# Lapis-Hong/wide_deep

Measured on NVIDIA H100. Metric: CTR examples/sec (train step), higher is better.
Workload: dtype bf16x3 (fp32 operands split into bf16 hi+lo, 3 tensor-core products, fp32 accumulate; 2^-16)

## Files before the change

wide_deep_b200/csrc/api.cu:

```cuda
#include <stdarg.h>
#include <stdlib.h>
#include <string.h>

#include <algorithm>
#include <cmath>
#include <random>

#include "common.cuh"
#include "farmhash.cuh"
#include "sparse_dev.cuh"

namespace wd {
static thread_local char g_err[1024] = "";
void set_error(const char* fmt, ...) {
    va_list ap;
    va_start(ap, fmt);
    vsnprintf(g_err, sizeof(g_err), fmt, ap);
    va_end(ap);
}
int init_sparse_tables(WdModel* m, uint64_t seed, int random_w);
int refresh_weight_copies(WdModel* m);
int wide_bias_grad(WdModel* m);
int metrics_setup();
int merge_sparse(WdModel* m, int which, const void* rows, const void* grads, int64_t n);
// ... 134 lines not shown
    if ((rc = upload(m, &p.col_field, d->col_field, C))) return rc;
    if ((rc = upload(m, &p.col_buckets, d->col_buckets, C))) return rc;
    if ((rc = upload(m, &p.col_aux_off, d->col_aux_off, C))) return rc;
    if ((rc = upload(m, &p.col_aux_n, d->col_aux_n, C))) return rc;
    if ((rc = upload(m, &p.col_norm_kind, d->col_norm_kind, C))) return rc;
    if ((rc = upload(m, &p.col_norm_a, d->col_norm_a, C))) return rc;
    if ((rc = upload(m, &p.col_norm_b, d->col_norm_b, C))) return rc;
    if ((rc = upload(m, &p.col_wide_base, d->col_wide_base, C))) return rc;
    if ((rc = upload(m, &p.col_emb_table, d->col_emb_table, C))) return rc;
    if ((rc = upload(m, &p.col_ind_off, d->col_ind_off, C))) return rc;
    if ((rc = upload(m, &p.vocab_fp, d->vocab_fp, d->n_vocab_fp))) return rc;
    if ((rc = upload(m, &p.boundaries, d->boundaries, d->n_boundaries))) return rc;
    if ((rc = upload(m, &p.cross_key_type, d->cross_key_type, d->n_cross_keys))) return rc;
    if ((rc = upload(m, &p.cross_key_idx, d->cross_key_idx, d->n_cross_keys))) return rc;
    if ((rc = upload(m, &m->d_num_field, d->num_field, d->n_numeric))) return rc;
    if ((rc = upload(m, &m->d_num_norm_kind, d->num_norm_kind, d->n_numeric))) return rc;
    if ((rc = upload(m, &m->d_num_x0_off, d->num_x0_off, d->n_numeric))) return rc;
    if ((rc = upload(m, &m->d_num_a, d->num_norm_a, d->n_numeric))) return rc;
    if ((rc = upload(m, &m->d_num_b, d->num_norm_b, d->n_numeric))) return rc;

    const int64_t Bm = m->max_batch;
    if ((rc = ensure_slot(m, 0))) return rc;
    if ((rc = dev_alloc(m, &m->d_col_offs, Bm * std::max(C, 1) + 2))) return rc;
    if ((rc = dev_alloc(m, &m->d_e_wide, m->max_nnz))) return rc;
    if ((rc = dev_alloc(m, &m->d_e_emb, m->max_nnz))) return rc;
    if ((rc = dev_alloc(m, &m->d_e_bc, m->max_nnz))) return rc;
    if ((rc = dev_alloc(m, &m->d_e_id, m->max_nnz))) return rc;
    if ((rc = dev_alloc(m, &m->d_nnz, 4))) return rc;
    if ((rc = dev_alloc(m, &m->d_flags, 4))) return rc;
    for (int k = 0; k < 4; ++k) if ((rc = dev_alloc(m, &m->d_sort_counter_s[k], 4))) return rc;
    {
        int64_t n = std::max<int64_t>(Bm * std::max(C, 1) + 2, m->max_nnz + 2);
        for (int k = 0; k < 4; ++k) {
            int32_t* t;
            if ((rc = dev_alloc(m, &t, n / 4096 + 8))) return rc;
            m->d_scan_tmp_s[k] = t;
        }
    }
    if ((rc = dev_alloc(m, &m->d_logits, Bm))) return rc;
    if (G == 1 && (rc = dev_alloc(m, &m->d_dlogit, Bm))) return rc;
    if ((rc = dev_alloc(m, &m->d_loss_part, 512))) return rc;
    if ((rc = dev_alloc(m, &m->d_loss, 4))) return rc;
    if ((rc = dev_alloc(m, &m->d_head_counter, 4))) return rc;
    if (getenv("WD_STEP_TRACE") && (rc = dev_alloc(m, &m->d_step_trace, 16))) return rc;
    if ((rc = dev_alloc(m, &m->d_step, 4))) return rc;
    if ((rc = dev_alloc(m, &m->d_bpow, 4))) return rc;
    {
        const float bp[4] = {m->lin_opt.beta1, m->lin_opt.beta2, m->dnn_opt.beta1, m->dnn_opt.beta2};
        WD_CUDA(cudaMemcpyAsync(m->d_bpow, bp, sizeof(bp), cudaMemcpyHostToDevice, m->stream));
        WD_CUDA(cudaStreamSynchronize(m->stream));
    }
    if (G == 1 && (rc = dev_alloc(m, &m->d_metrics, kMetricsDoubles))) return rc;
    WD_CUDA(cudaMallocHost(&m->h_loss_pinned, 64));

    auto add_dense = [&](int rows, int cols, int gparts, int g_rowtiles, int64_t gstride, bool transpose) {
        DenseTensor t{};
        t.off = m->dense_count; t.count = (int64_t)rows * cols; t.rows = rows; t.cols = cols;
        t.gpart_off = m->gpart_count; t.gparts = gparts; t.g_rowtiles = g_rowtiles; t.gstride = gstride;
        t.wt_off = transpose ? m->wt_count : -1;
        m->dense_count += (t.count + 3) / 4 * 4;
        m->gpart_count += (int64_t)gparts * gstride;
        if (transpose) m->wt_count += t.count;
        m->dense.push_back(t);
        return (int)m->dense.size() - 1;
    };
    if (m->use_wide) {
        add_dense(1, 1, m->row_tiles, 1, 4, false);
        if ((rc = dev_alloc(m, &m->d_wide, m->wide_rows))) return rc;
        if (m->lin_opt.kind == WD_OPT_ADAM && (rc = dev_alloc(m, &m->d_adam_touched[1], (m->wide_rows + 31) / 32))) return rc;
        if ((rc = dev_alloc(m, &m->d_wide_logit, Bm))) return rc;
    }

    m->x0_real.assign(std::max(d->d0_phys, 1), 0);
    if (m->use_deep) {
        int64_t row_base = 0;
        const int nslots = opt_nslots(m->dnn_opt);
        for (int t = 0; t < d->n_tables; ++t) {
            EmbTable tb{};
            tb.rows = d->table_rows[t]; tb.dim = d->table_dim[t]; tb.x0_off = d->table_x0_off[t];
            tb.dim_logical = d->table_dim_logical[t];
            if (tb.dim_logical < 1 || tb.dim_logical > tb.dim) { set_error("table %d: bad logical width", t); return WD_EINVAL; }
            tb.row_base = 0; tb.gs_off = -1; tb.stride = tb.dim * (1 + nslots); tb.col = -1;
            tb.sharded = G > 1 && d->table_sharded && d->table_sharded[t];
            tb.arows = tb.sharded ? (tb.rows - m->shard.rank + G - 1) / G : tb.rows;
            if (tb.dim % 4 || tb.x0_off % 4) { set_error("table %d: dim and deep-input offset must be multiples of 4", t); return WD_EINVAL; }
            for (int c = 0; c < C; ++c) if (d->col_emb_table[c] == t) tb.col = c;
            if (tb.col < 0) { set_error("table %d has no producing column", t); return WD_EINVAL; }
            tb.place = d->table_placement ? d->table_placement[t] : WD_PLACE_HBM;
            if (tb.place < WD_PLACE_HBM || tb.place > WD_PLACE_AUTO) { set_error("table %d: placement %d is not a WD_PLACE_*", t, tb.place); return WD_EINVAL; }
            tb.data = nullptr;
            for (int i = 0; i < tb.dim_logical; ++i) m->x0_real[tb.x0_off + i] = 1;
            m->emb_max_dim = std::max(m->emb_max_dim, tb.dim);
            m->tables.push_back(tb);
        }
        for (int pass = 0; pass < 2; ++pass) {
            if (pass == 1) m->small_base[0] = row_base;
            for (int t = 0; t < d->n_tables; ++t) {
                EmbTable& tb = m->tables[t];
                if (tb.sharded) continue;
                const bool small = m->dense_exchange_max_rows > 0 && tb.rows <= m->dense_exchange_max_rows;
                if (small != (pass == 1)) continue;
                if (small) {
                    m->n_small_tab++;
                    tb.gs_off = m->gs_emb_floats;
                    m->gs_emb_floats += tb.rows * tb.dim;
                }
                tb.row_base = row_base;
                row_base += tb.rows;
                m->rtab_order.push_back(t);
            }
        }
        m->emb_total_rows = row_base;
        if (m->dnn_opt.kind == WD_OPT_ADAM && (rc = dev_alloc(m, &m->d_adam_touched[0], (row_base + 31) / 32))) return rc;
        if (row_base >= (1ll << 31)) { set_error("more than 2^31 embedding rows on one device"); return WD_EUNSUPPORTED; }
        for (int i = 0; i < d->n_numeric; ++i) m->x0_real[d->num_x0_off[i]] = 1;
        for (int c = 0; c < C; ++c)
            if (d->col_ind_off[c] >= 0) for (int64_t i = 0; i < d->col_buckets[c]; ++i) m->x0_real[d->col_ind_off[c] + i] = 1;
        for (auto v : m->x0_real) m->d0_logical += v;
        const int nt = (int)m->tables.size();
        for (int t = 0; t < nt; ++t) {
            if (m->tables[t].sharded) continue;
            int di = -1;
            for (int i = 0; i < m->n_dims; ++i) if (m->dims[i] == m->tables[t].dim) di = i;
            if (di < 0) {
                if (m->n_dims == kMaxDims) { set_error("more than %d distinct embedding widths", kMaxDims); return WD_EUNSUPPORTED; }
                di = m->n_dims++; m->dims[di] = m->tables[t].dim; m->dim_ntables[di] = 0;
            }
            m->dim_ntables[di]++;
        }
        const int64_t actn = (int64_t)m->max_batch_pad * d->d0_phys;
        if ((rc = dev_alloc(m, &m->d_X0, actn))) return rc;
        if (fp32_ops && (rc = dev_alloc(m, &m->d_X0T, actn))) return rc;
        if (G == 1 && (rc = dev_alloc(m, &m->d_dX0, actn))) return rc;
        if (!fp32_ops)
            for (int part = 0; part < 2; ++part) {
                if ((rc = dev_alloc(m, &m->d_X0s[part], actn))) return rc;
            }

        if (d->n_towers > kMaxTowers) { set_error("more than %d towers", kMaxTowers); return WD_EUNSUPPORTED; }
        int hu_off = 0, did = 0;
        for (int t = 0; t < d->n_towers; ++t) {
            Tower tw{};
            tw.n_hidden = d->tower_nlayers[t]; tw.mode = d->tower_mode[t];
            std::vector<int> hu(d->hidden_units + hu_off, d->hidden_units + hu_off + tw.n_hidden);
            hu_off += tw.n_hidden;
            const std::vector<int> units = hu;
            if (m->crelu) for (int& h : hu) h *= 2;
            auto srcs = layer_sources(tw.mode, tw.n_hidden);
            for (int l = 0; l <= tw.n_hidden; ++l) {
                Layer L{};
                if ((int)srcs[l].size() > kMaxSegs) { set_error("layer with more than %d concatenated inputs", kMaxSegs); return WD_EUNSUPPORTED; }
                L.n_in_segs = (int)srcs[l].size();
                int koff = 0, klog = 0;
                for (int s = 0; s < L.n_in_segs; ++s) {
                    int src = srcs[l][s];
                    Seg sg{};
                    sg.src = src;
                    sg.width = src < 0 ? m->d0_logical : hu[src];
                    sg.width_phys = src < 0 ? d->d0_phys : pad_to(hu[src], 32);
                    sg.k_off = koff;
                    koff += sg.width_phys; klog += sg.width;
                    L.segs[s] = sg;
                }
                L.K = klog; L.K_phys = koff;
                const bool hidden = l < tw.n_hidden;
                L.N = hidden ? hu[l] : 1;
                L.N_phys = hidden ? pad_to(hu[l], 32) : 1;
                L.N_param = hidden ? units[l] : 1;
                L.t_gamma = L.t_beta = -1;
                bool logits_reads = false;
                for (int src : srcs[tw.n_hidden]) if (src == l) logits_reads = true;
                std::vector<int> idx(4, -1);
                if (hidden) {
                    {
                        const int tiles = ((L.K_phys + 127) / 128) * ((L.N_phys + 127) / 128);
                        int num_sms = kNumSms;
                        cudaDeviceGetAttribute(&num_sms, cudaDevAttrMultiProcessorCount, m->device);
                        int sp = m->wgrad_splits;
                        while (sp < 32 && tiles * sp * 2 <= num_sms && m->max_batch_pad / (sp * 2) >= 512) sp *= 2;
                        L.wgrad_splits = sp;
                    }
                    L.t_kernel = add_dense(L.K_phys, L.N_phys, L.wgrad_splits, 0, (int64_t)L.K_phys * L.N_phys, true);
                    L.t_bias = add_dense(1, L.N_phys, m->row_tiles, 1, L.N_phys, false);
                    if (m->crelu) m->dense[L.t_kernel].mirror_u = m->dense[L.t_bias].mirror_u = L.N_param;
                    if (m->batch_norm) {
                        L.t_gamma = add_dense(1, L.N_phys, m->row_tiles, 1, L.N_phys, false);
                        L.t_beta = add_dense(1, L.N_phys, m->row_tiles, 1, L.N_phys, false);
                    }
                    const int64_t n = (int64_t)m->max_batch_pad * L.N_phys;
                    if ((fp32_ops || logits_reads) && (rc = dev_alloc(m, &L.H, n))) return rc;
                    if (m->batch_norm || m->dropout_rate > 0.f || !L.H) { if ((rc = dev_alloc(m, &L.A, n))) return rc; } else L.A = L.H;
                    if (fp32_ops && (rc = dev_alloc(m, &L.HT, n))) return rc;
                    if ((rc = dev_alloc(m, &L.dH, n))) return rc;
                    if (fp32_ops) {
                        if ((rc = dev_alloc(m, &L.dZ, n))) return rc;
                        if ((rc = dev_alloc(m, &L.dZT, n))) return rc;
                    } else
                        for (int part = 0; part < 2; ++part) {
                            if ((rc = dev_alloc(m, &L.Hs[part], n))) return rc;
                            if ((rc = dev_alloc(m, &L.dZs[part], n))) return rc;
                        }
                } else {
                    L.t_kernel = add_dense(L.K_phys, 1, m->row_tiles, 1, L.K_phys, false);
                    L.t_bias = add_dense(1, 1, m->row_tiles, 1, 4, false);
                }
                idx[WD_D_KERNEL] = L.t_kernel; idx[WD_D_BIAS] = L.t_bias; idx[WD_D_GAMMA] = L.t_gamma; idx[WD_D_BETA] = L.t_beta;
                m->dense_index.push_back(idx);
                m->did_tower.push_back(t); m->did_layer.push_back(l);
                ++did;
                tw.layers.push_back(L);
            }
            if ((rc = dev_alloc(m, &tw.logit, Bm))) return rc;
            m->towers.push_back(tw);
        }
    }
    {
        const int64_t nw_small = m->use_wide ? m->wide_rows - m->small_base[1] : 0;
        const int64_t ne_small = (m->use_deep && m->n_small_tab > 0) ? m->emb_total_rows - m->small_base[0] : 0;
        const int64_t grads = m->gs_emb_floats + nw_small;
        m->gs_touch_off[0] = grads;
        m->gs_touch_off[1] = grads + ne_small;
        m->gs_count = grads > 0 ? grads + ne_small + nw_small : 0;
    }
    if (m->dense_count > 0) {
        if ((rc = dev_alloc(m, &m->d_P, m->dense_count))) return rc;
        if ((rc = dev_alloc(m, &m->d_S1, m->dense_count))) return rc;
        if ((rc = dev_alloc(m, &m->d_S2, m->dense_count))) return rc;
        if (G == 1 && (rc = dev_alloc(m, &m->d_G, m->dense_count + m->gs_count))) return rc;
        if ((rc = dev_alloc(m, &m->d_gpart, m->gpart_count))) return rc;
        if (fp32_ops) {
            if ((rc = dev_alloc(m, &m->d_Wt, m->wt_count))) return rc;
            float* split;
            if ((rc = dev_alloc(m, &split, 4 * m->wt_count))) return rc;
            m->d_W_hi = split; m->d_W_lo = split + m->wt_count; m->d_Wt_hi = split + 2 * m->wt_count; m->d_Wt_lo = split + 3 * m->wt_count;
        } else {
            if ((rc = dev_alloc(m, &m->d_Wq_hi, m->wt_count))) return rc;
            if ((rc = dev_alloc(m, &m->d_Wq_lo, m->wt_count))) return rc;
        }
        if ((rc = upload(m, &m->d_dense_desc, m->dense))) return rc;
    }

    m->sort_bits[0] = bits_for(std::max<int64_t>(m->emb_total_rows, 2));
    m->sort_bits[1] = bits_for(std::max<int64_t>(m->wide_rows, 2));
    if (m->sort_bits[0] > 30 || m->sort_bits[1] > 30) { set_error("more than 2^30 rows in one table space on one device"); return WD_EUNSUPPORTED; }
    const int which_lo = (m->use_deep && !m->tables.empty()) ? 0 : 1, which_hi = m->use_wide ? 1 : 0;
    for (int w = which_lo; w <= which_hi; ++w) {
        if ((rc = dev_alloc(m, &m->d_sk[w], m->max_nnz + 8))) return rc;
        if ((rc = dev_alloc(m, &m->d_sv[w], m->max_nnz + 8))) return rc;
        if ((rc = dev_alloc(m, &m->d_sk2[w], m->max_nnz + 8))) return rc;
        if ((rc = dev_alloc(m, &m->d_sv2[w], m->max_nnz + 8))) return rc;
        if ((rc = dev_alloc(m, &m->d_urow[w], m->max_nnz + 8))) return rc;
        if ((rc = dev_alloc(m, &m->d_ustart[w], m->max_nnz + 8))) return rc;
        if ((rc = dev_alloc(m, &m->d_ugrad[w], (m->max_nnz + 8) * (w == 0 ? std::max(m->emb_max_dim, 4) : 1)))) return rc;
        if ((rc = dev_alloc(m, &m->d_nuniq[w], 4))) return rc;
        if ((rc = dev_alloc(m, &m->d_nubig[w], 4))) return rc;
        if ((rc = dev_alloc(m, &m->d_nvalid[w], 4))) return rc;
        m->cpart_cap = 2 * (m->max_nnz / 16) + 64;
        if ((rc = dev_alloc(m, &m->d_choff[w], m->max_nnz + 8))) return rc;
        if ((rc = dev_alloc(m, &m->d_nchunks[w], 4))) return rc;
        if ((rc = dev_alloc(m, &m->d_cpart[w], m->cpart_cap * (w == 0 ? std::max(m->emb_max_dim, 4) : 1)))) return rc;
        m->sparse_cap[w] = m->max_nnz;
    }
    m->sort_hist_cap = 1024 * ((m->max_nnz + kSortTile - 1) / kSortTile + 1) + 4 * 1024 + 64;
    for (int k = 0; k < 4; ++k) if ((rc = dev_alloc(m, &m->d_sort_hist_s[k], m->sort_hist_cap))) return rc;
    if (m->use_deep) {
        if ((rc = place_tables(m, hbm_reserve_bytes(m) + (G > 1 ? shard_hbm_bytes(m, d) : 0)))) return rc;
    }
    if (G > 1 && (rc = shard_build(m, d))) return rc;
    if ((rc = build_record_sets(m))) return rc;
    if (G > 1) {
        DevPlan& dp = m->dplan;
        dp.sh_world = G;
        for (int sx = 0; sx < 2; ++sx) {
            ShardSpace& sp = m->shard.sp[sx];
            if (!sp.on) continue;
            if (sx == 0) { dp.sh_col_emb = sp.d_col_slot; dp.sh_base_emb = sp.set.rec.row_base; dp.sh_own_emb = sp.d_own; dp.sh_lrow_emb = sp.d_lrow; }
            else { dp.sh_col_wide = sp.d_col_slot; dp.sh_base_wide = sp.set.rec.row_base; dp.sh_own_wide = sp.d_own; dp.sh_lrow_wide = sp.d_lrow; }
        }
    }
    if ((rc = metrics_setup())) return rc;
    if ((rc = init_sparse_tables(m, 0, 0))) return rc;
    if ((rc = init_dense_slots(m))) return rc;
    for (auto& e : m->timer.ev) WD_CUDA(new_event(m, &e, cudaEventDefault));
    WD_CUDA(cudaStreamSynchronize(m->stream));
    return WD_OK;
}

extern "C" int wd_model_create(const WdPlanDesc* d, int device, WdModel** out) {
    if (!d || !out) { set_error("null argument"); return WD_EINVAL; }
    if (d->api_version != WD_API_VERSION) { set_error("plan api_version %d != library %d", d->api_version, WD_API_VERSION); return WD_EINVAL; }
    int ndev = 0;
    if (cudaGetDeviceCount(&ndev) != cudaSuccess || ndev == 0) {
        set_error("no CUDA device: libwd_b200 has no CPU fallback");
        return WD_ENODEVICE;
    }
    if (device < 0 || device >= ndev) { set_error("device %d out of range (%d devices)", device, ndev); return WD_EINVAL; }
    WD_CUDA(cudaSetDevice(device));
    WdModel* m = new WdModel();
    m->device = device;
    cudaError_t e = cudaSuccess;
    for (cudaStream_t* s : {&m->stream, &m->stream_up, &m->sstream[0], &m->sstream[1]})
        if (e == cudaSuccess) e = new_stream(m, s);
    for (cudaEvent_t* ev : {&m->ev_grouped[0], &m->ev_grouped[1], &m->ev_done[0], &m->ev_done[1], &m->ev_ids, &m->ev_wide_fwd,
                            &m->ev_wgrad_rest, &m->ev_head, &m->ev_dx0, &m->ev_bwd_done})
        if (e == cudaSuccess) e = new_event(m, ev, cudaEventDisableTiming);
    if (e != cudaSuccess) { set_error("cudaStreamCreate: %s", cudaGetErrorString(e)); wd_model_destroy(m); return WD_ECUDA; }
    m->graphs_enabled = getenv("WD_NO_GRAPH") == nullptr;
    int rc = build_model(d, m);
    if (rc) { wd_model_destroy(m); return rc; }
    *out = m;
    return WD_OK;
}

namespace wd {
int64_t hbm_reserve_bytes(const WdModel* m) {
    constexpr int kReserveSlots = 16;
    constexpr int64_t kGraphReserve = 256ll << 20;
    const int64_t Bm = m->max_batch;
    const int64_t slot_bytes = (Bm * std::max(m->n_cat_fields, 1) + 1) * 4 + m->keys_cap * 8 + Bm * std::max(m->n_dense_fields, 1) * 4 + 2 * Bm * 4;
    int max_stride = 0;
    for (auto& tb : m->tables) max_stride = std::max(max_stride, tb.stride);
    const int64_t stage_bytes = m->max_nnz * ((int64_t)max_stride + 1) * 4 + 64 * (int64_t)m->tables.size() + 4096;
    return kReserveSlots * slot_bytes + stage_bytes + kGraphReserve;
}
}

static int init_dense(WdModel* m, uint64_t seed) {
    if (m->dense_count == 0) return WD_OK;
    std::vector<float> P(m->dense_count, 0.f), S1(m->dense_count, 0.f), S2(m->dense_count, 0.f);
    std::mt19937_64 rng(seed * 7919 + 17);
    std::uniform_real_distribution<float> U(-1.f, 1.f);
    for (size_t ti = 0; ti < m->towers.size(); ++ti) {
        Tower& tw = m->towers[ti];
        for (int l = 0; l <= tw.n_hidden; ++l) {
            Layer& L = tw.layers[l];
            const DenseTensor& tk = m->dense[L.t_kernel];
            const float lim = std::sqrt(6.f / (float)(L.K + L.N_param));
            for (int s = 0; s < L.n_in_segs; ++s) {
                const Seg& sg = L.segs[s];
                for (int j = 0; j < sg.width_phys; ++j) {
                    bool real = sg.src < 0 ? (m->x0_real[j] != 0) : (j < sg.width);
                    if (!real) continue;
                    float* prow = &P[tk.off + (int64_t)(sg.k_off + j) * L.N_phys];
                    for (int n = 0; n < L.N_param; ++n) {
                        prow[n] = lim * U(rng);
                        if (tk.mirror_u) prow[n + tk.mirror_u] = -prow[n];
                    }
                }
            }
            if (L.t_gamma >= 0) for (int n = 0; n < L.N; ++n) P[m->dense[L.t_gamma].off + n] = 1.f;
        }
    }
    for (size_t i = 0; i < m->dense.size(); ++i) {
        const WdOptimizer& o = (m->use_wide && i == 0) ? m->lin_opt : m->dnn_opt;
        float s1 = slot1_init(o);
        for (int64_t j = 0; j < m->dense[i].count; ++j) S1[m->dense[i].off + j] = s1;
    }
    WD_CUDA(cudaMemcpyAsync(m->d_P, P.data(), P.size() * 4, cudaMemcpyHostToDevice, m->stream));
    WD_CUDA(cudaMemcpyAsync(m->d_S1, S1.data(), S1.size() * 4, cudaMemcpyHostToDevice, m->stream));
    WD_CUDA(cudaMemcpyAsync(m->d_S2, S2.data(), S2.size() * 4, cudaMemcpyHostToDevice, m->stream));
    WD_CUDA(cudaStreamSynchronize(m->stream));
    return refresh_weight_copies(m);
}

extern "C" int wd_model_init(WdModel* m, uint64_t seed) {
    if (!m) { set_error("null model"); return WD_EINVAL; }
    WD_CUDA(cudaSetDevice(m->device));
    int rc = init_sparse_tables(m, seed, 1);
    if (rc) return rc;
    rc = init_dense(m, seed);
    if (rc) return rc;
    WD_CUDA(cudaStreamSynchronize(m->stream));
    m->initialized = true;
    return WD_OK;
}

static int resolve_dense(WdModel* m, int did, int sub, int* out) {
    if (did < 0 || did >= (int)m->dense_index.size() || sub < 0 || sub > 3 || m->dense_index[did][sub] < 0) {
        set_error("no dense tensor (%d, %d)", did, sub);
        return WD_EINVAL;
    }
    *out = m->dense_index[did][sub];
    return WD_OK;
}

extern "C" int64_t wd_tensor_size(WdModel* m, int kind, int index, int sub) {
    if (!m) return WD_EINVAL;
    if (kind == WD_T_WIDE_COL) {
        if (index < 0 || index >= m->n_columns) return WD_EINVAL;
        const ShardSpace& sw = m->shard.sp[1];
        if (sw.on && sw.h_col_slot[index] >= 0) return (m->col_buckets[index] - m->shard.rank + m->shard.world - 1) / m->shard.world;
        return m->col_wide_base[index] >= 0 ? m->col_buckets[index] : WD_EINVAL;
    }
    if (kind == WD_T_WIDE_BIAS) return m->use_wide ? 1 : WD_EINVAL;
    if (kind == WD_T_EMB_TABLE) return (index >= 0 && index < (int)m->tables.size()) ? m->tables[index].arows * m->tables[index].dim_logical : WD_EINVAL;
    if (kind == WD_T_DENSE) {
        int di;
        if (resolve_dense(m, index, sub, &di)) return WD_EINVAL;
        Layer& L = m->towers[m->did_tower[index]].layers[m->did_layer[index]];
        return sub == WD_D_KERNEL ? (int64_t)L.K * L.N_param : (sub == WD_D_BIAS ? L.N_param : L.N);
    }
    return WD_EINVAL;
}

extern "C" int wd_memory_usage(WdModel* m, int64_t* device_bytes, int64_t* host_bytes) {
    if (!m) { set_error("null model"); return WD_EINVAL; }
    if (device_bytes) *device_bytes = m->bytes_allocated;
    if (host_bytes) *host_bytes = m->host_bytes;
    return WD_OK;
}

extern "C" int wd_tensor_io(WdModel* m, int kind, int index, int sub, int slot, void* host, int64_t count, int to_device) {
    if (!m || !host) { set_error("null argument"); return WD_EINVAL; }
    WD_CUDA(cudaSetDevice(m->device));
    WD_CUDA(cudaStreamSynchronize(m->stream));
    int64_t want = wd_tensor_size(m, kind, index, sub);
    if (want < 0 || want != count) { set_error("tensor (%d,%d,%d): size %lld, caller passed %lld", kind, index, sub, (long long)want, (long long)count); return WD_EINVAL; }
    if (slot < 0 || slot > 2) { set_error("slot out of range"); return WD_EINVAL; }
    const cudaMemcpyKind dir = to_device ? cudaMemcpyHostToDevice : cudaMemcpyDeviceToHost;
    if (kind == WD_T_WIDE_COL) {
        const ShardSpace& sw = m->shard.sp[1];
        float* dev = (sw.on && sw.h_col_slot[index] >= 0)
                         ? reinterpret_cast<float*>(sw.d_wide + sw.h_slot_base[sw.h_col_slot[index]]) + slot
                         : reinterpret_cast<float*>(m->d_wide + m->col_wide_base[index]) + slot;
        if (to_device) WD_CUDA(cudaMemcpy2DAsync(dev, 16, host, 4, 4, count, dir, m->stream));
        else WD_CUDA(cudaMemcpy2DAsync(host, 4, dev, 16, 4, count, dir, m->stream));
        WD_CUDA(cudaStreamSynchronize(m->stream));
        return WD_OK;
    }
    if (kind == WD_T_EMB_TABLE) {
        EmbTable& tb = m->tables[index];
        if (slot * tb.dim >= tb.stride) { set_error("table has no optimizer slot %d", slot); return WD_EINVAL; }
        float* dev = tb.data + slot * tb.dim;
        const size_t lw = (size_t)tb.dim_logical * 4;
        if (tb.host) {
            const int rc = host_cache_sync(m, true, to_device != 0);
            if (rc) return rc;
        }
        const cudaMemcpyKind dir = tb.host ? cudaMemcpyDefault : (to_device ? cudaMemcpyHostToDevice : cudaMemcpyDeviceToHost);
        if (to_device) WD_CUDA(cudaMemcpy2DAsync(dev, (size_t)tb.stride * 4, host, lw, lw, tb.arows, dir, m->stream));
        else WD_CUDA(cudaMemcpy2DAsync(host, lw, dev, (size_t)tb.stride * 4, lw, tb.arows, dir, m->stream));
        WD_CUDA(cudaStreamSynchronize(m->stream));
        return WD_OK;
    }
    float* arena = slot == 0 ? m->d_P : (slot == 1 ? m->d_S1 : m->d_S2);
    if (kind == WD_T_WIDE_BIAS) {
        WD_CUDA(cudaMemcpyAsync(to_device ? (void*)(arena + m->dense[0].off) : host, to_device ? host : (void*)(arena + m->dense[0].off), 4, dir, m->stream));
        WD_CUDA(cudaStreamSynchronize(m->stream));
        return WD_OK;
    }
    int di;
    int rc = resolve_dense(m, index, sub, &di);
    if (rc) return rc;
    const DenseTensor& t = m->dense[di];
    Layer& L = m->towers[m->did_tower[index]].layers[m->did_layer[index]];
    std::vector<float> phys(t.count, 0.f);
    float* h = (float*)host;
    if (!to_device || slot > 0) {
        WD_CUDA(cudaMemcpyAsync(phys.data(), arena + t.off, t.count * 4, cudaMemcpyDeviceToHost, m->stream));
        WD_CUDA(cudaStreamSynchronize(m->stream));
    }
    if (sub == WD_D_KERNEL) {
        int64_t lk = 0;
        for (int s = 0; s < L.n_in_segs; ++s) {
            const Seg& sg = L.segs[s];
            for (int j = 0; j < sg.width_phys; ++j) {
                bool real = sg.src < 0 ? (m->x0_real[j] != 0) : (j < sg.width);
                if (!real) continue;
                for (int n = 0; n < L.N_param; ++n) {
                    float& pv = phys[(int64_t)(sg.k_off + j) * L.N_phys + n];
                    if (to_device) {
                        pv = h[lk * L.N_param + n];
                        if (t.mirror_u) (&pv)[t.mirror_u] = slot == 0 ? -pv : pv;
                    } else h[lk * L.N_param + n] = pv;
                }
                ++lk;
            }
        }
        if (lk != L.K) { set_error("internal: logical K mismatch %lld vs %d", (long long)lk, L.K); return WD_ESTATE; }
    } else {
        const int nn = sub == WD_D_BIAS ? L.N_param : L.N;
        for (int n = 0; n < nn; ++n) {
            if (to_device) {
                phys[n] = h[n];
                if (t.mirror_u) phys[n + t.mirror_u] = slot == 0 ? -h[n] : h[n];
            } else h[n] = phys[n];
        }
    }
    if (to_device) {
        WD_CUDA(cudaMemcpyAsync(arena + t.off, phys.data(), t.count * 4, cudaMemcpyHostToDevice, m->stream));
        WD_CUDA(cudaStreamSynchronize(m->stream));
        if (slot == 0 && t.wt_off >= 0) return refresh_weight_copies(m);
    }
    return WD_OK;
}

static int check_ready(WdModel* m) {
    if (!m) { set_error("null model"); return WD_EINVAL; }
    WD_CUDA(cudaSetDevice(m->device));
    return WD_OK;
}
static void timer_begin(WdModel* m) {
    if (!m->timer.enabled) return;
    m->timer.n = 0;
    mark(m, "start");
}

static int ensure_slot(WdModel* m, int s) {
    if (s < 0 || s >= 64) { set_error("batch slot %d out of range [0, 64)", s); return WD_EINVAL; }
    while ((int)m->slots.size() <= s) {
        BatchSlot b;
        int rc;
        const int64_t Bm = m->max_batch;
        if ((rc = dev_alloc(m, &b.off, Bm * std::max(m->n_cat_fields, 1) + 1))) return rc;
        if ((rc = dev_alloc(m, &b.keys, m->keys_cap))) return rc;
        if ((rc = dev_alloc(m, &b.dense, Bm * std::max(m->n_dense_fields, 1)))) return rc;
        if ((rc = dev_alloc(m, &b.label, Bm))) return rc;
        if ((rc = dev_alloc(m, &b.weight, Bm))) return rc;
        m->slots.push_back(b);
    }
    return WD_OK;
}
static int select_slot(WdModel* m, int s) {
    int rc = ensure_slot(m, s);
    if (rc) return rc;
    BatchSlot& b = m->slots[s];
    m->cur_slot = s;
    if (b.filled) m->dbatch = b.view;
    if (b.up_pending) {
        WD_CUDA(cudaStreamWaitEvent(m->stream, b.ev_up, 0));
        b.up_pending = false;
    }
    return WD_OK;
}
static int use_slot(WdModel* m, int slot, const char* needs_labels) {
    int rc = select_slot(m, slot);
    if (rc) return rc;
    if (!m->slots[slot].filled) { set_error("batch slot %d was never uploaded", slot); return WD_ESTATE; }
    if (needs_labels && !m->dbatch.label) { set_error("%s needs labels", needs_labels); return WD_EINVAL; }
    return WD_OK;
}
static void fill_slot(WdModel* m, int s, const DevBatch& view, bool pending) {
    BatchSlot& sl = m->slots[s];
    sl.view = view;
    sl.filled = true;
    if (pending) sl.up_pending = true;
    if (s == m->cur_slot) m->dbatch = view;
}
static int mark_slot_used(WdModel* m) {
    BatchSlot& b = m->slots[m->cur_slot];
    if (!b.ev_used) WD_CUDA(new_event(m, &b.ev_used, cudaEventDisableTiming));
    WD_CUDA(cudaEventRecord(b.ev_used, m->stream));
    b.used_recorded = true;
    return WD_OK;
}

static int upload_into(WdModel* m, BatchSlot& sl, const WdBatch* b, cudaStream_t st, DevBatch* view) {
    if (!b || b->batch_size <= 0 || b->batch_size > m->max_batch) { set_error("batch_size %d outside (0, %d]", b ? b->batch_size : -1, m->max_batch); return WD_EINVAL; }
    const int B = b->batch_size, F = m->n_cat_fields, Nd = m->n_dense_fields;
    int64_t nnz = b->cat_offsets ? b->nnz : (int64_t)B * F;
    if (nnz > m->keys_cap) { set_error("batch has %lld keys, capacity %lld (raise max_keys)", (long long)nnz, (long long)m->keys_cap); return WD_EINVAL; }
    if (F > 0) {
        if (b->cat_offsets) WD_CUDA(cudaMemcpyAsync(sl.off, b->cat_offsets, ((int64_t)B * F + 1) * 4, cudaMemcpyHostToDevice, st));
        if (nnz > 0) WD_CUDA(cudaMemcpyAsync(sl.keys, b->cat_keys, nnz * 8, cudaMemcpyHostToDevice, st));
    }
    if (Nd > 0) WD_CUDA(cudaMemcpyAsync(sl.dense, b->dense, (int64_t)B * Nd * 4, cudaMemcpyHostToDevice, st));
    if (b->label) WD_CUDA(cudaMemcpyAsync(sl.label, b->label, (int64_t)B * 4, cudaMemcpyHostToDevice, st));
    if (b->weight) WD_CUDA(cudaMemcpyAsync(sl.weight, b->weight, (int64_t)B * 4, cudaMemcpyHostToDevice, st));
    view->B = B;
    view->cat_offsets = (F > 0 && b->cat_offsets) ? sl.off : nullptr;
    view->cat_keys = sl.keys;
    view->dense = sl.dense;
    view->label = b->label ? sl.label : nullptr;
    view->weight = b->weight ? sl.weight : nullptr;
    return WD_OK;
}

static int upload_current(WdModel* m, const WdBatch* b) {
    DevBatch view{};
    int rc = upload_into(m, m->slots[m->cur_slot], b, m->stream, &view);
    if (rc) return rc;
    fill_slot(m, m->cur_slot, view, false);
    mark(m, "h2d");
    return WD_OK;
}

extern "C" int wd_batch_prefetch_slot(WdModel* m, int slot, const WdBatch* b) {
    int rc = check_ready(m);
    if (rc) return rc;
    if ((rc = ensure_slot(m, slot))) return rc;
    BatchSlot& sl = m->slots[slot];
    if (!sl.ev_up) WD_CUDA(new_event(m, &sl.ev_up, cudaEventDisableTiming));
    if (sl.used_recorded) WD_CUDA(cudaStreamWaitEvent(m->stream_up, sl.ev_used, 0));
    DevBatch view{};
    if ((rc = upload_into(m, sl, b, m->stream_up, &view))) return rc;
    WD_CUDA(cudaEventRecord(sl.ev_up, m->stream_up));
    fill_slot(m, slot, view, true);
    return WD_OK;
}

extern "C" int wd_tsv_parse_slot(WdModel* m, int slot, const WdTsvSpec* sp, const char* text, int64_t text_len, const int64_t* starts,
                                 int32_t n_lines) {
    int rc = check_ready(m);
    if (rc) return rc;
    if (!sp || !text || !starts || n_lines < 0 || text_len < 0) { set_error("wd_tsv_parse_slot: bad arguments"); return WD_EINVAL; }
    if ((rc = ensure_slot(m, slot))) return rc;
    BatchSlot& sl = m->slots[slot];
    if (!sl.ev_up) WD_CUDA(new_event(m, &sl.ev_up, cudaEventDisableTiming));
    if (sl.used_recorded) WD_CUDA(cudaStreamWaitEvent(m->stream_up, sl.ev_used, 0));
    int status = 0;
    if ((rc = tsv_parse_device(m, sp, text, text_len, starts, n_lines, sl.off, sl.keys, sl.dense, sl.label, sl.weight, m->stream_up, &status))) return rc;
    DevBatch view{};
    if (status == 0) {
        view.B = n_lines;
        view.cat_offsets = m->n_cat_fields > 0 ? sl.off : nullptr;
        view.cat_keys = sl.keys;
        view.dense = sl.dense;
        view.label = sp->has_label ? sl.label : nullptr;
        view.weight = (sp->use_weight && sp->has_label) ? sl.weight : nullptr;
        m->tsv_device_batches++;
    } else {
        WdBatch hb{};
        if ((rc = tsv_parse_host(sp, text, starts, n_lines, &hb))) return rc;
        if ((rc = upload_into(m, sl, &hb, m->stream_up, &view))) return rc;
        m->tsv_host_batches++;
    }
    WD_CUDA(cudaEventRecord(sl.ev_up, m->stream_up));
    if (status != 0) WD_CUDA(cudaEventSynchronize(sl.ev_up));
    fill_slot(m, slot, view, true);
    return WD_OK;
}

extern "C" int wd_tsv_parse_stats(WdModel* m, int64_t* out, int32_t n, int32_t reset) {
    if (!m) { set_error("null model"); return WD_EINVAL; }
    const int64_t v[2] = {m->tsv_device_batches, m->tsv_host_batches};
    for (int i = 0; i < n && i < 2; ++i) out[i] = v[i];
    if (reset) m->tsv_device_batches = m->tsv_host_batches = 0;
    return WD_OK;
}

extern "C" int wd_batch_upload_slot(WdModel* m, int slot, const WdBatch* b) {
    int rc = check_ready(m);
    if (rc) return rc;
    if ((rc = select_slot(m, slot))) return rc;
    return upload_current(m, b);
}
extern "C" int wd_batch_upload(WdModel* m, const WdBatch* b) { return wd_batch_upload_slot(m, 0, b); }

static int finish_step(WdModel* m, float* loss_out, float* logits_out) {
    int32_t* flags_host = reinterpret_cast<int32_t*>(m->h_loss_pinned + 4);
    WD_CUDA(cudaMemcpyAsync(m->h_loss_pinned, m->d_loss, 4, cudaMemcpyDeviceToHost, m->stream));
    WD_CUDA(cudaMemcpyAsync(flags_host, m->d_flags, 4, cudaMemcpyDeviceToHost, m->stream));
    if (logits_out) WD_CUDA(cudaMemcpyAsync(logits_out, m->d_logits, (int64_t)m->dbatch.B * 4, cudaMemcpyDeviceToHost, m->stream));
    mark(m, "d2h");
    WD_CUDA(cudaStreamSynchronize(m->stream));
    if (flags_host[0] & 1) {
        cudaMemsetAsync(m->d_flags, 0, 16, m->stream);
        set_error("categorical-column id capacity exceeded (max_nnz=%lld): recreate the model with a larger max_nnz", (long long)m->max_nnz);
        return WD_EINVAL;
    }
    if (flags_host[0] & 2) {
        cudaMemsetAsync(m->d_flags, 0, 16, m->stream);
        set_error("row-sharded exchange capacity exceeded (a rank received more than %lld ids): raise shard_slack / shard_capacity", (long long)m->max_nnz);
        return WD_EINVAL;
    }
    if (flags_host[0] & 8) {
        cudaMemsetAsync(m->d_flags, 0, 16, m->stream);
        set_error("data-parallel list exchange: this rank touched more unique rows than the fixed list length it exchanges (wd_sparse_set_sorted list_len); raise fixed_rows");
        return WD_EINVAL;
    }
    if (flags_host[0] & 4) {
        cudaMemsetAsync(m->d_flags, 0, 16, m->stream);
        set_error("row-sharded exchange: a peer rank did not reach a barrier within 20 s (ranks out of step, or a rank failed)");
        return WD_ESTATE;
    }
    if (loss_out) *loss_out = m->dbatch.label ? m->h_loss_pinned[0] : 0.f;
    if (m->timer.enabled) {
        PhaseTimer& t = m->timer;
        for (int i = 1; i < t.n; ++i) cudaEventElapsedTime(&t.ms[i], t.ev[i - 1], t.ev[i]);
        t.ms[0] = 0.f;
        if (t.n > 1) cudaEventElapsedTime(&t.ms[0], t.ev[0], t.ev[t.n - 1]);
        t.n_last = t.n;
    }
    return WD_OK;
}

static bool list_present(const WdModel* m, int which) { return which == 0 ? (m->use_deep && !m->tables.empty()) : m->use_wide; }

__global__ void step_stamp_kernel(unsigned long long* t) { unsigned long long v; asm volatile("mov.u64 %0, %%globaltimer;" : "=l"(v)); *t = v; }
enum { ST_START = 0, ST_IDS, ST_GATHER, ST_HEAD, ST_BWD, ST_MAIN_END, ST_G0, ST_G1, ST_R0_BEG, ST_R0_END, ST_R1_BEG, ST_R1_END, ST_A0_END, ST_A1_END };
static void stamp(WdModel* m, int i) {
    if (!m->d_step_trace) return;
    step_stamp_kernel<<<1, 1, 0, m->stream>>>(m->d_step_trace + i);
    m->launches++;
}

namespace wd {
int group_async(WdModel* m) {
    if (m->timer.enabled) return WD_OK;
    WD_CUDA(cudaEventRecord(m->ev_ids, m->stream));
    for (int w = 0; w < 2; ++w) {
        if (!list_present(m, w)) continue;
        WD_CUDA(cudaStreamWaitEvent(m->sstream[w], m->ev_ids, 0));
        int rc = on_side(m, w, [&] { int r = sparse_group_which(m, w); stamp(m, ST_G0 + w); return r; });
        if (rc) return rc;
        WD_CUDA(cudaEventRecord(m->ev_grouped[w], m->sstream[w]));
        m->side_pending[w] = true;
    }
    return WD_OK;
}

static int forward_core(WdModel* m, bool train) {
    int rc;
    m->stepped = true;
    stamp(m, ST_START);
    if ((rc = ids_prepare(m))) return rc;
    mark(m, "ids");
    stamp(m, ST_IDS);
    const bool wide_aside = train && !m->timer.enabled && m->use_wide && m->use_deep && list_present(m, 1);
    if (wide_aside) {
        WD_CUDA(cudaEventRecord(m->ev_ids, m->stream));
        WD_CUDA(cudaStreamWaitEvent(m->sstream[1], m->ev_ids, 0));
        if ((rc = on_side(m, 1, [&] { return sparse_forward_wide(m); }))) return rc;
        WD_CUDA(cudaEventRecord(m->ev_wide_fwd, m->sstream[1]));
    }
    if (train && (rc = group_async(m))) return rc;
    if (!wide_aside && (rc = sparse_forward_wide(m))) return rc;
    if (m->n_host_tab > 0) {
        if (m->side_pending[0]) WD_CUDA(cudaStreamWaitEvent(m->stream, m->ev_grouped[0], 0));
        else if ((rc = sparse_group_which(m, 0))) return rc;
        if ((rc = host_tables_stage_in(m, train))) return rc;
    }
    if ((rc = sparse_forward_emb(m))) return rc;
    stamp(m, ST_GATHER);
    if ((rc = mlp_forward(m, train))) return rc;
    mark(m, "mlp_other");
    if (wide_aside) WD_CUDA(cudaStreamWaitEvent(m->stream, m->ev_wide_fwd, 0));
    if ((rc = loss_forward(m, train))) return rc;
    mark(m, "head");
    stamp(m, ST_HEAD);
    if (train && (m->side_pending[0] || m->side_pending[1])) WD_CUDA(cudaEventRecord(m->ev_head, m->stream));
    if (train && m->summary_armed && (rc = summary_launch(m))) return rc;
    return WD_OK;
}

int backward_core(WdModel* m) {
    int rc;
    m->side_active[0] = m->side_active[1] = false;
    if (m->gs_count > 0) WD_CUDA(cudaMemsetAsync(m->d_G + m->dense_count, 0, (size_t)m->gs_count * sizeof(float), m->stream));
    if (m->side_pending[1]) {
        if (m->gs_count > 0) { WD_CUDA(cudaEventRecord(m->ev_head, m->stream)); }
        WD_CUDA(cudaStreamWaitEvent(m->sstream[1], m->ev_head, 0));
        if ((rc = on_side(m, 1, [&] { stamp(m, ST_R1_BEG); int r = sparse_reduce_wide(m); if (!r) r = small_scatter(m, 1); stamp(m, ST_R1_END); return r; }))) return rc;
        m->side_active[1] = true;
    }
    m->record_dx0 = m->side_pending[0];
    m->dx0_recorded = false;
    m->dense_split_tensor = -1;
    m->record_wgrad_rest = m->fuse_dense && m->side_active[1] && m->operands == kBf16Operands && !m->timer.enabled && !m->crelu;
    if ((rc = mlp_backward(m))) return rc;
    m->record_dx0 = false;
    m->record_wgrad_rest = false;
    mark(m, "mlp_other");
    stamp(m, ST_BWD);
    if (m->side_pending[0] && m->dx0_recorded) {
        WD_CUDA(cudaStreamWaitEvent(m->sstream[0], m->ev_dx0, 0));
        if ((rc = on_side(m, 0, [&] { stamp(m, ST_R0_BEG); int r = sparse_reduce_emb(m); if (!r) r = small_scatter(m, 0); stamp(m, ST_R0_END); return r; }))) return rc;
        m->side_active[0] = true;
    }
    if ((rc = wide_bias_grad(m))) return rc;
    if ((rc = dense_reduce_grads(m))) return rc;
    mark(m, "dense_reduce");
    for (int w = 0; w < 2; ++w) {
        if (m->side_active[w] || !list_present(m, w)) { m->side_pending[w] = false; continue; }
        if (m->side_pending[w]) WD_CUDA(cudaStreamWaitEvent(m->stream, m->ev_grouped[w], 0));
        else if ((rc = sparse_group_which(m, w))) return rc;
        m->side_pending[w] = false;
        if ((rc = (w == 0 ? sparse_reduce_emb(m) : sparse_reduce_wide(m)))) return rc;
        if ((rc = small_scatter(m, w))) return rc;
    }
    if (m->gs_count > 0)
        for (int w = 0; w < 2; ++w)
            if (m->side_active[w]) {
                WD_CUDA(cudaEventRecord(m->ev_done[w], m->sstream[w]));
                WD_CUDA(cudaStreamWaitEvent(m->stream, m->ev_done[w], 0));
            }
    m->grads_pending = true;
    return WD_OK;
}

int apply_core(WdModel* m) {
    int rc;
    const bool split_dense = m->fuse_dense && m->dense_split_tensor >= 0 && m->side_active[1];
    for (int w = 0; w < 2; ++w) {
        if (m->side_active[w]) {
            if ((rc = on_side(m, w, [&]() -> int {
                    int r = sparse_apply_which(m, w);
                    stamp(m, ST_A0_END + w);
                    if (!r && w == 1 && split_dense) {
                        WD_CUDA(cudaStreamWaitEvent(m->stream, m->ev_wgrad_rest, 0));
                        m->dense_part = 2;
                        r = dense_apply(m);
                        m->dense_part = 0;
                    }
                    return r;
                }))) return rc;
            WD_CUDA(cudaEventRecord(m->ev_done[w], m->sstream[w]));
        } else if ((rc = sparse_apply_which(m, w))) return rc;
    }
    mark(m, "sparse_apply");
    m->dense_part = split_dense ? 1 : 0;
    rc = dense_apply(m);
    m->dense_part = 0;
    if (rc) return rc;
    if ((rc = small_apply(m))) return rc;
    mark(m, "dense_apply");
    stamp(m, ST_MAIN_END);
    if (m->dropout_rate > 0.f && (rc = step_tick(m))) return rc;
    if (m->lin_opt.kind == WD_OPT_ADAM || m->dnn_opt.kind == WD_OPT_ADAM) {
        for (int w = 0; w < 2; ++w)
            if (m->side_active[w]) WD_CUDA(cudaStreamWaitEvent(m->stream, m->ev_done[w], 0));
        if ((rc = adam_untouched_replicated(m))) return rc;
        mark(m, "adam_untouched");
        if ((rc = adam_tick(m))) return rc;
    }
    for (int w = 0; w < 2; ++w)
        if (m->side_active[w]) { WD_CUDA(cudaStreamWaitEvent(m->stream, m->ev_done[w], 0)); m->side_active[w] = false; }
    m->grads_pending = false;
    return WD_OK;
}
}

static int train_eager(WdModel* m) {
    int rc;
    m->fuse_dense = true;
    rc = forward_core(m, true);
    if (!rc) rc = backward_core(m);
    if (!rc) rc = apply_core(m);
    m->fuse_dense = false;
    return rc;
}

enum class GraphRun { eager, captured, replayed };

template <class Key, class F>
static int run_graphed(WdModel* m, StepGraph<Key>& g, const Key& key, cudaStream_t st, F issue, GraphRun* how) {
    *how = GraphRun::eager;
    if (!m->graphs_enabled || m->timer.enabled) return issue(false);
    if (g.exec && g.key == key) {
        *how = GraphRun::replayed;
        m->graph_replays++;
    } else if (g.eager < 2) {
        const int rc = issue(false);
        if (rc == WD_OK) g.eager++;
        return rc;
    } else {
        g.destroy();
        const int64_t l0 = m->launches;
        cudaGraph_t graph = nullptr;
        cudaError_t e = cudaStreamBeginCapture(st, cudaStreamCaptureModeThreadLocal);
        if (e == cudaSuccess) {
            const int rc = issue(true);
            const cudaError_t e2 = cudaStreamEndCapture(st, &graph);
            if (rc == WD_OK && e2 == cudaSuccess && graph) e = cudaGraphInstantiate(&g.exec, graph, 0);
            else e = e2 != cudaSuccess ? e2 : cudaErrorUnknown;
            if (graph) cudaGraphDestroy(graph);
        }
        if (e != cudaSuccess || !g.exec) {
            cudaGetLastError();
            g.exec = nullptr;
            m->graphs_enabled = false;
            return issue(false);
        }
        g.key = key;
        g.launches = m->launches - l0;
        m->launches = l0;
        *how = GraphRun::captured;
        m->graph_captures++;
    }
    WD_CUDA(cudaGraphLaunch(g.exec, st));
    m->launches += g.launches;
    return WD_OK;
}

template <class Key, class F>
static int run_train_graphed(WdModel* m, StepGraph<Key>& g, const Key& key, F issue, GraphRun* how) {
    if (m->summary_armed) {
        *how = GraphRun::eager;
        return issue(false);
    }
    return run_graphed(m, g, key, m->stream, issue, how);
}

static int after_graph(WdModel* m, GraphRun how, BatchSlot* bwd) {
    if (how == GraphRun::eager) return WD_OK;
    if (bwd && how == GraphRun::captured)
        for (int w = 0; w < 2; ++w) bwd->bwd_side_active[w] = m->side_active[w];
    if (bwd) WD_CUDA(cudaEventRecord(m->ev_bwd_done, m->stream));
    for (int w = 0; w < 2; ++w) {
        m->side_pending[w] = false;
        m->side_active[w] = bwd && bwd->bwd_side_active[w];
        if (m->side_active[w]) WD_CUDA(cudaStreamWaitEvent(m->sstream[w], m->ev_bwd_done, 0));
    }
    m->grads_pending = bwd != nullptr;
    return WD_OK;
}

static int train_current(WdModel* m, float* loss_out) {
    GraphRun how;
    int rc = run_train_graphed(m, m->slots[m->cur_slot].train, m->dbatch, [&](bool) { return train_eager(m); }, &how);
    if (rc) return rc;
    if ((rc = after_graph(m, how, nullptr))) return rc;
    if ((rc = mark_slot_used(m))) return rc;
    if (loss_out) return finish_step(m, loss_out, nullptr);
    return WD_OK;
}

extern "C" int wd_train_step_slot(WdModel* m, int slot, float* loss_out) {
    int rc = check_ready(m);
    if (rc) return rc;
    if ((rc = use_slot(m, slot, "training"))) return rc;
    timer_begin(m);
    return train_current(m, loss_out);
}
extern "C" int wd_train_step_resident(WdModel* m, float* loss_out) { return wd_train_step_slot(m, 0, loss_out); }

extern "C" int wd_train_step(WdModel* m, const WdBatch* b, float* loss_out) {
    int rc = check_ready(m);
    if (rc) return rc;
    if ((rc = select_slot(m, 0))) return rc;
    timer_begin(m);
    if ((rc = upload_current(m, b))) return rc;
    if ((rc = use_slot(m, 0, "training"))) return rc;
    float dummy;
    return train_current(m, loss_out ? loss_out : &dummy);
}

extern "C" int wd_forward_resident(WdModel* m, float* logits_out, float* loss_out) {
    int rc = check_ready(m);
    if (rc) return rc;
    if ((rc = select_slot(m, 0))) return rc;
    timer_begin(m);
    if ((rc = forward_core(m, false))) return rc;
    return finish_step(m, loss_out, logits_out);
}

extern "C" int wd_forward(WdModel* m, const WdBatch* b, float* logits_out, float* loss_out) {
    int rc = check_ready(m);
    if (rc) return rc;
    if ((rc = select_slot(m, 0))) return rc;
    timer_begin(m);
    if ((rc = upload_current(m, b))) return rc;
    if ((rc = forward_core(m, false))) return rc;
    return finish_step(m, loss_out, logits_out);
}


static int backward_eager(WdModel* m, bool join) {
    int rc;
    if ((rc = forward_core(m, true))) return rc;
    if ((rc = backward_core(m))) return rc;
    if (join)
        for (int w = 0; w < 2; ++w)
            if (m->side_active[w]) {
                WD_CUDA(cudaEventRecord(m->ev_done[w], m->sstream[w]));
                WD_CUDA(cudaStreamWaitEvent(m->stream, m->ev_done[w], 0));
            }
    return WD_OK;
}

static int refuse_split_step_with_cache(WdModel* m) {
    if (m->hcache.slots == 0) return WD_OK;
    set_error("the split step (wd_step_backward / wd_step_apply) is not supported on a model with a host-table cache");
    return WD_EUNSUPPORTED;
}

extern "C" int wd_step_backward_slot(WdModel* m, int slot, float* loss_out) {
    int rc = check_ready(m);
    if (rc) return rc;
    if ((rc = use_slot(m, slot, "training"))) return rc;
    if ((rc = refuse_split_step_with_cache(m))) return rc;
    timer_begin(m);
    BatchSlot& sl = m->slots[slot];
    GraphRun how;
    if ((rc = run_train_graphed(m, sl.bwd, m->dbatch, [&](bool capturing) { return backward_eager(m, capturing); }, &how))) return rc;
    if ((rc = after_graph(m, how, &sl))) return rc;
    if ((rc = mark_slot_used(m))) return rc;
    if (loss_out) return finish_step(m, loss_out, nullptr);
    return WD_OK;
}

extern "C" int wd_last_loss(WdModel* m, float* loss_out) {
    int rc = check_ready(m);
    if (rc) return rc;
    if (!loss_out) { set_error("wd_last_loss: null output"); return WD_EINVAL; }
    return finish_step(m, loss_out, nullptr);
}

extern "C" int wd_step_backward(WdModel* m, const WdBatch* b, float* loss_out) {
    int rc = check_ready(m);
    if (rc) return rc;
    if ((rc = refuse_split_step_with_cache(m))) return rc;
    if (b && (rc = wd_batch_upload(m, b))) return rc;
    timer_begin(m);
    if (!m->dbatch.label) { set_error("training needs labels"); return WD_EINVAL; }
    if ((rc = forward_core(m, true))) return rc;
    if ((rc = backward_core(m))) return rc;
    if (loss_out) return finish_step(m, loss_out, nullptr);
    return WD_OK;
}

extern "C" int wd_step_apply(WdModel* m) {
    int rc = check_ready(m);
    if (rc) return rc;
    if (!m->grads_pending) { set_error("wd_step_apply without wd_step_backward"); return WD_ESTATE; }
    return apply_core(m);
}

extern "C" int64_t wd_dense_grad_count(WdModel* m) { return m ? m->dense_count + m->gs_count : 0; }
extern "C" void* wd_dense_grad_ptr(WdModel* m) { return m ? m->d_G : nullptr; }

extern "C" int wd_sparse_grads(WdModel* m, int which, void** rows, void** grads, int64_t* n, int32_t* width, int64_t* capacity) {
    int rc = check_ready(m);
    if (rc) return rc;
    if (which < 0 || which > 1 || !m->d_urow[which]) { set_error("no sparse gradient list %d", which); return WD_EINVAL; }
    if (n) {
        int32_t nu = 0;
        WD_CUDA(cudaStreamSynchronize(m->stream));
        WD_CUDA(cudaStreamSynchronize(m->sstream[which]));
        WD_CUDA(cudaMemcpy(&nu, m->d_nuniq[which], 4, cudaMemcpyDeviceToHost));
        *n = nu;
    }
    if (rows) *rows = m->d_urow[which];
    if (grads) *grads = m->d_ugrad[which];
    if (width) *width = which == 0 ? m->emb_max_dim : 1;
    if (capacity) *capacity = m->sparse_cap[which];
    return WD_OK;
}

static int sparse_set_impl(WdModel* m, int which, const void* rows_dev, const void* grads_dev, int64_t n, int n_lists, int64_t list_len) {
    int rc = check_ready(m);
    if (rc) return rc;
    if (which < 0 || which > 1 || !m->d_urow[which]) { set_error("no sparse gradient list %d", which); return WD_EINVAL; }
    const bool side = m->side_active[which];
    auto merge = [&]() -> int {
        return n_lists > 0 ? merge_sparse_sorted(m, which, rows_dev, grads_dev, n_lists, list_len) : merge_sparse(m, which, rows_dev, grads_dev, n);
    };
    auto run = [&](bool) -> int { return side ? on_side(m, which, merge) : merge(); };
    if (n_lists == 0) return run(false);
    GraphRun how;
    return run_graphed(m, m->merge_graph[which], MergeKey{rows_dev, grads_dev, n_lists, list_len, side}, side ? m->sstream[which] : m->stream, run, &how);
}

extern "C" int wd_sparse_set(WdModel* m, int which, const void* rows_dev, const void* grads_dev, int64_t n) {
    return sparse_set_impl(m, which, rows_dev, grads_dev, n, 0, 0);
}
extern "C" int wd_sparse_set_sorted(WdModel* m, int which, const void* rows_dev, const void* grads_dev, int32_t n_lists, int64_t list_len) {
    if (n_lists < 1 || list_len < 1) { set_error("wd_sparse_set_sorted: bad list shape"); return WD_EINVAL; }
    return sparse_set_impl(m, which, rows_dev, grads_dev, 0, n_lists, list_len);
}

static int shard_ready(WdModel* m, int slot, const char* needs_labels) {
    int rc = check_ready(m);
    if (rc) return rc;
    if (m->shard.world <= 1) { set_error("model has no row-sharded tables (shard_world <= 1)"); return WD_ESTATE; }
    if (!m->shard.connected) { set_error("row-sharded model is not connected to its peers (wd_shard_connect_ipc / wd_shard_connect_local)"); return WD_ESTATE; }
    return use_slot(m, slot, needs_labels);
}

extern "C" int wd_shard_phase(WdModel* m, int slot, int phase, int train) {
    int rc = shard_ready(m, slot, train ? "training" : nullptr);
    if (rc) return rc;
    if (m->shard.ipc) { set_error("wd_shard_phase is for ranks of one process; multi-process ranks call wd_shard_train_step_slot"); return WD_ESTATE; }
    if (phase < 0 || phase > 4) { set_error("wd_shard_phase: phase %d outside [0, 4]", phase); return WD_EINVAL; }
    if (phase == 0) timer_begin(m);
    if ((rc = shard_step(m, train != 0, phase))) return rc;
    return train && phase == 4 ? mark_slot_used(m) : WD_OK;
}

extern "C" int wd_shard_finish(WdModel* m, float* loss_out, float* logits_out) {
    int rc = check_ready(m);
    if (rc) return rc;
    return finish_step(m, loss_out, logits_out);
}

extern "C" int wd_shard_train_step_slot(WdModel* m, int slot, float* loss_out) {
    int rc = shard_ready(m, slot, "training");
    if (rc) return rc;
    if (!m->shard.ipc) { set_error("wd_shard_train_step_slot needs wd_shard_connect_ipc (ranks of one process use wd_shard_phase)"); return WD_ESTATE; }
    timer_begin(m);
    GraphRun how;
    if ((rc = run_train_graphed(m, m->slots[slot].shard, m->dbatch, [&](bool) { return shard_step(m, true, kAllSegments); }, &how))) return rc;
    if ((rc = after_graph(m, how, nullptr))) return rc;
    if ((rc = mark_slot_used(m))) return rc;
    if (loss_out) return finish_step(m, loss_out, nullptr);
    return WD_OK;
}

extern "C" int wd_shard_forward_slot(WdModel* m, int slot, float* logits_out, float* loss_out) {
    int rc = shard_ready(m, slot, nullptr);
    if (rc) return rc;
    if (!m->shard.ipc) { set_error("wd_shard_forward_slot needs wd_shard_connect_ipc"); return WD_ESTATE; }
    if ((rc = shard_step(m, false, kAllSegments))) return rc;
    return finish_step(m, loss_out, logits_out);
}

namespace wd { int shard_metrics_reduce(WdModel* m); }

static int check_eval_rows(WdModel* m, int32_t n_valid) {
    if (n_valid < 0 || n_valid > m->dbatch.B) { set_error("n_valid %d outside [0, batch size %d]", n_valid, m->dbatch.B); return WD_EINVAL; }
    if (n_valid > 0 && !m->dbatch.label) { set_error("evaluation needs labels"); return WD_EINVAL; }
    return WD_OK;
}

extern "C" int wd_shard_eval_accumulate_slot(WdModel* m, int slot, int32_t n_valid) {
    int rc = shard_ready(m, slot, nullptr);
    if (rc) return rc;
// ... 191 lines not shown
```

wide_deep_b200/csrc/common.cuh:

```cuda
#pragma once
#include <cuda_bf16.h>
#include <cuda_runtime.h>
#include <stdint.h>
#include <stdio.h>
#include <string>
#include <vector>

#include "../../include/wd_b200.h"

namespace wd {

constexpr int kSortTile = 1024;

void set_error(const char* fmt, ...);

#define WD_CUDA(call)                                                                         \
    do {                                                                                      \
        cudaError_t e__ = (call);                                                             \
        if (e__ != cudaSuccess) {                                                             \
            wd::set_error("%s:%d %s -> %s", __FILE__, __LINE__, #call, cudaGetErrorString(e__)); \
            return WD_ECUDA;                                                                  \
        }                                                                                     \
    } while (0)

constexpr uint32_t kInvalidRow = 0xFFFFFFFFu;
constexpr int kMaxSegs = 8;
constexpr int kMaxTowers = 8;
constexpr int kNumSms = 132;
constexpr int kMaxDims = 8;
constexpr int kLists = 6;
constexpr int kMaxRanks = 16;
constexpr int kMetricsDoubles = 512;

struct DevPlan {
    int n_cat_fields, n_dense_fields, n_columns;
    const uint8_t* field_is_string;
    const int32_t* col_kind;
    const int32_t* col_field;
    const int64_t* col_buckets;
    const int32_t* col_aux_off;
    const int32_t* col_aux_n;
    const int32_t* col_norm_kind;
    const float* col_norm_a;
    const float* col_norm_b;
    const int64_t* col_wide_base;
    const int32_t* col_emb_table;
    const int32_t* col_ind_off;
    const uint64_t* vocab_fp;
    const float* boundaries;
    const int32_t* cross_key_type;
    const int32_t* cross_key_idx;
    const int64_t* table_row_base;
    int d0_phys;
    int sh_world;
    const int32_t *sh_col_emb, *sh_col_wide;
    const int64_t *sh_base_emb, *sh_base_wide;
    uint32_t *sh_own_emb, *sh_lrow_emb, *sh_own_wide, *sh_lrow_wide;
};

struct DevBatch {
    int B;
    const int32_t* cat_offsets;
    const uint64_t* cat_keys;
    const float* dense;
    const float* label;
    const float* weight;
};

struct EmbTable {
    int64_t rows;
    int dim;
    int dim_logical;
    int x0_off;
    int col;
    int64_t row_base;
    int64_t gs_off;
    float* data;
    int stride;
    bool sharded;
    int64_t arows;
    int place;
    bool host;
};

struct TabDesc {
    float* data;
    int64_t row_base;
    int stride, x0, col, dim;
};

struct RowRecords {
    int ntab;
    const int64_t* row_base;
    float* const* data;
    const int32_t* dim;
    const int32_t* stride;
    const int32_t* stage;
    float* stage_base;
    const int32_t* uslot;
};
struct RecordSet {
    RowRecords rec{};
    const int32_t* x0 = nullptr;
    const int64_t* rows = nullptr;
    const int64_t* gs_off = nullptr;
};

struct HostCache {
    int64_t slots = 0;
    int set_bits = 0;
    uint32_t* d_tag = nullptr;
    uint32_t* d_stamp = nullptr;
    uint8_t* d_dirty = nullptr;
    uint32_t* d_now = nullptr;
    unsigned long long* d_stats = nullptr;
    int32_t* d_uslot = nullptr;
    uint32_t* d_uvict = nullptr;
    uint8_t* d_uflag = nullptr;
    uint32_t *d_ck[2] = {}, *d_cv[2] = {};
};

struct DenseTensor {
    int64_t off;
    int64_t count;
    int rows, cols;
    int64_t gpart_off;
    int gparts;
    int g_rowtiles;
    int64_t gstride;
    int64_t wt_off;
    int mirror_u;
};

enum OperandFamily { kFp32Operands = 0, kBf16Operands = 1 };

struct Seg {
    int src;
    int width;
    int width_phys;
    int k_off;
};

struct Layer {
    int n_in_segs;
    Seg segs[kMaxSegs];
    int K, K_phys;
    int N, N_phys;
    int N_param;
    int t_kernel, t_bias, t_gamma, t_beta;
    int wgrad_splits;
    float* A;
    float* H;
    float* HT;
    float* dH;
    float* dZ;
    float* dZT;
    __nv_bfloat16 *Hs[2], *dZs[2];
    float* colpart;
};

struct Tower {
    int n_hidden;
    int mode;
    std::vector<Layer> layers;
    float* logit;
};

struct PhaseTimer {
    static constexpr int kMax = 160;
    cudaEvent_t ev[kMax];
    const char* name[kMax];
    float ms[kMax];
    int n = 0, n_last = 0;
    bool enabled = false;
};

template <class Key>
struct StepGraph {
    cudaGraphExec_t exec = nullptr;
    Key key{};
    int64_t launches = 0;
    int eager = 0;
    void destroy() {
        if (exec) cudaGraphExecDestroy(exec);
        exec = nullptr;
    }
};
inline bool operator==(const DevBatch& a, const DevBatch& b) {
    return a.B == b.B && a.cat_offsets == b.cat_offsets && a.cat_keys == b.cat_keys && a.dense == b.dense && a.label == b.label && a.weight == b.weight;
}
struct MergeKey {
    const void* rows;
    const void* grads;
    int n_lists;
    int64_t list_len;
    bool on_side;
    bool operator==(const MergeKey& o) const {
        return rows == o.rows && grads == o.grads && n_lists == o.n_lists && list_len == o.list_len && on_side == o.on_side;
    }
};

struct ShardEvalKey {
    DevBatch b;
    int n_valid;
    bool operator==(const ShardEvalKey& o) const { return b == o.b && n_valid == o.n_valid; }
};

struct BatchSlot {
    int32_t* off = nullptr;
    uint64_t* keys = nullptr;
    float *dense = nullptr, *label = nullptr, *weight = nullptr;
    DevBatch view{};
    bool filled = false;
    cudaEvent_t ev_up = nullptr;
    cudaEvent_t ev_used = nullptr;
    bool up_pending = false, used_recorded = false;
    StepGraph<DevBatch> train;
    StepGraph<DevBatch> bwd;
    StepGraph<DevBatch> shard;
    StepGraph<ShardEvalKey> shard_eval;
    bool bwd_side_active[2] = {false, false};
};


struct ShardPeer {
    uint2* inbox;
    int32_t* inbox_cnt;
    float* recv;
    const float* bagscale;
    const float* gradbase;
};
struct ShardSpace {
    bool on = false;
    int width = 0;
    int n_slots = 0;
    int bags_per_row = 0;
    int64_t nbags_cap = 0;
    int64_t local_rows = 0;
    int64_t pair_cap = 0;
    std::vector<int32_t> h_col_slot;
    std::vector<int64_t> h_slot_base;
    int32_t* d_col_slot = nullptr;
    RecordSet set;
    uint32_t* d_adam_touched = nullptr;
    int stage_stride = 0;
    float* d_stage = nullptr;
    HostCache cache;
    float4* d_wide = nullptr;
    uint32_t* d_own = nullptr;
    uint32_t* d_lrow = nullptr;
    int32_t* d_ostart = nullptr;
    int32_t* d_bagmask = nullptr;
    uint32_t* d_rtag = nullptr;
    uint32_t* d_rrow = nullptr;
    int32_t* d_nrecv = nullptr;
    ShardPeer* d_peers = nullptr;
    ShardPeer peers[kMaxRanks];
    int64_t off_inbox = 0, off_cnt = 0, off_recv = 0, off_bagscale = 0, off_grad = 0;
};
struct ShardState {
    int world = 1, rank = 0;
    bool connected = false, ipc = false;
    uint8_t* seg = nullptr;
    int64_t seg_bytes = 0;
    uint8_t* peer_seg[kMaxRanks] = {};
    ShardSpace sp[2];
    int64_t off_flags = 0, off_gred = 0, off_G = 0;
    int64_t off_metrics = 0;
    double* d_msum = nullptr;
    uint32_t** d_peer_flags = nullptr;
    uint32_t* d_epoch = nullptr;
    unsigned long long* d_trace = nullptr;
    float** d_peer_G = nullptr;
    float** d_peer_gred = nullptr;
    float* gred = nullptr;
    int64_t ar_count = 0;
    cudaEvent_t ev_a = nullptr;
    cudaStream_t aux = nullptr;
    cudaEvent_t ev_ids2 = nullptr, ev_routed1 = nullptr, ev_a2 = nullptr, ev_aux_done = nullptr;
};
constexpr int kBarriers = 8;
constexpr int kAllSegments = -1;

constexpr int kSummaryThreads = 256;
constexpr int kSummaryZeroBucket = (WD_SUMMARY_BUCKETS + 1) / 2;
struct SummarySeg {
    int kind;
    const float* ptr; int ld, cols;
    const uint8_t* mask;
    const float *gamma, *beta; int bn;
    float drop_rate; int layer_id;
    int blk0, nblk;
};
struct SummaryState {
    std::vector<SummarySeg> h;
    std::vector<int32_t> kind, tower, layer;
    int blocks = 0;
    SummarySeg* d_seg = nullptr;
    uint8_t* d_mask = nullptr;
    double* d_limits = nullptr;
    unsigned long long* d_counts = nullptr;
    double* d_part = nullptr;
    long long* d_ipart = nullptr;
};

struct TsvDev;

struct DevAlloc { void* p; int64_t bytes; };

}

struct WdModel {
    int device = 0;
    bool use_wide = false, use_deep = false;
    int n_cat_fields = 0, n_dense_fields = 0, n_columns = 0;
    std::vector<int32_t> col_kind, col_field, col_aux_off, col_aux_n, col_norm_kind, col_emb_table, col_ind_off;
    std::vector<int64_t> col_buckets, col_wide_base;
    std::vector<float> col_norm_a, col_norm_b;
    int n_numeric = 0;
    int d0_phys = 0;
    int64_t wide_rows = 0;
    int activation = 0, batch_norm = 0;
    WdOptimizer lin_opt{}, dnn_opt{};
    int max_batch = 0, max_batch_pad = 0;
    int64_t max_nnz = 0;
    int gemm_engine = 0;
    wd::OperandFamily operands = wd::kFp32Operands;

    cudaStream_t stream = nullptr;
    cudaStream_t sstream[2] = {nullptr, nullptr};
    cudaStream_t stream_up = nullptr;
    cudaEvent_t ev_ids = nullptr, ev_head = nullptr, ev_dx0 = nullptr, ev_bwd_done = nullptr, ev_wide_fwd = nullptr, ev_wgrad_rest = nullptr;
    bool sort_smem_opt_in = false;
    bool crelu = false;
    bool list_apply_fused[2] = {false, false};
    bool record_wgrad_rest = false;
    int dense_split_tensor = -1, dense_part = 0;
    cudaEvent_t ev_grouped[2] = {nullptr, nullptr}, ev_done[2] = {nullptr, nullptr};
    bool side_pending[2] = {false, false};
    bool side_active[2] = {false, false};
    bool record_dx0 = false, dx0_recorded = false;
    wd::StepGraph<wd::MergeKey> merge_graph[2];
    int64_t dense_exchange_max_rows = 0;
    int64_t small_base[2] = {0, 0};
    int64_t gs_count = 0, gs_emb_floats = 0;
    int64_t gs_touch_off[2] = {0, 0};
    int n_small_tab = 0;
    uint32_t* d_adam_touched[2] = {nullptr, nullptr};
    int32_t* d_nubig[2] = {nullptr, nullptr};
    wd::ShardState shard;
    wd::DevPlan dplan{};
    std::vector<cudaStream_t> streams;
    std::vector<cudaEvent_t> events;
    std::vector<wd::DevAlloc> allocs;
    int64_t bytes_allocated = 0;
    std::vector<void*> host_allocs;
    int64_t host_bytes = 0;
    int n_host_tab = 0;
    std::vector<int> rtab_order;
    float* d_stage = nullptr;
    int stage_stride = 0;
    uint32_t* d_g_emb = nullptr;
    wd::HostCache hcache;
    bool stepped = false;

    int32_t *d_num_field = nullptr, *d_num_norm_kind = nullptr, *d_num_x0_off = nullptr;
    float *d_num_a = nullptr, *d_num_b = nullptr;

    int64_t keys_cap = 0;
    wd::DevBatch dbatch{};

    int32_t* d_col_offs = nullptr;
    uint32_t* d_e_wide = nullptr;
    uint32_t* d_e_emb = nullptr;
    int32_t* d_e_bc = nullptr;
    int32_t* d_e_id = nullptr;
    int32_t* d_nnz = nullptr;
    int32_t* d_flags = nullptr;
    void* d_scan_tmp_s[4] = {nullptr, nullptr, nullptr, nullptr};
    int scratch_sel = 0;

    float4* d_wide = nullptr;
    float* d_wide_logit = nullptr;

    std::vector<wd::EmbTable> tables;
    int64_t emb_total_rows = 0;
    int emb_max_dim = 0;
    int n_dims = 0;
    int dims[wd::kMaxDims];
    int dim_ntables[wd::kMaxDims];
    wd::RecordSet tabs;
    wd::RecordSet rtabs;
    wd::TabDesc* d_dim_desc[wd::kMaxDims] = {};
    float *d_X0 = nullptr, *d_dX0 = nullptr;
    float* d_X0T = nullptr;
    __nv_bfloat16* d_X0s[2] = {nullptr, nullptr};
    int ldt = 0;
    std::vector<wd::Tower> towers;

    std::vector<wd::DenseTensor> dense;
    int64_t dense_count = 0, gpart_count = 0, wt_count = 0;
    float *d_P = nullptr, *d_S1 = nullptr, *d_S2 = nullptr, *d_G = nullptr, *d_gpart = nullptr;
    float* d_Wt = nullptr;
    float *d_W_hi = nullptr, *d_W_lo = nullptr;
    float *d_Wt_hi = nullptr, *d_Wt_lo = nullptr;
    __nv_bfloat16 *d_Wq_hi = nullptr, *d_Wq_lo = nullptr;
    wd::DenseTensor* d_dense_desc = nullptr;
    int row_tiles = 0;
    int wgrad_splits = 4;

    float* d_logits = nullptr;
    float* d_dlogit = nullptr;
    float* d_loss_part = nullptr;
    float* d_loss = nullptr;
    unsigned long long* d_step_trace = nullptr;
    int32_t* d_head_counter = nullptr;
    float* d_bpow = nullptr;
    float* h_loss_pinned = nullptr;

    uint32_t *d_sk[wd::kLists] = {}, *d_sv[wd::kLists] = {};
    uint32_t *d_sk2[wd::kLists] = {}, *d_sv2[wd::kLists] = {};
    int32_t* d_sort_hist_s[4] = {nullptr, nullptr, nullptr, nullptr};
    int64_t sort_hist_cap = 0;
    int32_t* d_sort_counter_s[4] = {nullptr, nullptr, nullptr, nullptr};
    uint32_t* d_urow[wd::kLists] = {};
    int32_t* d_ustart[wd::kLists] = {};
    float* d_ugrad[wd::kLists] = {};
    int32_t* d_nuniq[wd::kLists] = {};
    int32_t* d_nvalid[wd::kLists] = {};
    int32_t* d_choff[wd::kLists] = {};
    int32_t* d_nchunks[wd::kLists] = {};
    float* d_cpart[wd::kLists] = {};
    int64_t cpart_cap = 0;
    int64_t sparse_cap[2] = {0, 0};
    bool sparse_overridden[2] = {false, false};
    int64_t sparse_override_n[2] = {0, 0};
    int sort_bits[wd::kLists] = {};

    double* d_metrics = nullptr;
    int64_t eval_batches = 0;

    int64_t launches = 0;
    int64_t graph_captures = 0, graph_replays = 0;
    float dropout_rate = 0.f;
    unsigned long long dropout_seed = 0;
    unsigned int* d_step = nullptr;
    bool fuse_dense = false;
    int64_t gemm_fallbacks = 0;
    int cur_slot = 0;
    bool graphs_enabled = true;
    int cur_layer = 0;
    wd::PhaseTimer timer;
    std::vector<wd::BatchSlot> slots;
    wd::TsvDev* tsv = nullptr;
    int64_t tsv_device_batches = 0, tsv_host_batches = 0;
    bool initialized = false;
    bool grads_pending = false;
    wd::SummaryState* summ = nullptr;
    bool summary_armed = false, summary_ready = false;

    std::vector<uint8_t> x0_real;
    int d0_logical = 0;
    std::vector<std::vector<int>> dense_index;
    std::vector<int> did_tower, did_layer;
};

namespace wd {
int ids_prepare(WdModel* m);
int sparse_forward(WdModel* m);
int sparse_forward_wide(WdModel* m);
int sparse_forward_emb(WdModel* m);
int sparse_group(WdModel* m);
int sparse_reduce_emb(WdModel* m);
int sparse_reduce_wide(WdModel* m);
int sparse_apply(WdModel* m);
int sparse_apply_which(WdModel* m, int which);
int sparse_group_which(WdModel* m, int which);
int merge_sparse_sorted(WdModel* m, int which, const void* rows, const void* grads, int n_lists, int64_t list_len);
int small_scatter(WdModel* m, int which);
int small_apply(WdModel* m);
int adam_untouched_replicated(WdModel* m);
int mlp_forward(WdModel* m, bool want_transposes);
int mlp_backward(WdModel* m);
int dense_reduce_grads(WdModel* m);
int dense_apply(WdModel* m);
int loss_forward(WdModel* m, bool need_grad);
int model_init_params(WdModel* m, uint64_t seed);
int step_tick(WdModel* m);
int adam_tick(WdModel* m);
int place_tables(WdModel* m, int64_t hbm_reserve);
int build_record_sets(WdModel* m);
int host_tables_stage_in(WdModel* m, bool train);
int host_tables_write_back(WdModel* m);
int host_cache_sync(WdModel* m, bool flush, bool invalidate);
struct CacheMarks { const char *sort, *assign, *in, *out; };
int stage_in_rows(WdModel* m, HostCache& c, int L, const RowRecords& rr, int S, bool train, const CacheMarks& marks);
int write_back_rows(WdModel* m, const HostCache& c, int L, const RowRecords& rr, int S, const CacheMarks& marks);
int64_t shard_hbm_bytes(const WdModel* m, const WdPlanDesc* d);
int64_t hbm_reserve_bytes(const WdModel* m);
int tsv_parse_device(WdModel* m, const WdTsvSpec* sp, const char* text, int64_t text_len, const int64_t* starts, int n, int32_t* off,
                     uint64_t* keys, float* dense, float* label, float* weight, cudaStream_t st, int* status);
int tsv_parse_host(const WdTsvSpec* sp, const char* text, const int64_t* starts, int n, WdBatch* out);
void tsv_dev_destroy(WdModel* m);
int metrics_accumulate(WdModel* m, int rows);
int metrics_finish(WdModel* m, const double* acc, double* out10);
int summary_prepare(WdModel* m, const std::vector<uint8_t>& x0_real);
int summary_launch(WdModel* m);

int radix_sort_pairs(WdModel* m, uint32_t** keys, uint32_t** vals, uint32_t** keys2, uint32_t** vals2, int bits, const int32_t* d_n);
int exclusive_scan_i32(WdModel* m, int32_t* data, int64_t n, int32_t* total_out);
int seg_heads(WdModel* m, const int32_t* d_n, const uint32_t* keys, uint32_t invalid, int32_t* pos, int64_t cap, int32_t* ustart, uint32_t* urow,
              int32_t* d_nuniq);
int chunk_offsets(WdModel* m, const int32_t* d_nuniq, const int32_t* ustart, uint32_t* urow, int32_t* choff, int64_t cap, int chunk,
                  int32_t* d_nchunks);

template <typename T>
int dev_alloc(WdModel* m, T** p, int64_t count, bool zero = true) {
    if (count <= 0) count = 1;
    void* q = nullptr;
    cudaError_t e = cudaMalloc(&q, (size_t)count * sizeof(T));
    if (e != cudaSuccess) {
        set_error("cudaMalloc of %lld bytes failed: %s", (long long)(count * sizeof(T)), cudaGetErrorString(e));
        return WD_ENOMEM;
    }
    if (zero) {
        e = cudaMemsetAsync(q, 0, (size_t)count * sizeof(T), m->stream);
        if (e != cudaSuccess) { set_error("cudaMemset failed: %s", cudaGetErrorString(e)); return WD_ECUDA; }
    }
    m->allocs.push_back({q, count * (int64_t)sizeof(T)});
    m->bytes_allocated += count * (int64_t)sizeof(T);
    *p = (T*)q;
    return WD_OK;
}
inline int dev_free(WdModel* m, void* p) {
    for (size_t i = 0; i < m->allocs.size(); ++i) {
        if (m->allocs[i].p != p) continue;
        WD_CUDA(cudaFree(p));
        m->bytes_allocated -= m->allocs[i].bytes;
        m->allocs.erase(m->allocs.begin() + i);
        break;
    }
    return WD_OK;
}
inline cudaError_t new_stream(WdModel* m, cudaStream_t* s) {
    const cudaError_t e = cudaStreamCreateWithFlags(s, cudaStreamNonBlocking);
    if (e == cudaSuccess) m->streams.push_back(*s);
    return e;
}
inline cudaError_t new_event(WdModel* m, cudaEvent_t* ev, unsigned flags) {
    const cudaError_t e = cudaEventCreateWithFlags(ev, flags);
    if (e == cudaSuccess) m->events.push_back(*ev);
    return e;
}
template <typename T> struct same_type { using type = T; };
template <typename T>
int upload(WdModel* m, T** dst, const typename same_type<T>::type* src, int64_t n) {
    if (!*dst) {
        int rc = dev_alloc(m, dst, n, true);
        if (rc) return rc;
    }
    if (n > 0) WD_CUDA(cudaMemcpyAsync((void*)*dst, src, n * sizeof(T), cudaMemcpyHostToDevice, m->stream));
    return WD_OK;
}
template <typename T, typename A>
int upload(WdModel* m, T** dst, const std::vector<A>& h) { return upload(m, dst, h.data(), (int64_t)h.size()); }

inline void mark(WdModel* m, const char* name) {
    PhaseTimer& t = m->timer;
    if (!t.enabled || t.n >= PhaseTimer::kMax) return;
    t.name[t.n] = name;
    cudaEventRecord(t.ev[t.n], m->stream);
    t.n++;
}

template <typename F>
int on_stream(WdModel* m, cudaStream_t stream, int scratch_sel, F fn) {
    cudaStream_t main_stream = m->stream;
    m->stream = stream; m->scratch_sel = scratch_sel;
    int rc = fn();
    m->stream = main_stream; m->scratch_sel = 0;
    return rc;
}
template <typename F>
int on_side(WdModel* m, int which, F fn) { return on_stream(m, m->sstream[which], 1 + which, fn); }
template <typename F>
int on_aux(WdModel* m, F fn) { return on_stream(m, m->shard.aux, 3, fn); }

inline int grid_for(int64_t n, int block, int cap = kNumSms * 16) {
    int64_t g = (n + block - 1) / block;
    if (g < 1) g = 1;
    if (g > cap) g = cap;
    return (int)g;
}
}
```

wide_deep_b200/csrc/gemm.cuh:

```cuda
#pragma once
#include <cuda.h>
#include <cuda_bf16.h>

#include "common.cuh"

namespace wd {

__device__ __forceinline__ float act_fwd(int kind, float z) {
    switch (kind) {
        case WD_ACT_RELU: return fmaxf(z, 0.f);
        case WD_ACT_RELU6: return fminf(fmaxf(z, 0.f), 6.f);
        case WD_ACT_SIGMOID: return 1.f / (1.f + expf(-z));
        case WD_ACT_TANH: return tanhf(z);
        case WD_ACT_LEAKY_RELU: return z > 0.f ? z : 0.2f * z;
        case WD_ACT_ELU: return z > 0.f ? z : expm1f(z);
        case WD_ACT_SELU: return 1.0507009873554805f * (z > 0.f ? z : 1.6732632423543772f * expm1f(z));
        case WD_ACT_SOFTPLUS: return fmaxf(z, 0.f) + log1pf(expf(-fabsf(z)));
        case WD_ACT_SOFTSIGN: return z / (1.f + fabsf(z));
    }
    return z;
}
__device__ __forceinline__ float act_bwd(int kind, float a) {
    switch (kind) {
        case WD_ACT_RELU: return a > 0.f ? 1.f : 0.f;
        case WD_ACT_RELU6: return (a > 0.f && a < 6.f) ? 1.f : 0.f;
        case WD_ACT_SIGMOID: return a * (1.f - a);
        case WD_ACT_TANH: return 1.f - a * a;
        case WD_ACT_LEAKY_RELU: return a > 0.f ? 1.f : 0.2f;
        case WD_ACT_ELU: return a > 0.f ? 1.f : a + 1.f;
        case WD_ACT_SELU: return a > 0.f ? 1.0507009873554805f : a + 1.0507009873554805f * 1.6732632423543772f;
        case WD_ACT_SOFTPLUS: return 1.f - expf(-a);
        case WD_ACT_SOFTSIGN: { float t = 1.f - fabsf(a); return t * t; }
    }
    return 1.f;
}

struct GemmA {
    int n;
    const float* ptr[kMaxSegs];
    int ld[kMaxSegs];
    int k[kMaxSegs];
    const __nv_bfloat16* hi[kMaxSegs];
    const __nv_bfloat16* lo[kMaxSegs];
};
struct GemmB {
    const float* ptr; int ld;
    const float *tf32_hi, *tf32_lo;
    const __nv_bfloat16 *hi, *lo;
};
enum { EPI_FWD = 0, EPI_STORE = 1, EPI_WGRAD = 2 };
struct Epi {
    float* C; int ldc;
    int accumulate;
    float* A_out; float* H_out; int ldh;
    float* HT; int ldt;
    const float *bias, *gamma, *beta;
    int n_logical, act, bn;
    int m_valid;
    int64_t split_stride;
    __nv_bfloat16 *Hs_hi, *Hs_lo;
    uint64_t reserved[5];
};

int tc_gemm(WdModel* m, int mode, const GemmA& A, const GemmB& B, int M, int N, const Epi& ep, int splits, int ksplit_len);
int tc_gemm_bf16(WdModel* m, int mode, const GemmA& A, const GemmB& B, int M, int N, const Epi& ep, int splits, int ksplit_len);
int make_tensor_map(CUtensorMap* map, CUtensorMapDataType dtype, const void* ptr, int rows, int cols, int ld, int box_rows);

struct DropArgs { float rate; unsigned long long seed; const unsigned int* step; int layer_id; };
__device__ __forceinline__ unsigned long long splitmix64_dev(unsigned long long x) {
    x += 0x9E3779B97F4A7C15ULL;
    x = (x ^ (x >> 30)) * 0xBF58476D1CE4E5B9ULL;
    x = (x ^ (x >> 27)) * 0x94D049BB133111EBULL;
    return x ^ (x >> 31);
}
__device__ __forceinline__ unsigned long long drop_key(const DropArgs& d) {
    return splitmix64_dev(d.seed ^ ((unsigned long long)(*d.step) * 0x9E3779B97F4A7C15ULL) ^ ((unsigned long long)d.layer_id << 48));
}
__device__ __forceinline__ float drop_mult(unsigned long long key, unsigned int m, unsigned int n, float rate, float inv_keep) {
    const unsigned long long r = splitmix64_dev(key ^ ((unsigned long long)m * 65536ULL + n));
    const float u = (float)(unsigned int)(r >> 40) * (1.f / 16777216.f);
    return u >= rate ? inv_keep : 0.f;
}

__device__ __forceinline__ float bn_out(float a, const float* __restrict__ gamma, const float* __restrict__ beta, int n, int bn) {
    return bn ? fmaf(a, gamma[n] * 0.99950037468777f, beta[n]) : a;
}

__device__ __forceinline__ void split_bf16(float x, __nv_bfloat16& hi, __nv_bfloat16& lo) {
    hi = __float2bfloat16_rn(x);
    lo = __float2bfloat16_rn(x - __bfloat162float(hi));
}
__device__ __forceinline__ void split_pair(float x0, float x1, uint32_t& hi, uint32_t& lo) {
    const __nv_bfloat162 hp = __floats2bfloat162_rn(x0, x1);
    hi = *reinterpret_cast<const uint32_t*>(&hp);
    const __nv_bfloat162 lp = __floats2bfloat162_rn(x0 - __uint_as_float(hi << 16), x1 - __uint_as_float(hi & 0xFFFF0000u));
    lo = *reinterpret_cast<const uint32_t*>(&lp);
}
__device__ __forceinline__ void store_split4(__nv_bfloat16* hi, __nv_bfloat16* lo, float x0, float x1, float x2, float x3) {
    uint2 ph, pl;
    split_pair(x0, x1, ph.x, pl.x);
    split_pair(x2, x3, ph.y, pl.y);
    *reinterpret_cast<uint2*>(hi) = ph;
    *reinterpret_cast<uint2*>(lo) = pl;
}

}
```

wide_deep_b200/csrc/gemm_bf16.cu:

```cuda
#include <cuda.h>
#include <stdlib.h>

#include <algorithm>
#include <type_traits>

#include "common.cuh"
#include "gemm.cuh"
#include "wgmma_ptx.cuh"

namespace wd {

namespace {

constexpr int QBM = 128;
constexpr int QBN = 128;
constexpr int QNST = 3;
constexpr int QBK = 64;
constexpr int Q_THREADS = 384;

struct QMaps {
    CUtensorMap a_hi[kMaxSegs], a_lo[kMaxSegs];
    CUtensorMap b_hi, b_lo;
};
struct QSegs { int n; int k[kMaxSegs]; int koff[kMaxSegs]; };

__device__ unsigned long long g_probe[32 * 8];
__device__ __forceinline__ unsigned long long gtime() { unsigned long long t; asm volatile("mov.u64 %0, %globaltimer;" : "=l"(t)); return t; }
#define PROBE(i) do { if (probe >= 0 && blockIdx.x == 0 && (threadIdx.x & 127) == 0) g_probe[probe * 8 + (i)] = gtime(); } while (0)

template <int MODE>
__global__ void __launch_bounds__(Q_THREADS, 1) tc_gemm_bf16_kernel(const __grid_constant__ QMaps maps, const QSegs segs, int M, int N, int ktot,
                                                                   int ksplit_len, int nsplit, Epi ep, int probe) {
    extern __shared__ uint8_t smem_raw[];
    uint8_t* base = reinterpret_cast<uint8_t*>((reinterpret_cast<uintptr_t>(smem_raw) + 1023) & ~uintptr_t(1023));
    constexpr bool A_MN = MODE == EPI_WGRAD;
    constexpr bool B_MN = MODE == EPI_FWD || MODE == EPI_WGRAD;
    constexpr int A_BYTES = QBM * 128, B_BYTES = QBN * 128;
    constexpr int STAGE_BYTES = 2 * (A_BYTES + B_BYTES);
    auto a_hi = [&](int s) { return base + s * STAGE_BYTES; };
    auto a_lo = [&](int s) { return base + s * STAGE_BYTES + A_BYTES; };
    auto b_hi = [&](int s) { return base + s * STAGE_BYTES + 2 * A_BYTES; };
    auto b_lo = [&](int s) { return base + s * STAGE_BYTES + 2 * A_BYTES + B_BYTES; };
    uint64_t* bars = reinterpret_cast<uint64_t*>(base + QNST * STAGE_BYTES);
    uint64_t* full = bars; uint64_t* empty = bars + QNST;
    float* epi_vec = reinterpret_cast<float*>(base + QNST * STAGE_BYTES + 64);

    const int warp = threadIdx.x >> 5, lane = threadIdx.x & 31, wg = threadIdx.x >> 7;
    const int tiles_n = (N + QBN - 1) / QBN, tiles_m = (M + QBM - 1) / QBM;
    const int ntiles = tiles_n * tiles_m * nsplit;
    int nkb_all = 0;
    for (int s = 0; s < segs.n; ++s) nkb_all += (segs.k[s] + QBK - 1) / QBK;
    auto tile_range = [&](int tile, int& m0, int& n0, int& z, int& kbeg, int& nkb) {
        z = tile / (tiles_n * tiles_m);
        int r = tile % (tiles_n * tiles_m);
        m0 = (r / tiles_n) * QBM;
        n0 = (r % tiles_n) * QBN;
        kbeg = 0;
        nkb = nkb_all;
        if (MODE == EPI_WGRAD) {
            kbeg = z * ksplit_len;
            int kend = min(ktot, kbeg + ksplit_len);
            nkb = kend > kbeg ? (kend - kbeg + QBK - 1) / QBK : 0;
        }
    };

    if (threadIdx.x == 0) {
        for (int s = 0; s < QNST; ++s) { mbar_init(&full[s], 1); mbar_init(&empty[s], 8); }
        asm volatile("fence.mbarrier_init.release.cluster;" ::: "memory");
    }
    __syncthreads();

    if (wg == 0) {
        reg_dealloc<40>();
        PROBE(0);
        if (warp == 0 && lane == 0) {
            int g = 0;
            for (int tile = blockIdx.x; tile < ntiles; tile += gridDim.x) {
                int m0, n0, z, kbeg, nkb;
                tile_range(tile, m0, n0, z, kbeg, nkb);
                int seg = 0, kin = 0;
                for (int kb = 0; kb < nkb; ++kb, ++g) {
                    const int s = g % QNST, it = g / QNST;
                    if (it > 0) mbar_wait(&empty[s], (it - 1) & 1);
                    int ka, kbcoord;
                    if (MODE == EPI_WGRAD) { ka = kbeg + kb * QBK; kbcoord = ka; }
                    else {
                        if (kin >= segs.k[seg]) { ++seg; kin = 0; }
                        ka = kin; kbcoord = segs.koff[seg] + kin;
                        kin += QBK;
                    }
                    mbar_expect_tx(&full[s], 2 * (A_BYTES + B_BYTES));
                    if (!A_MN) {
                        tma_load_2d(a_hi(s), &maps.a_hi[seg], &full[s], ka, m0);
                        tma_load_2d(a_lo(s), &maps.a_lo[seg], &full[s], ka, m0);
                    } else {
#pragma unroll
                        for (int i = 0; i < QBM / 64; ++i) {
                            tma_load_2d(a_hi(s) + i * 8192, &maps.a_hi[seg], &full[s], m0 + 64 * i, ka);
                            tma_load_2d(a_lo(s) + i * 8192, &maps.a_lo[seg], &full[s], m0 + 64 * i, ka);
                        }
                    }
                    if (!B_MN) {
                        tma_load_2d(b_hi(s), &maps.b_hi, &full[s], kbcoord, n0);
                        tma_load_2d(b_lo(s), &maps.b_lo, &full[s], kbcoord, n0);
                    } else {
#pragma unroll
                        for (int i = 0; i < QBN / 64; ++i) {
                            tma_load_2d(b_hi(s) + i * 8192, &maps.b_hi, &full[s], n0 + 64 * i, kbcoord);
                            tma_load_2d(b_lo(s) + i * 8192, &maps.b_lo, &full[s], n0 + 64 * i, kbcoord);
                        }
                    }
                }
            }
        }
    } else {
        reg_alloc<232>();
        const int cw = wg - 1, cwarp = warp - 4;
        constexpr uint32_t a_step = A_MN ? 2048u : 32u, b_step = B_MN ? 2048u : 32u;
        constexpr int TA = A_MN ? 1 : 0, TB = B_MN ? 1 : 0;
        float d[QBN / 2];
        int g = 0, use = 0;
        for (int tile = blockIdx.x; tile < ntiles; tile += gridDim.x) {
            int m0, n0, z, kbeg, nkb;
            tile_range(tile, m0, n0, z, kbeg, nkb);
            if (nkb == 0) {
#pragma unroll
                for (int i = 0; i < QBN / 2; ++i) d[i] = 0.f;
            }
            const int ct = threadIdx.x - 128;
            float pre[2] = {0.f, 0.f};
            if (MODE == EPI_FWD) {
#pragma unroll
                for (int i = 0; i < 2; ++i) {
                    const int v = ct + 256 * i, c = n0 + (v & 127);
                    const bool in = c < ep.n_logical;
                    if (v < 128) pre[i] = in ? __ldg(ep.bias + c) : 0.f;
                    else if (v < 256) pre[i] = (in && ep.bn) ? __ldg(ep.gamma + c) * 0.99950037468777f : 1.f;
                    else if (v < 384) pre[i] = (in && ep.bn) ? __ldg(ep.beta + c) : 0.f;
                }
            }
            int prev = -1;
            for (int kb = 0; kb < nkb; ++kb, ++g) {
                const int s = g % QNST, it = g / QNST;
                mbar_wait(&full[s], it & 1);
                if (g == 0) PROBE(1);
                const uint32_t sa_hi = smem_u32(a_hi(s)) + cw * 8192, sa_lo = smem_u32(a_lo(s)) + cw * 8192;
                const uint32_t sb_hi = smem_u32(b_hi(s)), sb_lo = smem_u32(b_lo(s));
                wgmma_fence();
#pragma unroll
                for (int k = 0; k < QBK / 16; ++k) {
                    const uint64_t da_hi = A_MN ? make_desc_mn(sa_hi + k * a_step) : make_desc(sa_hi + k * a_step);
                    const uint64_t da_lo = A_MN ? make_desc_mn(sa_lo + k * a_step) : make_desc(sa_lo + k * a_step);
                    const uint64_t db_hi = B_MN ? make_desc_mn(sb_hi + k * b_step) : make_desc(sb_hi + k * b_step);
                    const uint64_t db_lo = B_MN ? make_desc_mn(sb_lo + k * b_step) : make_desc(sb_lo + k * b_step);
                    wgmma_bf16<TA, TB>(d, da_lo, db_hi, (kb > 0 || k > 0) ? 1u : 0u);
                    wgmma_bf16<TA, TB>(d, da_hi, db_lo, 1u);
                    wgmma_bf16<TA, TB>(d, da_hi, db_hi, 1u);
                }
                wgmma_commit();
                if (prev >= 0) {
                    wgmma_wait<1>();
                    if (lane == 0) mbar_arrive(&empty[prev]);
                }
                prev = s;
            }
            wgmma_wait<0>();
            if (prev >= 0 && lane == 0) mbar_arrive(&empty[prev]);
            if (cwarp == 0) PROBE(use == 0 ? 2 : 3);
            const float* ev = epi_vec + (use & 1) * 384;
            if (MODE == EPI_FWD) {
                epi_vec[(use & 1) * 384 + ct] = pre[0];
                if (ct < 128) epi_vec[(use & 1) * 384 + ct + 256] = pre[1];
                bar_sync(1, 256);
            }

            const int r0 = m0 + cw * 64 + (warp & 3) * 16 + (lane >> 2);
            const int cq = 2 * (lane & 3);
            auto epilogue = [&](auto relu) {
                constexpr bool RELU = decltype(relu)::value;
                uint32_t qh[2][2] = {}, ql[2][2] = {};
#pragma unroll
                for (int j = 0; j < QBN / 8; ++j) {
                    const int c = n0 + 8 * j + cq;
                    if (n0 + 8 * j < N) {
                        if (MODE == EPI_FWD) {
                            const bool in0 = c < ep.n_logical, in1 = c + 1 < ep.n_logical;
                            const int cl = 8 * j + cq;
                            const float b0 = ev[cl], b1 = ev[cl + 1], g0 = ev[128 + cl], g1 = ev[129 + cl], e0 = ev[256 + cl], e1 = ev[257 + cl];
#pragma unroll
                            for (int hh = 0; hh < 2; ++hh) {
                                const int r = r0 + 8 * hh;
                                if (r >= M) continue;
                                const bool rv = r < ep.m_valid;
                                float a0 = 0.f, a1 = 0.f, h0 = 0.f, h1 = 0.f;
                                if (rv && in0) { a0 = RELU ? fmaxf(d[4 * j + 2 * hh] + b0, 0.f) : act_fwd(ep.act, d[4 * j + 2 * hh] + b0); h0 = fmaf(a0, g0, e0); }
                                if (rv && in1) { a1 = RELU ? fmaxf(d[4 * j + 2 * hh + 1] + b1, 0.f) : act_fwd(ep.act, d[4 * j + 2 * hh + 1] + b1); h1 = fmaf(a1, g1, e1); }
                                const int64_t o = (int64_t)r * ep.ldh + c;
                                if (ep.A_out != ep.H_out) *reinterpret_cast<float2*>(ep.A_out + o) = make_float2(a0, a1);
                                if (ep.H_out) *reinterpret_cast<float2*>(ep.H_out + o) = make_float2(h0, h1);
                                split_pair(h0, h1, qh[j & 1][hh], ql[j & 1][hh]);
                            }
                            if (j & 1) {
                                const int q = lane & 3, src = (lane & ~3) + 2 * (q & 1);
                                const int64_t cp = n0 + 16 * (j >> 1) + 4 * q;
#pragma unroll
                                for (int hh = 0; hh < 2; ++hh) {
                                    uint2 vh, vl;
                                    const uint32_t h0a = __shfl_sync(0xffffffffu, qh[0][hh], src), h1a = __shfl_sync(0xffffffffu, qh[1][hh], src);
                                    const uint32_t h0b = __shfl_sync(0xffffffffu, qh[0][hh], src + 1), h1b = __shfl_sync(0xffffffffu, qh[1][hh], src + 1);
                                    const uint32_t l0a = __shfl_sync(0xffffffffu, ql[0][hh], src), l1a = __shfl_sync(0xffffffffu, ql[1][hh], src);
                                    const uint32_t l0b = __shfl_sync(0xffffffffu, ql[0][hh], src + 1), l1b = __shfl_sync(0xffffffffu, ql[1][hh], src + 1);
                                    vh.x = q < 2 ? h0a : h1a; vh.y = q < 2 ? h0b : h1b;
                                    vl.x = q < 2 ? l0a : l1a; vl.y = q < 2 ? l0b : l1b;
                                    const int r = r0 + 8 * hh;
                                    if (r >= M) continue;
                                    const int64_t o = (int64_t)r * ep.ldh + cp;
                                    *reinterpret_cast<uint2*>(ep.Hs_hi + o) = vh;
                                    *reinterpret_cast<uint2*>(ep.Hs_lo + o) = vl;
                                }
                            }
                        } else {
                            float* Cb = ep.C + (MODE == EPI_WGRAD ? (int64_t)z * ep.split_stride : 0);
#pragma unroll
                            for (int hh = 0; hh < 2; ++hh) {
                                const int r = r0 + 8 * hh;
                                if (r >= M) continue;
                                float2* pc = reinterpret_cast<float2*>(Cb + (int64_t)r * ep.ldc + c);
                                float2 o = make_float2(d[4 * j + 2 * hh], d[4 * j + 2 * hh + 1]);
                                if (MODE == EPI_STORE && ep.accumulate) { const float2 p = *pc; o.x += p.x; o.y += p.y; }
                                *pc = o;
                            }
                        }
                    }
                }
            };
            if (MODE == EPI_FWD && ep.act == WD_ACT_RELU) epilogue(std::true_type{});
            else epilogue(std::false_type{});
            if (cwarp == 0) PROBE(use == 0 ? 4 : 5);
            ++use;
        }
    }
}

int g_probe_slot = 0;

template <int MODE>
int launch_q(WdModel* m, const QMaps& maps, const QSegs& segs, int M, int N, int ktot, int splits, int ksplit_len, const Epi& ep) {
    constexpr int smem = QNST * 2 * (QBM * 128 + QBN * 128) + 1024 + 64 + 2 * 384 * 4;
    static bool configured = false;
    static int num_sms = 0;
    if (!configured) {
        WD_CUDA(cudaFuncSetAttribute(tc_gemm_bf16_kernel<MODE>, cudaFuncAttributeMaxDynamicSharedMemorySize, smem));
        WD_CUDA(cudaDeviceGetAttribute(&num_sms, cudaDevAttrMultiProcessorCount, m->device));
        configured = true;
    }
    const int nsplit = MODE == EPI_WGRAD ? splits : 1;
    const int ntiles = ((N + QBN - 1) / QBN) * ((M + QBM - 1) / QBM) * nsplit;
    static const bool probe_on = getenv("WD_GEMM_PROBE") != nullptr;
    const int probe = probe_on ? (g_probe_slot++ & 31) : -1;
    tc_gemm_bf16_kernel<MODE><<<ntiles < num_sms ? ntiles : num_sms, Q_THREADS, smem, m->stream>>>(maps, segs, M, N, ktot, ksplit_len, nsplit, ep, probe);
    m->launches++;
    WD_CUDA(cudaGetLastError());
    return WD_OK;
}

}

extern "C" int wd_debug_gemm_probe(unsigned long long* out) {
    cudaDeviceSynchronize();
    cudaError_t e = cudaMemcpyFromSymbol(out, g_probe, sizeof(unsigned long long) * 32 * 8);
    g_probe_slot = 0;
    return e == cudaSuccess ? 0 : -1;
}

int tc_gemm_bf16(WdModel* m, int mode, const GemmA& A, const GemmB& B, int M, int N, const Epi& ep, int splits, int ksplit_len) {
    constexpr CUtensorMapDataType BF16 = CU_TENSOR_MAP_DATA_TYPE_BFLOAT16;
    if (N % 32 != 0 || A.n > kMaxSegs || !B.hi || !B.lo) { set_error("bf16 GEMM engine: unsupported operands"); return WD_EUNSUPPORTED; }
    QMaps maps;
    QSegs segs{};
    segs.n = A.n;
    int rc, ktot = 0;
    const bool a_mn = mode == EPI_WGRAD, b_mn = mode == EPI_FWD || mode == EPI_WGRAD;
    for (int s = 0; s < A.n; ++s) {
        if (!A.hi[s] || !A.lo[s]) { set_error("bf16 GEMM engine: operand without hi/lo copies"); return WD_EINVAL; }
        if (!a_mn) {
            if ((rc = make_tensor_map(&maps.a_hi[s], BF16, A.hi[s], M, A.k[s], A.ld[s], QBM))) return rc;
            if ((rc = make_tensor_map(&maps.a_lo[s], BF16, A.lo[s], M, A.k[s], A.ld[s], QBM))) return rc;
        } else {
            if ((rc = make_tensor_map(&maps.a_hi[s], BF16, A.hi[s], A.k[s], M, A.ld[s], 64))) return rc;
            if ((rc = make_tensor_map(&maps.a_lo[s], BF16, A.lo[s], A.k[s], M, A.ld[s], 64))) return rc;
        }
        segs.k[s] = A.k[s]; segs.koff[s] = ktot;
        ktot += A.k[s];
    }
    for (int s = A.n; s < kMaxSegs; ++s) { maps.a_hi[s] = maps.a_hi[0]; maps.a_lo[s] = maps.a_lo[0]; }
    if (!b_mn) {
        if ((rc = make_tensor_map(&maps.b_hi, BF16, B.hi, N, ktot, B.ld, QBN))) return rc;
        if ((rc = make_tensor_map(&maps.b_lo, BF16, B.lo, N, ktot, B.ld, QBN))) return rc;
    } else {
        if ((rc = make_tensor_map(&maps.b_hi, BF16, B.hi, ktot, N, B.ld, 64))) return rc;
        if ((rc = make_tensor_map(&maps.b_lo, BF16, B.lo, ktot, N, B.ld, 64))) return rc;
    }
    if (mode == EPI_WGRAD) ksplit_len = (ksplit_len + QBK - 1) / QBK * QBK;
    if (mode == EPI_FWD && (!ep.Hs_hi || !ep.Hs_lo)) { set_error("bf16 GEMM engine: epilogue without hi/lo outputs"); return WD_EINVAL; }
    if (mode == EPI_FWD) return launch_q<EPI_FWD>(m, maps, segs, M, N, ktot, splits, ksplit_len, ep);
    if (mode == EPI_STORE) return launch_q<EPI_STORE>(m, maps, segs, M, N, ktot, splits, ksplit_len, ep);
    return launch_q<EPI_WGRAD>(m, maps, segs, M, N, ktot, splits, ksplit_len, ep);
}

}
```

wide_deep_b200/csrc/mlp.cu:

```cuda
#include "common.cuh"
#include "gemm.cuh"

namespace wd {

constexpr int BM = 128, BN = 128, BK = 16, GT = 256;

template <int MODE>
__global__ void __launch_bounds__(GT) gemm_tn_ffma(GemmA A, const float* __restrict__ Bm, int ldb, int M, int N, int ksplit_len, Epi ep) {
    __shared__ __align__(16) float As[2][BK][BM + 4];
    __shared__ __align__(16) float Bs[2][BK][BN + 4];
    const int tid = threadIdx.x, tx = tid & 15, ty = tid >> 4;
    const int m0 = blockIdx.y * BM, n0 = blockIdx.x * BN;
    float acc[8][8];
#pragma unroll
    for (int i = 0; i < 8; ++i)
#pragma unroll
        for (int j = 0; j < 8; ++j) acc[i][j] = 0.f;

    int ktot = 0;
    for (int s = 0; s < A.n; ++s) ktot += A.k[s];
    int kbeg = 0, kend = ktot;
    if (MODE == EPI_WGRAD) {
        kbeg = blockIdx.z * ksplit_len;
        kend = min(ktot, kbeg + ksplit_len);
    }
    const int lrow = tid >> 2, lkc = tid & 3;
    float4 ra[2], rb[2];

    auto gload = [&](int kg) {
        int s = 0, kk = kg;
        while (s < A.n - 1 && kk >= A.k[s]) { kk -= A.k[s]; ++s; }
        const float* ap = A.ptr[s];
        const int lda = A.ld[s];
#pragma unroll
        for (int p = 0; p < 2; ++p) {
            int r = lrow + p * 64;
            int gm = m0 + r, gn = n0 + r;
            ra[p] = (gm < M) ? *reinterpret_cast<const float4*>(ap + (int64_t)gm * lda + kk + lkc * 4) : make_float4(0, 0, 0, 0);
            rb[p] = (gn < N) ? *reinterpret_cast<const float4*>(Bm + (int64_t)gn * ldb + kg + lkc * 4) : make_float4(0, 0, 0, 0);
        }
    };
    auto sstore = [&](int buf) {
#pragma unroll
        for (int p = 0; p < 2; ++p) {
            int r = lrow + p * 64;
            As[buf][lkc * 4 + 0][r] = ra[p].x; As[buf][lkc * 4 + 1][r] = ra[p].y;
            As[buf][lkc * 4 + 2][r] = ra[p].z; As[buf][lkc * 4 + 3][r] = ra[p].w;
            Bs[buf][lkc * 4 + 0][r] = rb[p].x; Bs[buf][lkc * 4 + 1][r] = rb[p].y;
            Bs[buf][lkc * 4 + 2][r] = rb[p].z; Bs[buf][lkc * 4 + 3][r] = rb[p].w;
        }
    };

    int buf = 0;
    if (kbeg < kend) {
        gload(kbeg);
        sstore(0);
    }
    __syncthreads();
    for (int kg = kbeg; kg < kend; kg += BK) {
        bool more = kg + BK < kend;
        if (more) gload(kg + BK);
#pragma unroll
        for (int k = 0; k < BK; ++k) {
            float4 a0 = *reinterpret_cast<const float4*>(&As[buf][k][ty * 4]);
            float4 a1 = *reinterpret_cast<const float4*>(&As[buf][k][64 + ty * 4]);
            float4 b0 = *reinterpret_cast<const float4*>(&Bs[buf][k][tx * 4]);
            float4 b1 = *reinterpret_cast<const float4*>(&Bs[buf][k][64 + tx * 4]);
            float av[8] = {a0.x, a0.y, a0.z, a0.w, a1.x, a1.y, a1.z, a1.w};
            float bv[8] = {b0.x, b0.y, b0.z, b0.w, b1.x, b1.y, b1.z, b1.w};
#pragma unroll
            for (int i = 0; i < 8; ++i)
#pragma unroll
                for (int j = 0; j < 8; ++j) acc[i][j] = fmaf(av[i], bv[j], acc[i][j]);
        }
        if (more) sstore(buf ^ 1);
        __syncthreads();
        buf ^= 1;
    }

#pragma unroll
    for (int ih = 0; ih < 2; ++ih) {
#pragma unroll
        for (int jh = 0; jh < 2; ++jh) {
            const int mb = m0 + ih * 64 + ty * 4, nb = n0 + jh * 64 + tx * 4;
            if (nb >= N) continue;
            if (MODE == EPI_FWD) {
                float hv[4][4];
#pragma unroll
                for (int i = 0; i < 4; ++i) {
                    const int gm = mb + i;
                    float a4[4];
#pragma unroll
                    for (int j = 0; j < 4; ++j) {
                        const int gn = nb + j;
                        float a = 0.f, h = 0.f;
                        if (gn < ep.n_logical && gm < ep.m_valid) {
                            a = act_fwd(ep.act, acc[ih * 4 + i][jh * 4 + j] + ep.bias[gn]);
                            h = bn_out(a, ep.gamma, ep.beta, gn, ep.bn);
                        }
                        a4[j] = a;
                        hv[i][j] = h;
                    }
                    if (gm < M) {
                        if (ep.A_out != ep.H_out)
                            *reinterpret_cast<float4*>(ep.A_out + (int64_t)gm * ep.ldh + nb) = make_float4(a4[0], a4[1], a4[2], a4[3]);
                        *reinterpret_cast<float4*>(ep.H_out + (int64_t)gm * ep.ldh + nb) = make_float4(hv[i][0], hv[i][1], hv[i][2], hv[i][3]);
                    }
                }
                if (ep.HT) {
#pragma unroll
                    for (int j = 0; j < 4; ++j)
                        *reinterpret_cast<float4*>(ep.HT + (int64_t)(nb + j) * ep.ldt + mb) = make_float4(hv[0][j], hv[1][j], hv[2][j], hv[3][j]);
                }
            } else {
                float* Cb = ep.C + (MODE == EPI_WGRAD ? (int64_t)blockIdx.z * ep.split_stride : 0);
#pragma unroll
                for (int i = 0; i < 4; ++i) {
                    const int gm = mb + i;
                    if (gm >= M) continue;
                    float4 v = make_float4(acc[ih * 4 + i][jh * 4 + 0], acc[ih * 4 + i][jh * 4 + 1], acc[ih * 4 + i][jh * 4 + 2], acc[ih * 4 + i][jh * 4 + 3]);
                    float4* dst = reinterpret_cast<float4*>(Cb + (int64_t)gm * ep.ldc + nb);
                    if (MODE == EPI_STORE && ep.accumulate) {
                        float4 o = *dst;
                        v.x += o.x; v.y += o.y; v.z += o.z; v.w += o.w;
                    }
                    *dst = v;
                }
            }
        }
    }
}

static void launch_gemm(WdModel* m, int mode, const GemmA& A, const GemmB& B, int M, int N, const Epi& ep, int splits, int ksplit_len) {
    dim3 grid((N + BN - 1) / BN, (M + BM - 1) / BM, mode == EPI_WGRAD ? splits : 1);
    if (mode == EPI_FWD) gemm_tn_ffma<EPI_FWD><<<grid, GT, 0, m->stream>>>(A, B.ptr, B.ld, M, N, 0, ep);
    else if (mode == EPI_STORE) gemm_tn_ffma<EPI_STORE><<<grid, GT, 0, m->stream>>>(A, B.ptr, B.ld, M, N, 0, ep);
    else gemm_tn_ffma<EPI_WGRAD><<<grid, GT, 0, m->stream>>>(A, B.ptr, B.ld, M, N, ksplit_len, ep);
    m->launches++;
}

static int run_gemm(WdModel* m, int mode, const GemmA& A, const GemmB& B, int M, int N, const Epi& ep, int splits = 1, int ksplit_len = 0) {
    static const char* kNamesL[3][4] = {{"gemm_fwd_l0", "gemm_fwd_l1", "gemm_fwd_l2", "gemm_fwd_l3+"},
                                        {"gemm_dgrad_l0", "gemm_dgrad_l1", "gemm_dgrad_l2", "gemm_dgrad_l3+"},
                                        {"gemm_wgrad_l0", "gemm_wgrad_l1", "gemm_wgrad_l2", "gemm_wgrad_l3+"}};
    const char* kNames[3] = {kNamesL[0][m->cur_layer < 3 ? m->cur_layer : 3], kNamesL[1][m->cur_layer < 3 ? m->cur_layer : 3],
                             kNamesL[2][m->cur_layer < 3 ? m->cur_layer : 3]};
    mark(m, "mlp_other");
    if (m->operands == kBf16Operands) {
        int rc = tc_gemm_bf16(m, mode, A, B, M, N, ep, splits, ksplit_len);
        mark(m, kNames[mode]);
        return rc;
    }
    if (m->gemm_engine == WD_GEMM_TC3X || m->gemm_engine == WD_GEMM_TC1X) {
        int rc = tc_gemm(m, mode, A, B, M, N, ep, splits, ksplit_len);
        if (rc != WD_EUNSUPPORTED) { mark(m, kNames[mode]); return rc; }
        m->gemm_fallbacks++;
        static bool warned = false;
        if (!warned) { fprintf(stderr, "libwd_b200: wgmma engine does not cover a GEMM (M=%d N=%d segs=%d): running it on the FFMA kernel\n", M, N, A.n); warned = true; }
    }
    launch_gemm(m, mode, A, B, M, N, ep, splits, ksplit_len);
    mark(m, kNames[mode]);
    return WD_OK;
}

__global__ void transpose_kernel(const float* __restrict__ in, int ld_in, int M, int Mpad, int N, float* __restrict__ out, int ld_out) {
    __shared__ float t[32][33];
    int m0 = blockIdx.y * 32, n0 = blockIdx.x * 32;
    for (int i = threadIdx.y; i < 32; i += 8) {
        int mm = m0 + i, nn = n0 + threadIdx.x;
        t[i][threadIdx.x] = (mm < M && nn < N) ? in[(int64_t)mm * ld_in + nn] : 0.f;
    }
    __syncthreads();
    for (int i = threadIdx.y; i < 32; i += 8) {
        int nn = n0 + i, mm = m0 + threadIdx.x;
        if (nn < N && mm < Mpad) out[(int64_t)nn * ld_out + mm] = t[threadIdx.x][i];
    }
}

__global__ void x0_split_kernel(const float* __restrict__ in, int64_t n4, __nv_bfloat16* __restrict__ hi, __nv_bfloat16* __restrict__ lo) {
    for (int64_t i = (int64_t)blockIdx.x * blockDim.x + threadIdx.x; i < n4; i += (int64_t)gridDim.x * blockDim.x) {
        const float4 x = reinterpret_cast<const float4*>(in)[i];
        store_split4(hi + 4 * i, lo + 4 * i, x.x, x.y, x.z, x.w);
    }
}

__global__ void __launch_bounds__(256) dropout_fwd_kernel(int B, int N, int n_logical, const float* __restrict__ A, int ld,
                                                         const float* __restrict__ gamma, const float* __restrict__ beta, int bn,
                                                         float* __restrict__ H, __nv_bfloat16* __restrict__ q_hi, __nv_bfloat16* __restrict__ q_lo,
                                                         float* __restrict__ HT, int ldt, DropArgs dr) {
    const unsigned long long key = drop_key(dr);
    const float inv_keep = 1.f / (1.f - dr.rate);
    const int64_t total = (int64_t)B * N;
    for (int64_t t = (int64_t)blockIdx.x * blockDim.x + threadIdx.x; t < total; t += (int64_t)gridDim.x * blockDim.x) {
        const int mrow = (int)(t / N), n = (int)(t % N);
        float h = 0.f;
        if (n < n_logical) {
            const float a = A[(int64_t)mrow * ld + n] * drop_mult(key, (unsigned)mrow, (unsigned)n, dr.rate, inv_keep);
            h = bn_out(a, gamma, beta, n, bn);
        }
        if (H) H[(int64_t)mrow * ld + n] = h;
        if (q_hi) {
            __nv_bfloat16 hh, hl;
            split_bf16(h, hh, hl);
            q_hi[(int64_t)mrow * ld + n] = hh; q_lo[(int64_t)mrow * ld + n] = hl;
        }
        if (HT) HT[(int64_t)n * ldt + mrow] = h;
    }
}

struct GemvSegs { int n; const float* ptr[kMaxSegs]; int ld[kMaxSegs]; int k[kMaxSegs]; int koff[kMaxSegs]; };

struct HeadIn { int n; GemvSegs S[kMaxTowers]; const float* kernel[kMaxTowers]; const float* bias[kMaxTowers]; float* tower_logit[kMaxTowers]; };
__global__ void __launch_bounds__(256) logits_head_kernel(HeadIn in, int B, const float* __restrict__ wide_logit, const float* __restrict__ label,
                                                        const float* __restrict__ weight, float* __restrict__ logits, float* __restrict__ dlogit,
                                                        float* __restrict__ loss_part, int32_t* __restrict__ counter, float* __restrict__ loss_out) {
    __shared__ float red[8];
    __shared__ bool is_last;
    const int warp = (blockIdx.x * blockDim.x + threadIdx.x) >> 5, lane = threadIdx.x & 31, lig = lane & 7, grp = lane >> 3;
    const int nw = (gridDim.x * blockDim.x) >> 5;
    float lsum = 0.f;
    for (int b0 = warp * 4; b0 < B; b0 += nw * 4) {
        const int b = b0 + grp;
        const bool live = b < B;
        float x = (live && wide_logit) ? wide_logit[b] : 0.f;
        for (int t = 0; t < in.n; ++t) {
            const GemvSegs& S = in.S[t];
            float acc = 0.f;
            if (live) {
                for (int s = 0; s < S.n; ++s) {
                    const float* row = S.ptr[s] + (int64_t)b * S.ld[s];
                    const float* kw = in.kernel[t] + S.koff[s];
                    const int K = S.k[s];
                    int k = lig * 4;
                    for (; k + 96 < K; k += 128) {
                        float4 xv[4], w[4];
#pragma unroll
                        for (int u = 0; u < 4; ++u) { xv[u] = *reinterpret_cast<const float4*>(row + k + 32 * u); w[u] = *reinterpret_cast<const float4*>(kw + k + 32 * u); }
#pragma unroll
                        for (int u = 0; u < 4; ++u) {
                            acc = fmaf(xv[u].x, w[u].x, acc); acc = fmaf(xv[u].y, w[u].y, acc); acc = fmaf(xv[u].z, w[u].z, acc); acc = fmaf(xv[u].w, w[u].w, acc);
                        }
                    }
                    for (; k < K; k += 32) {
                        const float4 xv = *reinterpret_cast<const float4*>(row + k);
                        const float4 w = *reinterpret_cast<const float4*>(kw + k);
                        acc = fmaf(xv.x, w.x, acc); acc = fmaf(xv.y, w.y, acc); acc = fmaf(xv.z, w.z, acc); acc = fmaf(xv.w, w.w, acc);
                    }
                }
            }
#pragma unroll
            for (int d = 4; d > 0; d >>= 1) acc += __shfl_xor_sync(0xffffffffu, acc, d);
            const float tl = acc + in.bias[t][0];
            if (lig == 0 && live) in.tower_logit[t][b] = tl;
            x += tl;
        }
        if (lig == 0 && live) {
            logits[b] = x;
            if (label) {
                const float y = label[b], w = weight ? weight[b] : 1.f;
                lsum += w * (fmaxf(x, 0.f) - x * y + log1pf(expf(-fabsf(x))));
                if (dlogit) dlogit[b] = (1.f / (1.f + expf(-x)) - y) * w;
            }
        }
    }
    lsum += __shfl_xor_sync(0xffffffffu, lsum, 8);
    lsum += __shfl_xor_sync(0xffffffffu, lsum, 16);
    if (lane == 0) red[threadIdx.x >> 5] = lsum;
    __syncthreads();
    if (threadIdx.x == 0) {
        float s = 0.f;
        for (int i = 0; i < 8; ++i) s += red[i];
        loss_part[blockIdx.x] = s;
        __threadfence();
        is_last = atomicAdd(counter, 1) == (int)gridDim.x - 1;
    }
    __syncthreads();
    if (is_last) {
        __shared__ double dred[256];
        __threadfence();
        const int nb = (int)gridDim.x;
        double s = 0.0;
        for (int i = threadIdx.x; i < nb; i += 256) s += (double)__ldcg(loss_part + i);
        dred[threadIdx.x] = s;
        __syncthreads();
        for (int d = 128; d > 0; d >>= 1) {
            if ((int)threadIdx.x < d) dred[threadIdx.x] += dred[threadIdx.x + d];
            __syncthreads();
        }
        if (threadIdx.x == 0) { *loss_out = (float)dred[0]; *counter = 0; }
    }
}

__global__ void __launch_bounds__(256) logits_bwd_kernel(int B, int K, const float* __restrict__ src, int ld, const float* __restrict__ dlogit,
                                                        const float* __restrict__ kw, float* __restrict__ gpart, int64_t gstride,
                                                        float* __restrict__ bias_part, int64_t bias_stride, float* __restrict__ wide_bias_part,
                                                        int64_t wide_bias_stride, float* __restrict__ dst, int dld, int accumulate) {
    __shared__ float red[4][64];
    __shared__ float dl[128];
    const int rt = blockIdx.y, kx = threadIdx.x & 63, ry = threadIdx.x >> 6;
    const int k = blockIdx.x * 64 + kx;
    const int b0 = rt * 128;
    if (threadIdx.x < 128) dl[threadIdx.x] = (b0 + threadIdx.x < B) ? dlogit[b0 + threadIdx.x] : 0.f;
    __syncthreads();
    float acc = 0.f;
    if (k < K) {
        const int r0 = b0 + ry * 32;
        const float w = dst ? kw[k] : 0.f;
#pragma unroll 8
        for (int i = 0; i < 32; ++i)
            if (r0 + i < B) {
                const float g = dl[ry * 32 + i];
                acc = fmaf(src[(int64_t)(r0 + i) * ld + k], g, acc);
                if (dst) {
                    float* d = dst + (int64_t)(r0 + i) * dld + k;
                    *d = accumulate ? *d + g * w : g * w;
                }
            }
    }
    red[ry][kx] = acc;
    __syncthreads();
    if (ry == 0 && k < K) gpart[(int64_t)rt * gstride + k] = red[0][kx] + red[1][kx] + red[2][kx] + red[3][kx];
    if (blockIdx.x == 0 && threadIdx.x == 0 && (bias_part || wide_bias_part)) {
        float s = 0.f;
        for (int i = 0; i < 128; ++i) s += dl[i];
        if (bias_part) bias_part[(int64_t)rt * bias_stride] = s;
        if (wide_bias_part) wide_bias_part[(int64_t)rt * wide_bias_stride] = s;
    }
}

__global__ void __launch_bounds__(256) act_bn_bwd_kernel(int B, int N, int n_logical, const float* __restrict__ dH, const float* __restrict__ Aact,
                                                        int ld, const float* __restrict__ gamma, int act, int bn,
                                                        float* __restrict__ dZ, float* __restrict__ dZT, int ldt,
                                                        float* __restrict__ p_bias, float* __restrict__ p_gamma, float* __restrict__ p_beta,
                                                        int64_t pstride, DropArgs dr) {
    __shared__ float tile[32][33];
    const unsigned long long dkey = dr.rate > 0.f ? drop_key(dr) : 0ull;
    const float inv_keep = dr.rate > 0.f ? 1.f / (1.f - dr.rate) : 1.f;
    __shared__ float red[3][8][32];
    const int tx = threadIdx.x & 31, ty = threadIdx.x >> 5;
    const int n = blockIdx.x * 32 + tx, rt = blockIdx.y;
    const float inv = 0.99950037468777f;
    float sb = 0.f, sg = 0.f, sbe = 0.f;
    const float gsc = (bn && n < n_logical) ? gamma[n] * inv : 1.f;
    for (int sub = 0; sub < 4; ++sub) {
        const int mbase = rt * 128 + sub * 32;
#pragma unroll
        for (int i = 0; i < 4; ++i) {
            int mm = mbase + ty * 4 + i;
            float dz = 0.f;
            if (mm < B && n < n_logical) {
                float dh = dH[(int64_t)mm * ld + n], a = Aact[(int64_t)mm * ld + n];
                const float dm = dr.rate > 0.f ? drop_mult(dkey, (unsigned)mm, (unsigned)n, dr.rate, inv_keep) : 1.f;
                dz = dh * gsc * dm * act_bwd(act, a);
                sb += dz; sg += dh * (a * dm) * inv; sbe += dh;
            }
            if (mm < B && n < N) dZ[(int64_t)mm * ld + n] = dz;
            tile[ty * 4 + i][tx] = dz;
        }
        __syncthreads();
#pragma unroll
        for (int i = 0; i < 4; ++i) {
            int nn = blockIdx.x * 32 + ty * 4 + i;
            if (nn < N) dZT[(int64_t)nn * ldt + mbase + tx] = tile[tx][ty * 4 + i];
        }
        __syncthreads();
    }
    red[0][ty][tx] = sb; red[1][ty][tx] = sg; red[2][ty][tx] = sbe;
    __syncthreads();
    if (ty == 0 && n < N) {
        float a = 0.f, b = 0.f, c = 0.f;
        for (int i = 0; i < 8; ++i) { a += red[0][i][tx]; b += red[1][i][tx]; c += red[2][i][tx]; }
        p_bias[(int64_t)rt * pstride + n] = a;
        if (bn) { p_gamma[(int64_t)rt * pstride + n] = b; p_beta[(int64_t)rt * pstride + n] = c; }
    }
}

__global__ void __launch_bounds__(256) act_bn_bwd_q_kernel(int B, int N, int n_logical, const float* __restrict__ dH, const float* __restrict__ Aact,
                                                          int ld, const float* __restrict__ gamma, int act, int bn,
                                                          float* __restrict__ p_bias, float* __restrict__ p_gamma, float* __restrict__ p_beta,
                                                          int64_t pstride, __nv_bfloat16* __restrict__ q_hi, __nv_bfloat16* __restrict__ q_lo, DropArgs dr) {
    __shared__ float red[3][16][64];
    const unsigned long long dkey = dr.rate > 0.f ? drop_key(dr) : 0ull;
    const float inv_keep = dr.rate > 0.f ? 1.f / (1.f - dr.rate) : 1.f;
    const int cx = threadIdx.x & 15, ry = threadIdx.x >> 4;
    const int n0 = blockIdx.x * 64 + cx * 4, rt = blockIdx.y, b0 = rt * 128;
    const float inv = 0.99950037468777f;
    float gsc[4], sb[4] = {0.f, 0.f, 0.f, 0.f}, sg[4] = {0.f, 0.f, 0.f, 0.f}, sbe[4] = {0.f, 0.f, 0.f, 0.f};
#pragma unroll
    for (int j = 0; j < 4; ++j) gsc[j] = (bn && n0 + j < n_logical) ? gamma[n0 + j] * inv : 1.f;
    if (n0 < N) {
        float4 dhv[8], av[8];
#pragma unroll
        for (int u = 0; u < 8; ++u) {
            const int mr = min(b0 + u * 16 + ry, B - 1);
            dhv[u] = *reinterpret_cast<const float4*>(dH + (int64_t)mr * ld + n0);
            av[u] = *reinterpret_cast<const float4*>(Aact + (int64_t)mr * ld + n0);
        }
#pragma unroll
        for (int u = 0; u < 8; ++u) {
            const int mm = b0 + u * 16 + ry;
            if (mm >= B) continue;
            const float dh[4] = {dhv[u].x, dhv[u].y, dhv[u].z, dhv[u].w}, a[4] = {av[u].x, av[u].y, av[u].z, av[u].w};
            float dz[4];
#pragma unroll
            for (int j = 0; j < 4; ++j) {
                dz[j] = 0.f;
                if (n0 + j < n_logical) {
                    const float dm = dr.rate > 0.f ? drop_mult(dkey, (unsigned)mm, (unsigned)(n0 + j), dr.rate, inv_keep) : 1.f;
                    dz[j] = dh[j] * gsc[j] * dm * act_bwd(act, a[j]);
                    sb[j] += dz[j]; sg[j] += dh[j] * (a[j] * dm) * inv; sbe[j] += dh[j];
                }
            }
            store_split4(q_hi + (int64_t)mm * ld + n0, q_lo + (int64_t)mm * ld + n0, dz[0], dz[1], dz[2], dz[3]);
        }
    }
#pragma unroll
    for (int j = 0; j < 4; ++j) { red[0][ry][cx * 4 + j] = sb[j]; red[1][ry][cx * 4 + j] = sg[j]; red[2][ry][cx * 4 + j] = sbe[j]; }
    __syncthreads();
    if (threadIdx.x < 192) {
        const int which = threadIdx.x >> 6, c = threadIdx.x & 63, n = blockIdx.x * 64 + c;
        if (n < N && (which == 0 || bn)) {
            float x = 0.f;
#pragma unroll
            for (int i = 0; i < 16; ++i) x += red[which][i][c];
            (which == 0 ? p_bias : which == 1 ? p_gamma : p_beta)[(int64_t)rt * pstride + n] = x;
        }
    }
}

__global__ void __launch_bounds__(256) logits_act_bwd_q_kernel(int B, int N, int n_logical, const float* __restrict__ H, int ldh,
                                                              const float* __restrict__ Aact, int ld, const float* __restrict__ dlogit,
                                                              const float* __restrict__ kw, const float* __restrict__ gamma, int act, int bn,
                                                              float* __restrict__ p_kw, int64_t kw_stride, float* __restrict__ p_lbias, int64_t lbias_stride,
                                                              float* __restrict__ p_wbias, int64_t wbias_stride,
                                                              float* __restrict__ p_bias, float* __restrict__ p_gamma, float* __restrict__ p_beta, int64_t pstride,
                                                              __nv_bfloat16* __restrict__ q_hi, __nv_bfloat16* __restrict__ q_lo) {
    __shared__ float red[4][16][64];
    __shared__ float dl[128];
    const int cx = threadIdx.x & 15, ry = threadIdx.x >> 4;
    const int n0 = blockIdx.x * 64 + cx * 4, rt = blockIdx.y, b0 = rt * 128;
    const float inv = 0.99950037468777f;
    if (threadIdx.x < 128) dl[threadIdx.x] = (b0 + threadIdx.x < B) ? dlogit[b0 + threadIdx.x] : 0.f;
    float gsc[4], w[4], sk[4] = {0.f, 0.f, 0.f, 0.f}, sb[4] = {0.f, 0.f, 0.f, 0.f}, sg[4] = {0.f, 0.f, 0.f, 0.f}, sbe[4] = {0.f, 0.f, 0.f, 0.f};
#pragma unroll
    for (int j = 0; j < 4; ++j) {
        gsc[j] = (bn && n0 + j < n_logical) ? gamma[n0 + j] * inv : 1.f;
        w[j] = n0 + j < N ? kw[n0 + j] : 0.f;
    }
    __syncthreads();
    if (n0 < N) {
        float4 hv[8], av[8];
#pragma unroll
        for (int u = 0; u < 8; ++u) {
            const int mr = min(b0 + u * 16 + ry, B - 1);
            hv[u] = *reinterpret_cast<const float4*>(H + (int64_t)mr * ldh + n0);
            av[u] = *reinterpret_cast<const float4*>(Aact + (int64_t)mr * ld + n0);
        }
#pragma unroll
        for (int u = 0; u < 8; ++u) {
            const int mm = b0 + u * 16 + ry;
            if (mm >= B) continue;
            const float g = dl[u * 16 + ry];
            const float h[4] = {hv[u].x, hv[u].y, hv[u].z, hv[u].w}, a[4] = {av[u].x, av[u].y, av[u].z, av[u].w};
            float dz[4];
#pragma unroll
            for (int j = 0; j < 4; ++j) {
                sk[j] = fmaf(h[j], g, sk[j]);
                dz[j] = 0.f;
                if (n0 + j < n_logical) {
                    const float dh = g * w[j];
                    dz[j] = dh * gsc[j] * act_bwd(act, a[j]);
                    sb[j] += dz[j]; sg[j] += dh * a[j] * inv; sbe[j] += dh;
                }
            }
            store_split4(q_hi + (int64_t)mm * ld + n0, q_lo + (int64_t)mm * ld + n0, dz[0], dz[1], dz[2], dz[3]);
        }
    }
#pragma unroll
    for (int j = 0; j < 4; ++j) { red[0][ry][cx * 4 + j] = sk[j]; red[1][ry][cx * 4 + j] = sb[j]; red[2][ry][cx * 4 + j] = sg[j]; red[3][ry][cx * 4 + j] = sbe[j]; }
    __syncthreads();
    {
        const int which = threadIdx.x >> 6, c = threadIdx.x & 63, n = blockIdx.x * 64 + c;
        if (n < N) {
            float x = 0.f;
#pragma unroll
            for (int i = 0; i < 16; ++i) x += red[which][i][c];
            if (which == 0) p_kw[(int64_t)rt * kw_stride + n] = x;
            else if (which == 1) p_bias[(int64_t)rt * pstride + n] = x;
            else if (bn) (which == 2 ? p_gamma : p_beta)[(int64_t)rt * pstride + n] = x;
        }
    }
    if (blockIdx.x == 0 && threadIdx.x == 0 && (p_lbias || p_wbias)) {
        float s = 0.f;
        for (int i = 0; i < 128; ++i) s += dl[i];
        if (p_lbias) p_lbias[(int64_t)rt * lbias_stride] = s;
        if (p_wbias) p_wbias[(int64_t)rt * wbias_stride] = s;
    }
}

__global__ void rowtile_sum_kernel(int B, const float* __restrict__ v, float* __restrict__ part, int64_t stride) {
    int rt = blockIdx.x;
    int b0 = rt * 128, b1 = min(B, b0 + 128);
    float s = 0.f;
    for (int b = b0 + threadIdx.x; b < b1; b += 32) s += v[b];
#pragma unroll
    for (int d = 16; d > 0; d >>= 1) s += __shfl_xor_sync(0xffffffffu, s, d);
    if (threadIdx.x == 0) part[(int64_t)rt * stride] = s;
}
int wide_bias_grad(WdModel* m) {
    if (!m->use_wide) return WD_OK;
    if (m->use_deep && !m->towers.empty()) return WD_OK;
    const int rts = (m->dbatch.B + 127) / 128;
    rowtile_sum_kernel<<<rts, 32, 0, m->stream>>>(m->dbatch.B, m->d_dlogit, m->d_gpart + m->dense[0].gpart_off, m->dense[0].gstride);
    m->launches++;
    WD_CUDA(cudaGetLastError());
    return WD_OK;
}

__global__ void dense_reduce_kernel(const DenseTensor* __restrict__ T, int nt, int64_t total, const float* __restrict__ gpart,
                                    float* __restrict__ G, int live_row_tiles) {
    for (int64_t i = (int64_t)blockIdx.x * blockDim.x + threadIdx.x; i < total; i += (int64_t)gridDim.x * blockDim.x) {
        int lo = 0, hi = nt - 1;
        while (lo < hi) {
            int mid = (lo + hi + 1) >> 1;
            if (T[mid].off <= i) lo = mid; else hi = mid - 1;
        }
        const DenseTensor t = T[lo];
        if (i - t.off >= t.count) { G[i] = 0.f; continue; }
        int parts = t.g_rowtiles ? live_row_tiles : t.gparts;
        float s = 0.f;
        const float* p = gpart + t.gpart_off + (i - t.off);
        for (int q = 0; q < parts; ++q) s += p[(int64_t)q * t.gstride];
        G[i] = s;
    }
}

struct OptParamsD { int kind; float lr, l1, l2, beta1, beta2, epsilon, rho, momentum; const float* bpow; };
static OptParamsD make_opt_d(const WdOptimizer& o, const float* bpow) {
    return OptParamsD{o.kind, o.lr, o.l1, o.l2, o.beta1, o.beta2, o.epsilon, o.rho, o.momentum, bpow};
}
__device__ __forceinline__ void opt_update_d(const OptParamsD& o, float g, float& w, float& s1, float& s2) {
    if (o.kind == WD_OPT_ADAGRAD) {
        s1 += g * g;
        w -= o.lr * g / sqrtf(s1);
    } else if (o.kind == WD_OPT_FTRL) {
        float n1 = s1 + g * g;
        float z1 = s2 + g - (sqrtf(n1) - sqrtf(s1)) / o.lr * w;
        float wn = 0.f;
        if (fabsf(z1) > o.l1) wn = (copysignf(o.l1, z1) - z1) / (sqrtf(n1) / o.lr + 2.f * o.l2);
        w = wn; s1 = n1; s2 = z1;
    } else if (o.kind == WD_OPT_ADAM) {
        const float lr_t = o.lr * sqrtf(1.f - o.bpow[1]) / (1.f - o.bpow[0]);
        s1 += (g - s1) * (1.f - o.beta1);
        s2 += (g * g - s2) * (1.f - o.beta2);
        w -= lr_t * s1 / (sqrtf(s2) + o.epsilon);
    } else if (o.kind == WD_OPT_RMSPROP) {
        s1 += (g * g - s1) * (1.f - o.rho);
        s2 = s2 * o.momentum + (g * o.lr) / sqrtf(s1 + o.epsilon);
        w -= s2;
    } else {
        w -= o.lr * g;
    }
}
__device__ __forceinline__ void store_split(float* __restrict__ W_hi, float* __restrict__ W_lo, float* __restrict__ Wt_hi,
                                            float* __restrict__ Wt_lo, int64_t e, int64_t et, float w) {
    float hi = __uint_as_float(__float_as_uint(w) & 0xFFFFE000u), lo = w - hi;
    W_hi[e] = hi;
    W_lo[e] = lo;
    Wt_hi[et] = hi;
    Wt_lo[et] = lo;
}
__global__ void dense_apply_kernel(const DenseTensor* __restrict__ T, int nt, int64_t total, const float* __restrict__ G,
                                   float* __restrict__ P, float* __restrict__ S1, float* __restrict__ S2, float* __restrict__ Wt,
                                   float* __restrict__ W_hi, float* __restrict__ W_lo, float* __restrict__ Wt_hi, float* __restrict__ Wt_lo,
                                   OptParamsD dnn, OptParamsD lin, int lin_tensor) {
    for (int64_t i = (int64_t)blockIdx.x * blockDim.x + threadIdx.x; i < total; i += (int64_t)gridDim.x * blockDim.x) {
        int lo = 0, hi = nt - 1;
        while (lo < hi) {
            int mid = (lo + hi + 1) >> 1;
            if (T[mid].off <= i) lo = mid; else hi = mid - 1;
        }
        const DenseTensor t = T[lo];
        if (i - t.off >= t.count) continue;
        float w = P[i], s1 = S1[i], s2 = S2[i];
        opt_update_d(lo == lin_tensor ? lin : dnn, G[i], w, s1, s2);
        P[i] = w; S1[i] = s1; S2[i] = s2;
        if (t.wt_off >= 0) {
            int64_t e = i - t.off;
            int k = (int)(e / t.cols), n = (int)(e % t.cols);
            Wt[t.wt_off + (int64_t)n * t.rows + k] = w;
            store_split(W_hi, W_lo, Wt_hi, Wt_lo, t.wt_off + e, t.wt_off + (int64_t)n * t.rows + k, w);
        }
    }
}
template <int MODE>
__global__ void __launch_bounds__(256) dense_vec_kernel(const DenseTensor* __restrict__ T, int nt, int64_t total4, const float* __restrict__ gpart,
                                                        float* __restrict__ G, float* __restrict__ P, float* __restrict__ S1, float* __restrict__ S2,
                                                        __nv_bfloat16* __restrict__ Wq_hi, __nv_bfloat16* __restrict__ Wq_lo, OptParamsD dnn, OptParamsD lin, int lin_tensor,
                                                        int live_row_tiles, int64_t begin4, int64_t hole_lo4, int64_t hole_hi4) {
    for (int64_t i4 = begin4 + (int64_t)blockIdx.x * blockDim.x + threadIdx.x; i4 < total4; i4 += (int64_t)gridDim.x * blockDim.x) {
        if (i4 >= hole_lo4 && i4 < hole_hi4) continue;
        const int64_t i = i4 * 4;
        int lo = 0, hi = nt - 1;
        while (lo < hi) {
            int mid = (lo + hi + 1) >> 1;
            if (T[mid].off <= i) lo = mid; else hi = mid - 1;
        }
        const DenseTensor t = T[lo];
        const int64_t e = i - t.off;
        if (e >= t.count) {
            if (MODE == 0) reinterpret_cast<float4*>(G)[i4] = make_float4(0.f, 0.f, 0.f, 0.f);
            continue;
        }
        float4 g;
        if (MODE != 1) {
            const int parts = t.g_rowtiles ? live_row_tiles : t.gparts;
            const float* p = gpart + t.gpart_off + e;
            g = make_float4(0.f, 0.f, 0.f, 0.f);
            int q = 0;
            for (; q + 4 <= parts; q += 4) {
                const float4 v0 = *reinterpret_cast<const float4*>(p + (int64_t)q * t.gstride);
                const float4 v1 = *reinterpret_cast<const float4*>(p + (int64_t)(q + 1) * t.gstride);
                const float4 v2 = *reinterpret_cast<const float4*>(p + (int64_t)(q + 2) * t.gstride);
                const float4 v3 = *reinterpret_cast<const float4*>(p + (int64_t)(q + 3) * t.gstride);
                g.x += v0.x; g.y += v0.y; g.z += v0.z; g.w += v0.w;
                g.x += v1.x; g.y += v1.y; g.z += v1.z; g.w += v1.w;
                g.x += v2.x; g.y += v2.y; g.z += v2.z; g.w += v2.w;
                g.x += v3.x; g.y += v3.y; g.z += v3.z; g.w += v3.w;
            }
            for (; q < parts; ++q) {
                const float4 v = *reinterpret_cast<const float4*>(p + (int64_t)q * t.gstride);
                g.x += v.x; g.y += v.y; g.z += v.z; g.w += v.w;
            }
            if (e + 1 >= t.count) g.y = 0.f;
            if (e + 2 >= t.count) g.z = 0.f;
            if (e + 3 >= t.count) g.w = 0.f;
            if (MODE == 0) { reinterpret_cast<float4*>(G)[i4] = g; continue; }
        } else {
            g = reinterpret_cast<const float4*>(G)[i4];
        }
        const OptParamsD o = lo == lin_tensor ? lin : dnn;
        float4 w = reinterpret_cast<float4*>(P)[i4], s1 = reinterpret_cast<float4*>(S1)[i4], s2 = reinterpret_cast<float4*>(S2)[i4];
        opt_update_d(o, g.x, w.x, s1.x, s2.x);
        if (e + 1 < t.count) opt_update_d(o, g.y, w.y, s1.y, s2.y);
        if (e + 2 < t.count) opt_update_d(o, g.z, w.z, s1.z, s2.z);
        if (e + 3 < t.count) opt_update_d(o, g.w, w.w, s1.w, s2.w);
        reinterpret_cast<float4*>(P)[i4] = w;
        reinterpret_cast<float4*>(S1)[i4] = s1;
        reinterpret_cast<float4*>(S2)[i4] = s2;
        if (t.wt_off >= 0)
            store_split4(Wq_hi + t.wt_off + e, Wq_lo + t.wt_off + e, w.x, w.y, w.z, w.w);
    }
}

__global__ void weight_copies_kernel(const DenseTensor* __restrict__ T, int nt, int64_t total, const float* __restrict__ P, float* __restrict__ Wt,
                                     float* __restrict__ W_hi, float* __restrict__ W_lo, float* __restrict__ Wt_hi, float* __restrict__ Wt_lo,
                                     __nv_bfloat16* __restrict__ Wq_hi, __nv_bfloat16* __restrict__ Wq_lo) {
    for (int64_t i = (int64_t)blockIdx.x * blockDim.x + threadIdx.x; i < total; i += (int64_t)gridDim.x * blockDim.x) {
        int lo = 0, hi = nt - 1;
        while (lo < hi) {
            int mid = (lo + hi + 1) >> 1;
            if (T[mid].off <= i) lo = mid; else hi = mid - 1;
        }
        const DenseTensor t = T[lo];
        if (t.wt_off >= 0 && i - t.off < t.count) {
            int64_t e = i - t.off;
            if (Wq_hi) {
                __nv_bfloat16 qh, ql;
                split_bf16(P[i], qh, ql);
                Wq_hi[t.wt_off + e] = qh;
                Wq_lo[t.wt_off + e] = ql;
                continue;
            }
            int k = (int)(e / t.cols), n = (int)(e % t.cols);
            Wt[t.wt_off + (int64_t)n * t.rows + k] = P[i];
            store_split(W_hi, W_lo, Wt_hi, Wt_lo, t.wt_off + e, t.wt_off + (int64_t)n * t.rows + k, P[i]);
        }
    }
}
int refresh_weight_copies(WdModel* m) {
    if (m->dense_count == 0) return WD_OK;
    weight_copies_kernel<<<grid_for(m->dense_count, 256), 256, 0, m->stream>>>(m->d_dense_desc, (int)m->dense.size(), m->dense_count, m->d_P, m->d_Wt,
                                                                               m->d_W_hi, m->d_W_lo, m->d_Wt_hi, m->d_Wt_lo, m->d_Wq_hi, m->d_Wq_lo);
    m->launches++;
    WD_CUDA(cudaGetLastError());
    return WD_OK;
}

static const float* src_ptr(WdModel* m, Tower& tw, int src) { return src < 0 ? m->d_X0 : tw.layers[src].H; }
static const __nv_bfloat16* src_split(WdModel* m, Tower& tw, int src, int part) { return src < 0 ? m->d_X0s[part] : tw.layers[src].Hs[part]; }
static int src_ld(WdModel* m, Tower& tw, int src) { return src < 0 ? m->d0_phys : tw.layers[src].N_phys; }

static void fwd_operands(WdModel* m, Tower& tw, const Layer& L, GemmA& A, GemmB& B) {
    const int64_t wo = m->dense[L.t_kernel].wt_off;
    A.n = L.n_in_segs;
    for (int s = 0; s < L.n_in_segs; ++s) {
        const int src = L.segs[s].src;
        A.ld[s] = src_ld(m, tw, src); A.k[s] = L.segs[s].width_phys;
        if (m->operands == kFp32Operands) A.ptr[s] = src_ptr(m, tw, src);
        else { A.hi[s] = src_split(m, tw, src, 0); A.lo[s] = src_split(m, tw, src, 1); }
    }
    if (m->operands == kFp32Operands) B = GemmB{m->d_Wt + wo, L.K_phys, m->d_Wt_hi + wo, m->d_Wt_lo + wo, nullptr, nullptr};
    else B = GemmB{nullptr, L.N_phys, nullptr, nullptr, m->d_Wq_hi + wo, m->d_Wq_lo + wo};
}
static void dgrad_operands(WdModel* m, const Layer& L, const Seg& sg, GemmA& A, GemmB& B) {
    const DenseTensor& tk = m->dense[L.t_kernel];
    const int64_t eo = (int64_t)sg.k_off * L.N_phys, wo = tk.wt_off + eo;
    A.n = 1; A.ld[0] = L.N_phys; A.k[0] = L.N_phys;
    if (m->operands == kFp32Operands) {
        A.ptr[0] = L.dZ;
        B = GemmB{m->d_P + tk.off + eo, L.N_phys, m->d_W_hi + wo, m->d_W_lo + wo, nullptr, nullptr};
    } else {
        A.hi[0] = L.dZs[0]; A.lo[0] = L.dZs[1];
        B = GemmB{nullptr, L.N_phys, nullptr, nullptr, m->d_Wq_hi + wo, m->d_Wq_lo + wo};
    }
}
static void wgrad_operands(WdModel* m, Tower& tw, const Layer& L, const Seg& sg, GemmA& A, GemmB& B) {
    A.n = 1;
    if (m->operands == kFp32Operands) {
        A.ptr[0] = sg.src < 0 ? m->d_X0T : tw.layers[sg.src].HT; A.ld[0] = m->ldt; A.k[0] = (m->dbatch.B + 15) / 16 * 16;
        B = GemmB{L.dZT, m->ldt, nullptr, nullptr, nullptr, nullptr};
    } else {
        A.hi[0] = src_split(m, tw, sg.src, 0); A.lo[0] = src_split(m, tw, sg.src, 1); A.ld[0] = src_ld(m, tw, sg.src); A.k[0] = m->dbatch.B;
        B = GemmB{nullptr, L.N_phys, nullptr, nullptr, L.dZs[0], L.dZs[1]};
    }
}

int mlp_forward(WdModel* m, bool train) {
    const int B = m->dbatch.B;
    if (!m->use_deep) return WD_OK;
    if (m->operands == kBf16Operands) {
        const int64_t n4 = (int64_t)B * m->d0_phys / 4;
        x0_split_kernel<<<grid_for(n4, 256), 256, 0, m->stream>>>(m->d_X0, n4, m->d_X0s[0], m->d_X0s[1]);
        m->launches++;
    } else if (train) {
        int Bp = (B + 127) / 128 * 128;
        dim3 g((m->d0_phys + 31) / 32, (Bp + 31) / 32);
        transpose_kernel<<<g, dim3(32, 8), 0, m->stream>>>(m->d_X0, m->d0_phys, B, Bp, m->d0_phys, m->d_X0T, m->ldt);
        m->launches++;
    }
    for (auto& tw : m->towers) {
        for (int l = 0; l < tw.n_hidden; ++l) {
            Layer& L = tw.layers[l];
            m->cur_layer = l;
            GemmA A{}; GemmB W{};
            fwd_operands(m, tw, L, A, W);
            Epi ep{};
            ep.A_out = L.A; ep.H_out = L.H; ep.ldh = L.N_phys;
            ep.HT = train ? L.HT : nullptr; ep.ldt = m->ldt;
            ep.Hs_hi = L.Hs[0]; ep.Hs_lo = L.Hs[1];
            ep.bias = m->d_P + m->dense[L.t_bias].off;
            ep.gamma = L.t_gamma >= 0 ? m->d_P + m->dense[L.t_gamma].off : nullptr;
            ep.beta = L.t_beta >= 0 ? m->d_P + m->dense[L.t_beta].off : nullptr;
            ep.n_logical = L.N; ep.act = m->activation; ep.bn = m->batch_norm; ep.m_valid = B;
            int rc = run_gemm(m, EPI_FWD, A, W, B, L.N_phys, ep);
            if (rc) return rc;
            if (train && m->dropout_rate > 0.f) {
                const DropArgs dr{m->dropout_rate, m->dropout_seed, m->d_step, (int)(&tw - &m->towers[0]) * 64 + l};
                dropout_fwd_kernel<<<grid_for((int64_t)B * L.N_phys, 256), 256, 0, m->stream>>>(B, L.N_phys, L.N, L.A, L.N_phys, ep.gamma, ep.beta, m->batch_norm,
                    L.H, L.Hs[0], L.Hs[1], ep.HT, m->ldt, dr);
                m->launches++;
            }
        }
    }
    WD_CUDA(cudaGetLastError());
    return WD_OK;
}

int loss_forward(WdModel* m, bool need_grad) {
    const int B = m->dbatch.B;
    const int ntow = m->use_deep ? (int)m->towers.size() : 0;
    HeadIn in{};
    in.n = ntow;
    for (int t = 0; t < ntow; ++t) {
        Tower& tw = m->towers[t];
        Layer& LL = tw.layers[tw.n_hidden];
        in.S[t].n = LL.n_in_segs;
        for (int s = 0; s < LL.n_in_segs; ++s) {
            in.S[t].ptr[s] = src_ptr(m, tw, LL.segs[s].src);
            in.S[t].ld[s] = src_ld(m, tw, LL.segs[s].src);
            in.S[t].k[s] = LL.segs[s].width_phys;
            in.S[t].koff[s] = LL.segs[s].k_off;
        }
        in.kernel[t] = m->d_P + m->dense[LL.t_kernel].off;
        in.bias[t] = m->d_P + m->dense[LL.t_bias].off;
        in.tower_logit[t] = tw.logit;
    }
    const int blocks = grid_for((int64_t)B * 8, 256, 512);
    logits_head_kernel<<<blocks, 256, 0, m->stream>>>(in, B, m->use_wide ? m->d_wide_logit : nullptr, m->dbatch.label,
                                                     m->dbatch.weight, m->d_logits, need_grad ? m->d_dlogit : nullptr, m->d_loss_part,
                                                     m->d_head_counter, m->d_loss);
    m->launches++;
    WD_CUDA(cudaGetLastError());
    return WD_OK;
}

int mlp_backward(WdModel* m) {
    const int B = m->dbatch.B;
    if (!m->use_deep) return WD_OK;
    const int rts = (B + 127) / 128;
    const int Bk = (B + 15) / 16 * 16;
    bool dx0_written = false;
    const bool need_dx0 = !m->tables.empty();
    const bool bf16_ops = m->operands == kBf16Operands;
    for (auto& tw : m->towers) {
        std::vector<char> written(tw.n_hidden, 0);
        std::vector<int> readers(tw.n_hidden, 0);
        std::vector<char> fused(tw.n_hidden, 0);
        for (int l = 0; l <= tw.n_hidden; ++l)
            for (int s = 0; s < tw.layers[l].n_in_segs; ++s)
                if (tw.layers[l].segs[s].src >= 0) readers[tw.layers[l].segs[s].src] += (l == tw.n_hidden ? 2 : 1);
        auto grad_dst = [&](int src, float** p, int* ld, int* acc) {
            if (src < 0) { *p = m->d_dX0; *ld = m->d0_phys; *acc = dx0_written ? 1 : 0; dx0_written = true; }
            else { *p = tw.layers[src].dH; *ld = tw.layers[src].N_phys; *acc = written[src] ? 1 : 0; written[src] = 1; }
        };
        Layer& LL = tw.layers[tw.n_hidden];
        const DenseTensor& tk = m->dense[LL.t_kernel];
        const DenseTensor& tb = m->dense[LL.t_bias];
        for (int s = 0; s < LL.n_in_segs; ++s) {
            const Seg& sg = LL.segs[s];
            const float* src = src_ptr(m, tw, sg.src);
            int ld = src_ld(m, tw, sg.src);
            dim3 g((sg.width_phys + 63) / 64, rts);
            float* dst = nullptr; int dld = 0, acc = 0;
            if (!(sg.src < 0 && !need_dx0)) grad_dst(sg.src, &dst, &dld, &acc);
            const bool wb = m->use_wide && s == 0 && &tw == &m->towers.front();
            if (bf16_ops && LL.n_in_segs == 1 && sg.src >= 0 && readers[sg.src] == 2 && m->dropout_rate <= 0.f &&
                sg.width_phys == tw.layers[sg.src].N_phys) {
                Layer& S = tw.layers[sg.src];
                logits_act_bwd_q_kernel<<<dim3((S.N_phys + 63) / 64, rts), 256, 0, m->stream>>>(B, S.N_phys, S.N, src, ld, S.A, S.N_phys, m->d_dlogit,
                    m->d_P + tk.off + sg.k_off, S.t_gamma >= 0 ? m->d_P + m->dense[S.t_gamma].off : nullptr, m->activation, m->batch_norm,
                    m->d_gpart + tk.gpart_off + sg.k_off, tk.gstride, m->d_gpart + tb.gpart_off, tb.gstride,
                    wb ? m->d_gpart + m->dense[0].gpart_off : nullptr, wb ? m->dense[0].gstride : 0,
                    m->d_gpart + m->dense[S.t_bias].gpart_off, S.t_gamma >= 0 ? m->d_gpart + m->dense[S.t_gamma].gpart_off : nullptr,
                    S.t_beta >= 0 ? m->d_gpart + m->dense[S.t_beta].gpart_off : nullptr, m->dense[S.t_bias].gstride, S.dZs[0], S.dZs[1]);
                m->launches++;
                fused[sg.src] = 1;
                continue;
            }
            logits_bwd_kernel<<<g, 256, 0, m->stream>>>(B, sg.width_phys, src, ld, m->d_dlogit, m->d_P + tk.off + sg.k_off,
                                                       m->d_gpart + tk.gpart_off + sg.k_off, tk.gstride,
                                                       s == 0 ? m->d_gpart + tb.gpart_off : nullptr, tb.gstride,
                                                       wb ? m->d_gpart + m->dense[0].gpart_off : nullptr, wb ? m->dense[0].gstride : 0, dst, dld, acc);
            m->launches++;
        }
        for (int l = tw.n_hidden - 1; l >= 0; --l) {
            Layer& L = tw.layers[l];
            m->cur_layer = l;
            float* pb = m->d_gpart + m->dense[L.t_bias].gpart_off;
            float* pg = L.t_gamma >= 0 ? m->d_gpart + m->dense[L.t_gamma].gpart_off : nullptr;
            float* pbe = L.t_beta >= 0 ? m->d_gpart + m->dense[L.t_beta].gpart_off : nullptr;
            if (!written[l] && !fused[l]) {
                WD_CUDA(cudaMemsetAsync(L.dH, 0, (size_t)m->max_batch_pad * L.N_phys * sizeof(float), m->stream));
            }
            dim3 g((L.N_phys + 31) / 32, rts);
            const DropArgs dr{m->dropout_rate, m->dropout_seed, m->d_step, (int)(&tw - &m->towers[0]) * 64 + l};
            if (fused[l]) {
            } else if (bf16_ops)
                act_bn_bwd_q_kernel<<<dim3((L.N_phys + 63) / 64, rts), 256, 0, m->stream>>>(B, L.N_phys, L.N, L.dH, L.A, L.N_phys,
                    L.t_gamma >= 0 ? m->d_P + m->dense[L.t_gamma].off : nullptr, m->activation, m->batch_norm, pb, pg, pbe,
                    m->dense[L.t_bias].gstride, L.dZs[0], L.dZs[1], dr);
            else
            act_bn_bwd_kernel<<<g, 256, 0, m->stream>>>(B, L.N_phys, L.N, L.dH, L.A, L.N_phys,
                                                       L.t_gamma >= 0 ? m->d_P + m->dense[L.t_gamma].off : nullptr, m->activation,
                                                       m->batch_norm, L.dZ, L.dZT, m->ldt, pb, pg, pbe, m->dense[L.t_bias].gstride, dr);
            if (!fused[l]) m->launches++;
            for (int s = 0; s < L.n_in_segs; ++s) {
                const Seg& sg = L.segs[s];
                if (sg.src < 0 && !need_dx0) continue;
                float* dst; int dld, acc;
                grad_dst(sg.src, &dst, &dld, &acc);
                GemmA A{}; GemmB W{};
                dgrad_operands(m, L, sg, A, W);
                Epi ep{};
                ep.C = dst; ep.ldc = dld; ep.accumulate = acc;
                int rc = run_gemm(m, EPI_STORE, A, W, B, sg.width_phys, ep);
                if (rc) return rc;
            }
            if (l == 0 && &tw == &m->towers.back() && need_dx0 && m->ev_dx0 && m->record_dx0) {
                WD_CUDA(cudaEventRecord(m->ev_dx0, m->stream));
                m->dx0_recorded = true;
            }
        }
        for (int l = tw.n_hidden - 1; l >= 0; --l) {
            Layer& L = tw.layers[l];
            m->cur_layer = l;
            const DenseTensor& tkn = m->dense[L.t_kernel];
            if (l == 0 && m->record_wgrad_rest && m->towers.size() == 1 && L.n_in_segs == 1) {
                WD_CUDA(cudaEventRecord(m->ev_wgrad_rest, m->stream));
                m->dense_split_tensor = L.t_kernel;
            }
            for (int s = 0; s < L.n_in_segs; ++s) {
                const Seg& sg = L.segs[s];
                GemmA A{}; GemmB W{};
                wgrad_operands(m, tw, L, sg, A, W);
                Epi ep{};
                ep.C = m->d_gpart + tkn.gpart_off + (int64_t)sg.k_off * L.N_phys; ep.ldc = L.N_phys; ep.split_stride = tkn.gstride;
                const int ks = ((Bk + L.wgrad_splits - 1) / L.wgrad_splits + 31) / 32 * 32;
                int rc = run_gemm(m, EPI_WGRAD, A, W, sg.width_phys, L.N_phys, ep, L.wgrad_splits, ks);
                if (rc) return rc;
            }
        }
    }
    WD_CUDA(cudaGetLastError());
    return WD_OK;
}

__global__ void crelu_fold_kernel(float* __restrict__ gp, int parts, int64_t gstride, int rows, int cols, int u) {
    const int64_t total = (int64_t)parts * rows * u;
    for (int64_t i = (int64_t)blockIdx.x * blockDim.x + threadIdx.x; i < total; i += (int64_t)gridDim.x * blockDim.x) {
        const int n = (int)(i % u);
        const int64_t pr = i / u;
        float* q = gp + (pr / rows) * gstride + (pr % rows) * cols + n;
        q[0] -= q[u];
        q[u] = 0.f;
    }
}
__global__ void crelu_mirror_kernel(float* __restrict__ P, float* __restrict__ S1, float* __restrict__ S2, int rows, int cols, int u) {
    const int64_t total = (int64_t)rows * u;
    for (int64_t i = (int64_t)blockIdx.x * blockDim.x + threadIdx.x; i < total; i += (int64_t)gridDim.x * blockDim.x) {
        const int64_t e = (i / u) * cols + i % u;
        P[e + u] = -P[e];
        S1[e + u] = S1[e];
        S2[e + u] = S2[e];
    }
}
static int crelu_fold(WdModel* m) {
    const int rts = (m->dbatch.B + 127) / 128;
    for (const DenseTensor& t : m->dense) {
        if (!t.mirror_u) continue;
        const int parts = t.g_rowtiles ? rts : t.gparts;
        crelu_fold_kernel<<<grid_for((int64_t)parts * t.rows * t.mirror_u, 256), 256, 0, m->stream>>>(m->d_gpart + t.gpart_off, parts, t.gstride, t.rows, t.cols,
                                                                                                    t.mirror_u);
        m->launches++;
    }
    WD_CUDA(cudaGetLastError());
    return WD_OK;
}
static int crelu_mirror(WdModel* m) {
    for (const DenseTensor& t : m->dense) {
        if (!t.mirror_u) continue;
        crelu_mirror_kernel<<<grid_for((int64_t)t.rows * t.mirror_u, 256), 256, 0, m->stream>>>(m->d_P + t.off, m->d_S1 + t.off, m->d_S2 + t.off, t.rows, t.cols,
                                                                                              t.mirror_u);
        m->launches++;
    }
    WD_CUDA(cudaGetLastError());
    return refresh_weight_copies(m);
}

int dense_reduce_grads(WdModel* m) {
    if (m->dense_count == 0) return WD_OK;
    const int rts = (m->dbatch.B + 127) / 128;
    if (m->crelu) { int rc = crelu_fold(m); if (rc) return rc; }
    if (m->operands == kBf16Operands) {
        if (m->fuse_dense) return WD_OK;
        OptParamsD z{};
        dense_vec_kernel<0><<<grid_for(m->dense_count / 4, 256), 256, 0, m->stream>>>(m->d_dense_desc, (int)m->dense.size(), m->dense_count / 4, m->d_gpart,
            m->d_G, nullptr, nullptr, nullptr, nullptr, nullptr, z, z, -1, rts, 0, 0, 0);
        m->launches++;
        WD_CUDA(cudaGetLastError());
        return WD_OK;
    }
    dense_reduce_kernel<<<grid_for(m->dense_count, 256), 256, 0, m->stream>>>(m->d_dense_desc, (int)m->dense.size(), m->dense_count,
                                                                             m->d_gpart, m->d_G, rts);
    m->launches++;
    WD_CUDA(cudaGetLastError());
    return WD_OK;
}

static int dense_apply_plain(WdModel* m) {
    if (m->dense_count == 0) return WD_OK;
    OptParamsD d = make_opt_d(m->dnn_opt, m->d_bpow + 2);
    OptParamsD l = make_opt_d(m->lin_opt, m->d_bpow);
    int lin_tensor = m->use_wide ? 0 : -1;
    if (m->operands == kBf16Operands) {
        const int rts = (m->dbatch.B + 127) / 128;
        const int g = grid_for(m->dense_count / 4, 256);
        if (m->fuse_dense) {
            int64_t b4 = 0, e4 = m->dense_count / 4, hlo = 0, hhi = 0;
            if (m->dense_part && m->dense_split_tensor >= 0) {
                const DenseTensor& t = m->dense[m->dense_split_tensor];
                const int64_t k0 = t.off / 4, k1 = (t.off + t.count + 3) / 4;
                if (m->dense_part == 1) { b4 = k0; e4 = k1; } else { hlo = k0; hhi = k1; }
            }
            dense_vec_kernel<2><<<grid_for(e4 - b4, 256), 256, 0, m->stream>>>(m->d_dense_desc, (int)m->dense.size(), e4, m->d_gpart, m->d_G, m->d_P,
                                                                                m->d_S1, m->d_S2, m->d_Wq_hi, m->d_Wq_lo, d, l, lin_tensor, rts, b4, hlo, hhi);
        } else
            dense_vec_kernel<1><<<g, 256, 0, m->stream>>>(m->d_dense_desc, (int)m->dense.size(), m->dense_count / 4, m->d_gpart, m->d_G, m->d_P, m->d_S1,
                                                          m->d_S2, m->d_Wq_hi, m->d_Wq_lo, d, l, lin_tensor, rts, 0, 0, 0);
        m->launches++;
        WD_CUDA(cudaGetLastError());
        return WD_OK;
    }
    dense_apply_kernel<<<grid_for(m->dense_count, 256), 256, 0, m->stream>>>(m->d_dense_desc, (int)m->dense.size(), m->dense_count, m->d_G,
                                                                            m->d_P, m->d_S1, m->d_S2, m->d_Wt, m->d_W_hi, m->d_W_lo, m->d_Wt_hi,
                                                                            m->d_Wt_lo, d, l, lin_tensor);
    m->launches++;
    WD_CUDA(cudaGetLastError());
    return WD_OK;
}

int dense_apply(WdModel* m) {
    int rc = dense_apply_plain(m);
    if (!rc && m->crelu && m->dense_count > 0) rc = crelu_mirror(m);
    return rc;
}

}
```

Before: 10.48 million.

## Batch dgrad and wgrad GEMMs into grouped persistent launches with tile schedules

The backward dgrad GEMMs of each layer, and all wgrad GEMMs across layers, are now collected and run as one grouped bf16x3 kernel per group. A host-built, cached tile schedule assigns tiles of several problems to each CTA, with some SMs kept free for the wgrad group. This removes per-GEMM launch overhead and the tail underutilisation of small GEMMs. It also drops the earlier split of dense apply across streams (the wgrad_rest event and the hole/range logic), which gives up that overlap of the dense update with the sparse side stream.

```diff
diff --git a/wide_deep_b200/csrc/api.cu b/wide_deep_b200/csrc/api.cu
--- a/wide_deep_b200/csrc/api.cu
+++ b/wide_deep_b200/csrc/api.cu
@@ -460,7 +460,7 @@
     for (cudaStream_t* s : {&m->stream, &m->stream_up, &m->sstream[0], &m->sstream[1]})
         if (e == cudaSuccess) e = new_stream(m, s);
     for (cudaEvent_t* ev : {&m->ev_grouped[0], &m->ev_grouped[1], &m->ev_done[0], &m->ev_done[1], &m->ev_ids, &m->ev_wide_fwd,
-                            &m->ev_wgrad_rest, &m->ev_head, &m->ev_dx0, &m->ev_bwd_done})
+                            &m->ev_head, &m->ev_dx0, &m->ev_bwd_done})
         if (e == cudaSuccess) e = new_event(m, ev, cudaEventDisableTiming);
     if (e != cudaSuccess) { set_error("cudaStreamCreate: %s", cudaGetErrorString(e)); wd_model_destroy(m); return WD_ECUDA; }
     m->graphs_enabled = getenv("WD_NO_GRAPH") == nullptr;
@@ -914,11 +914,8 @@
     }
     m->record_dx0 = m->side_pending[0];
     m->dx0_recorded = false;
-    m->dense_split_tensor = -1;
-    m->record_wgrad_rest = m->fuse_dense && m->side_active[1] && m->operands == kBf16Operands && !m->timer.enabled && !m->crelu;
     if ((rc = mlp_backward(m))) return rc;
     m->record_dx0 = false;
-    m->record_wgrad_rest = false;
     mark(m, "mlp_other");
     stamp(m, ST_BWD);
     if (m->side_pending[0] && m->dx0_recorded) {
@@ -949,28 +946,18 @@
 
 int apply_core(WdModel* m) {
     int rc;
-    const bool split_dense = m->fuse_dense && m->dense_split_tensor >= 0 && m->side_active[1];
     for (int w = 0; w < 2; ++w) {
         if (m->side_active[w]) {
             if ((rc = on_side(m, w, [&]() -> int {
                     int r = sparse_apply_which(m, w);
                     stamp(m, ST_A0_END + w);
-                    if (!r && w == 1 && split_dense) {
-                        WD_CUDA(cudaStreamWaitEvent(m->stream, m->ev_wgrad_rest, 0));
-                        m->dense_part = 2;
-                        r = dense_apply(m);
-                        m->dense_part = 0;
-                    }
                     return r;
                 }))) return rc;
             WD_CUDA(cudaEventRecord(m->ev_done[w], m->sstream[w]));
         } else if ((rc = sparse_apply_which(m, w))) return rc;
     }
     mark(m, "sparse_apply");
-    m->dense_part = split_dense ? 1 : 0;
-    rc = dense_apply(m);
-    m->dense_part = 0;
-    if (rc) return rc;
+    if ((rc = dense_apply(m))) return rc;
     if ((rc = small_apply(m))) return rc;
     mark(m, "dense_apply");
     stamp(m, ST_MAIN_END);
diff --git a/wide_deep_b200/csrc/common.cuh b/wide_deep_b200/csrc/common.cuh
--- a/wide_deep_b200/csrc/common.cuh
+++ b/wide_deep_b200/csrc/common.cuh
@@ -3,6 +3,7 @@
 #include <cuda_runtime.h>
 #include <stdint.h>
 #include <stdio.h>
+#include <map>
 #include <string>
 #include <vector>
 
@@ -330,12 +331,10 @@
     cudaStream_t stream = nullptr;
     cudaStream_t sstream[2] = {nullptr, nullptr};
     cudaStream_t stream_up = nullptr;
-    cudaEvent_t ev_ids = nullptr, ev_head = nullptr, ev_dx0 = nullptr, ev_bwd_done = nullptr, ev_wide_fwd = nullptr, ev_wgrad_rest = nullptr;
+    cudaEvent_t ev_ids = nullptr, ev_head = nullptr, ev_dx0 = nullptr, ev_bwd_done = nullptr, ev_wide_fwd = nullptr;
     bool sort_smem_opt_in = false;
     bool crelu = false;
     bool list_apply_fused[2] = {false, false};
-    bool record_wgrad_rest = false;
-    int dense_split_tensor = -1, dense_part = 0;
     cudaEvent_t ev_grouped[2] = {nullptr, nullptr}, ev_done[2] = {nullptr, nullptr};
     bool side_pending[2] = {false, false};
     bool side_active[2] = {false, false};
@@ -406,6 +405,7 @@
     float *d_Wt_hi = nullptr, *d_Wt_lo = nullptr;
     __nv_bfloat16 *d_Wq_hi = nullptr, *d_Wq_lo = nullptr;
     wd::DenseTensor* d_dense_desc = nullptr;
+    std::map<std::vector<int>, const int*> gemm_schedules;
     int row_tiles = 0;
     int wgrad_splits = 4;
 
diff --git a/wide_deep_b200/csrc/gemm.cuh b/wide_deep_b200/csrc/gemm.cuh
--- a/wide_deep_b200/csrc/gemm.cuh
+++ b/wide_deep_b200/csrc/gemm.cuh
@@ -62,8 +62,12 @@
     uint64_t reserved[5];
 };
 
+struct GemmProblem {
+    GemmA A; GemmB B; int M, N; Epi ep; int splits, ksplit_len;
+};
 int tc_gemm(WdModel* m, int mode, const GemmA& A, const GemmB& B, int M, int N, const Epi& ep, int splits, int ksplit_len);
-int tc_gemm_bf16(WdModel* m, int mode, const GemmA& A, const GemmB& B, int M, int N, const Epi& ep, int splits, int ksplit_len);
+int tc_gemm_bf16(WdModel* m, const GemmA& A, const GemmB& B, int M, int N, const Epi& ep);
+int tc_gemm_bf16_group(WdModel* m, int mode, const GemmProblem* probs, int n);
 int make_tensor_map(CUtensorMap* map, CUtensorMapDataType dtype, const void* ptr, int rows, int cols, int ld, int box_rows);
 
 struct DropArgs { float rate; unsigned long long seed; const unsigned int* step; int layer_id; };
diff --git a/wide_deep_b200/csrc/gemm_bf16.cu b/wide_deep_b200/csrc/gemm_bf16.cu
--- a/wide_deep_b200/csrc/gemm_bf16.cu
+++ b/wide_deep_b200/csrc/gemm_bf16.cu
@@ -2,7 +2,11 @@
 #include <stdlib.h>
 
 #include <algorithm>
+#include <functional>
+#include <queue>
 #include <type_traits>
+#include <utility>
+#include <vector>
 
 #include "common.cuh"
 #include "gemm.cuh"
@@ -24,13 +28,65 @@
 };
 struct QSegs { int n; int k[kMaxSegs]; int koff[kMaxSegs]; };
 
+struct QProblem {
+    CUtensorMap a_hi, a_lo, b_hi, b_lo;
+    int M, N, ktot, ksplit_len, nsplit;
+    float* C; int ldc; int accumulate; int64_t split_stride;
+};
+constexpr int kGroupMax = 16;
+constexpr int kWgradFreeSms = 8;
+struct QGroup { QProblem p[kGroupMax]; };
+static_assert(sizeof(QGroup) + 16 <= 32764, "grouped GEMM parameters exceed the sm_90 limit");
+
+struct QOne {
+    const QMaps& maps; const QSegs& segs; int M_, N_; const Epi& ep; int nkb_all_;
+    __device__ int begin() const { return blockIdx.x; }
+    __device__ int end() const { return ((N_ + QBN - 1) / QBN) * ((M_ + QBM - 1) / QBM); }
+    __device__ int stride() const { return gridDim.x; }
+    __device__ int entry(int i) const { return i; }
+    __device__ int problem(int) const { return 0; }
+    __device__ int tile(int e) const { return e; }
+    __device__ const CUtensorMap* a_hi(int, int s) const { return &maps.a_hi[s]; }
+    __device__ const CUtensorMap* a_lo(int, int s) const { return &maps.a_lo[s]; }
+    __device__ const CUtensorMap* b_hi(int) const { return &maps.b_hi; }
+    __device__ const CUtensorMap* b_lo(int) const { return &maps.b_lo; }
+    __device__ int seg_k(int, int s) const { return segs.k[s]; }
+    __device__ int seg_koff(int, int s) const { return segs.koff[s]; }
+    __device__ int M(int) const { return M_; }
+    __device__ int N(int) const { return N_; }
+    __device__ int nkb_all(int) const { return nkb_all_; }
+};
+struct QGrp {
+    const QGroup& g; const int* __restrict__ sched;
+    __device__ int begin() const { return __ldg(sched + blockIdx.x); }
+    __device__ int end() const { return __ldg(sched + blockIdx.x + 1); }
+    __device__ int stride() const { return 1; }
+    __device__ int entry(int i) const { return __ldg(sched + i); }
+    __device__ int problem(int e) const { return e >> 24; }
+    __device__ int tile(int e) const { return e & 0xFFFFFF; }
+    __device__ const CUtensorMap* a_hi(int p, int) const { return &g.p[p].a_hi; }
+    __device__ const CUtensorMap* a_lo(int p, int) const { return &g.p[p].a_lo; }
+    __device__ const CUtensorMap* b_hi(int p) const { return &g.p[p].b_hi; }
+    __device__ const CUtensorMap* b_lo(int p) const { return &g.p[p].b_lo; }
+    __device__ int seg_k(int p, int) const { return g.p[p].ktot; }
+    __device__ int seg_koff(int, int) const { return 0; }
+    __device__ int M(int p) const { return g.p[p].M; }
+    __device__ int N(int p) const { return g.p[p].N; }
+    __device__ int ktot(int p) const { return g.p[p].ktot; }
+    __device__ int ksplit_len(int p) const { return g.p[p].ksplit_len; }
+    __device__ int nkb_all(int p) const { return (g.p[p].ktot + 63) / 64; }
+    __device__ float* C(int p) const { return g.p[p].C; }
+    __device__ int ldc(int p) const { return g.p[p].ldc; }
+    __device__ int accumulate(int p) const { return g.p[p].accumulate; }
+    __device__ int64_t split_stride(int p) const { return g.p[p].split_stride; }
+};
+
 __device__ unsigned long long g_probe[32 * 8];
 __device__ __forceinline__ unsigned long long gtime() { unsigned long long t; asm volatile("mov.u64 %0, %globaltimer;" : "=l"(t)); return t; }
 #define PROBE(i) do { if (probe >= 0 && blockIdx.x == 0 && (threadIdx.x & 127) == 0) g_probe[probe * 8 + (i)] = gtime(); } while (0)
 
-template <int MODE>
-__global__ void __launch_bounds__(Q_THREADS, 1) tc_gemm_bf16_kernel(const __grid_constant__ QMaps maps, const QSegs segs, int M, int N, int ktot,
-                                                                   int ksplit_len, int nsplit, Epi ep, int probe) {
+template <int MODE, class S>
+__device__ __forceinline__ void q_gemm(const S& src, int probe) {
     extern __shared__ uint8_t smem_raw[];
     uint8_t* base = reinterpret_cast<uint8_t*>((reinterpret_cast<uintptr_t>(smem_raw) + 1023) & ~uintptr_t(1023));
     constexpr bool A_MN = MODE == EPI_WGRAD;
@@ -46,20 +102,17 @@
     float* epi_vec = reinterpret_cast<float*>(base + QNST * STAGE_BYTES + 64);
 
     const int warp = threadIdx.x >> 5, lane = threadIdx.x & 31, wg = threadIdx.x >> 7;
-    const int tiles_n = (N + QBN - 1) / QBN, tiles_m = (M + QBM - 1) / QBM;
-    const int ntiles = tiles_n * tiles_m * nsplit;
-    int nkb_all = 0;
-    for (int s = 0; s < segs.n; ++s) nkb_all += (segs.k[s] + QBK - 1) / QBK;
-    auto tile_range = [&](int tile, int& m0, int& n0, int& z, int& kbeg, int& nkb) {
+    auto tile_range = [&](int p, int tile, int& m0, int& n0, int& z, int& kbeg, int& nkb) {
+        const int tiles_n = (src.N(p) + QBN - 1) / QBN, tiles_m = (src.M(p) + QBM - 1) / QBM;
         z = tile / (tiles_n * tiles_m);
         int r = tile % (tiles_n * tiles_m);
         m0 = (r / tiles_n) * QBM;
         n0 = (r % tiles_n) * QBN;
         kbeg = 0;
-        nkb = nkb_all;
-        if (MODE == EPI_WGRAD) {
-            kbeg = z * ksplit_len;
-            int kend = min(ktot, kbeg + ksplit_len);
+        nkb = src.nkb_all(p);
+        if constexpr (MODE == EPI_WGRAD) {
+            kbeg = z * src.ksplit_len(p);
+            int kend = min(src.ktot(p), kbeg + src.ksplit_len(p));
             nkb = kend > kbeg ? (kend - kbeg + QBK - 1) / QBK : 0;
         }
     };
@@ -75,9 +128,10 @@
         PROBE(0);
         if (warp == 0 && lane == 0) {
             int g = 0;
-            for (int tile = blockIdx.x; tile < ntiles; tile += gridDim.x) {
+            for (int i = src.begin(); i < src.end(); i += src.stride()) {
+                const int e = src.entry(i), p = src.problem(e);
                 int m0, n0, z, kbeg, nkb;
-                tile_range(tile, m0, n0, z, kbeg, nkb);
+                tile_range(p, src.tile(e), m0, n0, z, kbeg, nkb);
                 int seg = 0, kin = 0;
                 for (int kb = 0; kb < nkb; ++kb, ++g) {
                     const int s = g % QNST, it = g / QNST;
@@ -85,29 +139,29 @@
                     int ka, kbcoord;
                     if (MODE == EPI_WGRAD) { ka = kbeg + kb * QBK; kbcoord = ka; }
                     else {
-                        if (kin >= segs.k[seg]) { ++seg; kin = 0; }
-                        ka = kin; kbcoord = segs.koff[seg] + kin;
+                        if (kin >= src.seg_k(p, seg)) { ++seg; kin = 0; }
+                        ka = kin; kbcoord = src.seg_koff(p, seg) + kin;
                         kin += QBK;
                     }
                     mbar_expect_tx(&full[s], 2 * (A_BYTES + B_BYTES));
                     if (!A_MN) {
-                        tma_load_2d(a_hi(s), &maps.a_hi[seg], &full[s], ka, m0);
-                        tma_load_2d(a_lo(s), &maps.a_lo[seg], &full[s], ka, m0);
+                        tma_load_2d(a_hi(s), src.a_hi(p, seg), &full[s], ka, m0);
+                        tma_load_2d(a_lo(s), src.a_lo(p, seg), &full[s], ka, m0);
                     } else {
 #pragma unroll
                         for (int i = 0; i < QBM / 64; ++i) {
-                            tma_load_2d(a_hi(s) + i * 8192, &maps.a_hi[seg], &full[s], m0 + 64 * i, ka);
-                            tma_load_2d(a_lo(s) + i * 8192, &maps.a_lo[seg], &full[s], m0 + 64 * i, ka);
+                            tma_load_2d(a_hi(s) + i * 8192, src.a_hi(p, seg), &full[s], m0 + 64 * i, ka);
+                            tma_load_2d(a_lo(s) + i * 8192, src.a_lo(p, seg), &full[s], m0 + 64 * i, ka);
                         }
                     }
                     if (!B_MN) {
-                        tma_load_2d(b_hi(s), &maps.b_hi, &full[s], kbcoord, n0);
-                        tma_load_2d(b_lo(s), &maps.b_lo, &full[s], kbcoord, n0);
+                        tma_load_2d(b_hi(s), src.b_hi(p), &full[s], kbcoord, n0);
+                        tma_load_2d(b_lo(s), src.b_lo(p), &full[s], kbcoord, n0);
                     } else {
 #pragma unroll
                         for (int i = 0; i < QBN / 64; ++i) {
-                            tma_load_2d(b_hi(s) + i * 8192, &maps.b_hi, &full[s], n0 + 64 * i, kbcoord);
-                            tma_load_2d(b_lo(s) + i * 8192, &maps.b_lo, &full[s], n0 + 64 * i, kbcoord);
+                            tma_load_2d(b_hi(s) + i * 8192, src.b_hi(p), &full[s], n0 + 64 * i, kbcoord);
+                            tma_load_2d(b_lo(s) + i * 8192, src.b_lo(p), &full[s], n0 + 64 * i, kbcoord);
                         }
                     }
                 }
@@ -120,16 +174,19 @@
         constexpr int TA = A_MN ? 1 : 0, TB = B_MN ? 1 : 0;
         float d[QBN / 2];
         int g = 0, use = 0;
-        for (int tile = blockIdx.x; tile < ntiles; tile += gridDim.x) {
+        for (int i = src.begin(); i < src.end(); i += src.stride()) {
+            const int e = src.entry(i), p = src.problem(e);
+            const int M = src.M(p), N = src.N(p);
             int m0, n0, z, kbeg, nkb;
-            tile_range(tile, m0, n0, z, kbeg, nkb);
+            tile_range(p, src.tile(e), m0, n0, z, kbeg, nkb);
             if (nkb == 0) {
 #pragma unroll
                 for (int i = 0; i < QBN / 2; ++i) d[i] = 0.f;
             }
             const int ct = threadIdx.x - 128;
             float pre[2] = {0.f, 0.f};
-            if (MODE == EPI_FWD) {
+            if constexpr (MODE == EPI_FWD) {
+                const Epi& ep = src.ep;
 #pragma unroll
                 for (int i = 0; i < 2; ++i) {
                     const int v = ct + 256 * i, c = n0 + (v & 127);
@@ -177,13 +234,14 @@
             const int r0 = m0 + cw * 64 + (warp & 3) * 16 + (lane >> 2);
             const int cq = 2 * (lane & 3);
             auto epilogue = [&](auto relu) {
-                constexpr bool RELU = decltype(relu)::value;
-                uint32_t qh[2][2] = {}, ql[2][2] = {};
+                [[maybe_unused]] constexpr bool RELU = decltype(relu)::value;
+                [[maybe_unused]] uint32_t qh[2][2] = {}, ql[2][2] = {};
 #pragma unroll
                 for (int j = 0; j < QBN / 8; ++j) {
                     const int c = n0 + 8 * j + cq;
                     if (n0 + 8 * j < N) {
-                        if (MODE == EPI_FWD) {
+                        if constexpr (MODE == EPI_FWD) {
+                            const Epi& ep = src.ep;
                             const bool in0 = c < ep.n_logical, in1 = c + 1 < ep.n_logical;
                             const int cl = 8 * j + cq;
                             const float b0 = ev[cl], b1 = ev[cl + 1], g0 = ev[128 + cl], g1 = ev[129 + cl], e0 = ev[256 + cl], e1 = ev[257 + cl];
@@ -220,21 +278,23 @@
                                 }
                             }
                         } else {
-                            float* Cb = ep.C + (MODE == EPI_WGRAD ? (int64_t)z * ep.split_stride : 0);
+                            float* Cb = src.C(p) + (MODE == EPI_WGRAD ? (int64_t)z * src.split_stride(p) : 0);
 #pragma unroll
                             for (int hh = 0; hh < 2; ++hh) {
                                 const int r = r0 + 8 * hh;
                                 if (r >= M) continue;
-                                float2* pc = reinterpret_cast<float2*>(Cb + (int64_t)r * ep.ldc + c);
+                                float2* pc = reinterpret_cast<float2*>(Cb + (int64_t)r * src.ldc(p) + c);
                                 float2 o = make_float2(d[4 * j + 2 * hh], d[4 * j + 2 * hh + 1]);
-                                if (MODE == EPI_STORE && ep.accumulate) { const float2 p = *pc; o.x += p.x; o.y += p.y; }
+                                if (MODE == EPI_STORE && src.accumulate(p)) { const float2 p = *pc; o.x += p.x; o.y += p.y; }
                                 *pc = o;
                             }
                         }
                     }
                 }
             };
-            if (MODE == EPI_FWD && ep.act == WD_ACT_RELU) epilogue(std::true_type{});
+            bool relu = false;
+            if constexpr (MODE == EPI_FWD) relu = src.ep.act == WD_ACT_RELU;
+            if (relu) epilogue(std::true_type{});
             else epilogue(std::false_type{});
             if (cwarp == 0) PROBE(use == 0 ? 4 : 5);
             ++use;
@@ -242,26 +302,115 @@
     }
 }
 
+template <int MODE>
+__global__ void __launch_bounds__(Q_THREADS, 1) tc_gemm_bf16_kernel(const __grid_constant__ QMaps maps, const QSegs segs, int M, int N, int ktot,
+                                                                   int ksplit_len, int nsplit, Epi ep, int probe) {
+    int nkb_all = 0;
+    for (int s = 0; s < segs.n; ++s) nkb_all += (segs.k[s] + QBK - 1) / QBK;
+    q_gemm<MODE>(QOne{maps, segs, M, N, ep, nkb_all}, probe);
+}
+template <int MODE>
+__global__ void __launch_bounds__(Q_THREADS, 1) tc_gemm_bf16_group_kernel(const __grid_constant__ QGroup grp, const int* __restrict__ sched, int probe) {
+    q_gemm<MODE>(QGrp{grp, sched}, probe);
+}
+
+constexpr int kQSmem = QNST * 2 * (QBM * 128 + QBN * 128) + 1024 + 64 + 2 * 384 * 4;
 int g_probe_slot = 0;
 
+template <auto kernel>
+int q_configure(WdModel* m, int* num_sms) {
+    static bool configured = false;
+    static int sms = 0;
+    if (!configured) {
+        WD_CUDA(cudaFuncSetAttribute(kernel, cudaFuncAttributeMaxDynamicSharedMemorySize, kQSmem));
+        WD_CUDA(cudaDeviceGetAttribute(&sms, cudaDevAttrMultiProcessorCount, m->device));
+        configured = true;
+    }
+    *num_sms = sms;
+    return WD_OK;
+}
+int probe_slot() {
+    static const bool probe_on = getenv("WD_GEMM_PROBE") != nullptr;
+    return probe_on ? (g_probe_slot++ & 31) : -1;
+}
+
+int tile_kblocks(int mode, const QProblem& P, int tile) {
+    if (mode != EPI_WGRAD) return (P.ktot + QBK - 1) / QBK;
+    const int z = tile / (((P.N + QBN - 1) / QBN) * ((P.M + QBM - 1) / QBM));
+    const int kbeg = z * P.ksplit_len, kend = std::min(P.ktot, kbeg + P.ksplit_len);
+    return kend > kbeg ? (kend - kbeg + QBK - 1) / QBK : 0;
+}
+
+std::vector<int> group_schedule(int mode, const QProblem* P, int np, int grid) {
+    std::vector<std::pair<int, int>> t;
+    for (int p = 0; p < np; ++p) {
+        const int nt = ((P[p].N + QBN - 1) / QBN) * ((P[p].M + QBM - 1) / QBM) * P[p].nsplit;
+        for (int i = 0; i < nt; ++i) t.push_back({tile_kblocks(mode, P[p], i), p << 24 | i});
+    }
+    std::stable_sort(t.begin(), t.end(), [](const std::pair<int, int>& a, const std::pair<int, int>& b) { return a.first > b.first; });
+    std::priority_queue<std::pair<int64_t, int>, std::vector<std::pair<int64_t, int>>, std::greater<std::pair<int64_t, int>>> load;
+    for (int c = 0; c < grid; ++c) load.push({0, c});
+    std::vector<std::vector<int>> per(grid);
+    for (const auto& x : t) {
+        const auto l = load.top();
+        load.pop();
+        per[l.second].push_back(x.second);
+        load.push({l.first + x.first + 1, l.second});
+    }
+    std::vector<int> out(grid + 1);
+    for (int c = 0; c < grid; ++c) {
+        out[c] = (int)out.size();
+        out.insert(out.end(), per[c].begin(), per[c].end());
+    }
+    out[grid] = (int)out.size();
+    return out;
+}
+
+int schedule_on_device(WdModel* m, int mode, const QProblem* P, int np, int grid, const int** out) {
+    std::vector<int> key{mode, grid};
+    for (int p = 0; p < np; ++p) key.insert(key.end(), {P[p].M, P[p].N, P[p].ktot, P[p].ksplit_len, P[p].nsplit});
+    auto it = m->gemm_schedules.find(key);
+    if (it != m->gemm_schedules.end()) { *out = it->second; return WD_OK; }
+    const std::vector<int> h = group_schedule(mode, P, np, grid);
+    cudaStreamCaptureMode cm = cudaStreamCaptureModeRelaxed;
+    WD_CUDA(cudaThreadExchangeStreamCaptureMode(&cm));
+    int* d = nullptr;
+    int rc = dev_alloc(m, &d, (int64_t)h.size(), false);
+    cudaError_t e = cudaSuccess;
+    if (!rc) e = cudaMemcpy(d, h.data(), h.size() * sizeof(int), cudaMemcpyHostToDevice);
+    if (!rc && e == cudaSuccess) e = cudaStreamSynchronize(cudaStreamLegacy);
+    cudaThreadExchangeStreamCaptureMode(&cm);
+    if (rc) return rc;
+    if (e != cudaSuccess) { set_error("bf16 GEMM engine: schedule upload: %s", cudaGetErrorString(e)); return WD_ECUDA; }
+    m->gemm_schedules[key] = d;
+    *out = d;
+    return WD_OK;
+}
+
 template <int MODE>
-int launch_q(WdModel* m, const QMaps& maps, const QSegs& segs, int M, int N, int ktot, int splits, int ksplit_len, const Epi& ep) {
-    constexpr int smem = QNST * 2 * (QBM * 128 + QBN * 128) + 1024 + 64 + 2 * 384 * 4;
-    static bool configured = false;
-    static int num_sms = 0;
-    if (!configured) {
-        WD_CUDA(cudaFuncSetAttribute(tc_gemm_bf16_kernel<MODE>, cudaFuncAttributeMaxDynamicSharedMemorySize, smem));
-        WD_CUDA(cudaDeviceGetAttribute(&num_sms, cudaDevAttrMultiProcessorCount, m->device));
-        configured = true;
-    }
-    const int nsplit = MODE == EPI_WGRAD ? splits : 1;
-    const int ntiles = ((N + QBN - 1) / QBN) * ((M + QBM - 1) / QBM) * nsplit;
-    static const bool probe_on = getenv("WD_GEMM_PROBE") != nullptr;
-    const int probe = probe_on ? (g_probe_slot++ & 31) : -1;
-    tc_gemm_bf16_kernel<MODE><<<ntiles < num_sms ? ntiles : num_sms, Q_THREADS, smem, m->stream>>>(maps, segs, M, N, ktot, ksplit_len, nsplit, ep, probe);
+int launch_group(WdModel* m, const QGroup& grp, int np) {
+    int rc, num_sms;
+    if ((rc = q_configure<tc_gemm_bf16_group_kernel<MODE>>(m, &num_sms))) return rc;
+    int ntiles = 0;
+    for (int p = 0; p < np; ++p) ntiles += ((grp.p[p].N + QBN - 1) / QBN) * ((grp.p[p].M + QBM - 1) / QBM) * grp.p[p].nsplit;
+    const int grid = std::min(ntiles, MODE == EPI_WGRAD ? std::max(1, num_sms - kWgradFreeSms) : num_sms);
+    const int* sched;
+    if ((rc = schedule_on_device(m, MODE, grp.p, np, grid, &sched))) return rc;
+    tc_gemm_bf16_group_kernel<MODE><<<grid, Q_THREADS, kQSmem, m->stream>>>(grp, sched, probe_slot());
     m->launches++;
     WD_CUDA(cudaGetLastError());
     return WD_OK;
+}
+
+int q_map_pair(CUtensorMap* hi, CUtensorMap* lo, const __nv_bfloat16* phi, const __nv_bfloat16* plo, bool mn, int rows, int k, int ld, int box_rows) {
+    constexpr CUtensorMapDataType BF16 = CU_TENSOR_MAP_DATA_TYPE_BFLOAT16;
+    int rc;
+    if (!mn) {
+        if ((rc = make_tensor_map(hi, BF16, phi, rows, k, ld, box_rows))) return rc;
+        return make_tensor_map(lo, BF16, plo, rows, k, ld, box_rows);
+    }
+    if ((rc = make_tensor_map(hi, BF16, phi, k, rows, ld, 64))) return rc;
+    return make_tensor_map(lo, BF16, plo, k, rows, ld, 64);
 }
 
 }
@@ -273,39 +422,55 @@
     return e == cudaSuccess ? 0 : -1;
 }
 
-int tc_gemm_bf16(WdModel* m, int mode, const GemmA& A, const GemmB& B, int M, int N, const Epi& ep, int splits, int ksplit_len) {
-    constexpr CUtensorMapDataType BF16 = CU_TENSOR_MAP_DATA_TYPE_BFLOAT16;
+int tc_gemm_bf16(WdModel* m, const GemmA& A, const GemmB& B, int M, int N, const Epi& ep) {
     if (N % 32 != 0 || A.n > kMaxSegs || !B.hi || !B.lo) { set_error("bf16 GEMM engine: unsupported operands"); return WD_EUNSUPPORTED; }
+    if (!ep.Hs_hi || !ep.Hs_lo) { set_error("bf16 GEMM engine: epilogue without hi/lo outputs"); return WD_EINVAL; }
     QMaps maps;
     QSegs segs{};
     segs.n = A.n;
     int rc, ktot = 0;
-    const bool a_mn = mode == EPI_WGRAD, b_mn = mode == EPI_FWD || mode == EPI_WGRAD;
     for (int s = 0; s < A.n; ++s) {
         if (!A.hi[s] || !A.lo[s]) { set_error("bf16 GEMM engine: operand without hi/lo copies"); return WD_EINVAL; }
-        if (!a_mn) {
-            if ((rc = make_tensor_map(&maps.a_hi[s], BF16, A.hi[s], M, A.k[s], A.ld[s], QBM))) return rc;
-            if ((rc = make_tensor_map(&maps.a_lo[s], BF16, A.lo[s], M, A.k[s], A.ld[s], QBM))) return rc;
-        } else {
-            if ((rc = make_tensor_map(&maps.a_hi[s], BF16, A.hi[s], A.k[s], M, A.ld[s], 64))) return rc;
-            if ((rc = make_tensor_map(&maps.a_lo[s], BF16, A.lo[s], A.k[s], M, A.ld[s], 64))) return rc;
-        }
+        if ((rc = q_map_pair(&maps.a_hi[s], &maps.a_lo[s], A.hi[s], A.lo[s], false, M, A.k[s], A.ld[s], QBM))) return rc;
         segs.k[s] = A.k[s]; segs.koff[s] = ktot;
         ktot += A.k[s];
     }
     for (int s = A.n; s < kMaxSegs; ++s) { maps.a_hi[s] = maps.a_hi[0]; maps.a_lo[s] = maps.a_lo[0]; }
-    if (!b_mn) {
-        if ((rc = make_tensor_map(&maps.b_hi, BF16, B.hi, N, ktot, B.ld, QBN))) return rc;
-        if ((rc = make_tensor_map(&maps.b_lo, BF16, B.lo, N, ktot, B.ld, QBN))) return rc;
-    } else {
-        if ((rc = make_tensor_map(&maps.b_hi, BF16, B.hi, ktot, N, B.ld, 64))) return rc;
-        if ((rc = make_tensor_map(&maps.b_lo, BF16, B.lo, ktot, N, B.ld, 64))) return rc;
-    }
-    if (mode == EPI_WGRAD) ksplit_len = (ksplit_len + QBK - 1) / QBK * QBK;
-    if (mode == EPI_FWD && (!ep.Hs_hi || !ep.Hs_lo)) { set_error("bf16 GEMM engine: epilogue without hi/lo outputs"); return WD_EINVAL; }
-    if (mode == EPI_FWD) return launch_q<EPI_FWD>(m, maps, segs, M, N, ktot, splits, ksplit_len, ep);
-    if (mode == EPI_STORE) return launch_q<EPI_STORE>(m, maps, segs, M, N, ktot, splits, ksplit_len, ep);
-    return launch_q<EPI_WGRAD>(m, maps, segs, M, N, ktot, splits, ksplit_len, ep);
-}
-
-}
+    if ((rc = q_map_pair(&maps.b_hi, &maps.b_lo, B.hi, B.lo, true, N, ktot, B.ld, QBN))) return rc;
+    int num_sms;
+    if ((rc = q_configure<tc_gemm_bf16_kernel<EPI_FWD>>(m, &num_sms))) return rc;
+    const int ntiles = ((N + QBN - 1) / QBN) * ((M + QBM - 1) / QBM);
+    tc_gemm_bf16_kernel<EPI_FWD><<<std::min(ntiles, num_sms), Q_THREADS, kQSmem, m->stream>>>(maps, segs, M, N, ktot, 0, 1, ep, probe_slot());
+    m->launches++;
+    WD_CUDA(cudaGetLastError());
+    return WD_OK;
+}
+
+int tc_gemm_bf16_group(WdModel* m, int mode, const GemmProblem* probs, int n) {
+    if (mode != EPI_STORE && mode != EPI_WGRAD) { set_error("bf16 GEMM engine: a group is of data or weight gradients"); return WD_EINVAL; }
+    const bool mn = mode == EPI_WGRAD;
+    for (int i0 = 0; i0 < n; i0 += kGroupMax) {
+        const int np = std::min(kGroupMax, n - i0);
+        QGroup grp;
+        for (int j = 0; j < np; ++j) {
+            const GemmProblem& g = probs[i0 + j];
+            if (g.N % 32 != 0 || g.A.n != 1 || !g.A.hi[0] || !g.A.lo[0] || !g.B.hi || !g.B.lo) {
+                set_error("bf16 GEMM engine: unsupported grouped operands"); return WD_EUNSUPPORTED;
+            }
+            QProblem& P = grp.p[j];
+            const int ktot = g.A.k[0];
+            int rc;
+            if ((rc = q_map_pair(&P.a_hi, &P.a_lo, g.A.hi[0], g.A.lo[0], mn, g.M, ktot, g.A.ld[0], QBM))) return rc;
+            if ((rc = q_map_pair(&P.b_hi, &P.b_lo, g.B.hi, g.B.lo, mn, g.N, ktot, g.B.ld, QBN))) return rc;
+            P.M = g.M; P.N = g.N; P.ktot = ktot;
+            P.ksplit_len = mn ? (g.ksplit_len + QBK - 1) / QBK * QBK : 0;
+            P.nsplit = mn ? g.splits : 1;
+            P.C = g.ep.C; P.ldc = g.ep.ldc; P.accumulate = g.ep.accumulate; P.split_stride = g.ep.split_stride;
+        }
+        const int rc = mode == EPI_STORE ? launch_group<EPI_STORE>(m, grp, np) : launch_group<EPI_WGRAD>(m, grp, np);
+        if (rc) return rc;
+    }
+    return WD_OK;
+}
+
+}
diff --git a/wide_deep_b200/csrc/mlp.cu b/wide_deep_b200/csrc/mlp.cu
--- a/wide_deep_b200/csrc/mlp.cu
+++ b/wide_deep_b200/csrc/mlp.cu
@@ -139,29 +139,52 @@
     m->launches++;
 }
 
+static const char* gemm_mark(int mode, int layer) {
+    static const char* kNames[3][4] = {{"gemm_fwd_l0", "gemm_fwd_l1", "gemm_fwd_l2", "gemm_fwd_l3+"},
+                                       {"gemm_dgrad_l0", "gemm_dgrad_l1", "gemm_dgrad_l2", "gemm_dgrad_l3+"},
+                                       {"gemm_wgrad_l0", "gemm_wgrad_l1", "gemm_wgrad_l2", "gemm_wgrad_l3+"}};
+    return kNames[mode][layer < 3 ? layer : 3];
+}
+
 static int run_gemm(WdModel* m, int mode, const GemmA& A, const GemmB& B, int M, int N, const Epi& ep, int splits = 1, int ksplit_len = 0) {
-    static const char* kNamesL[3][4] = {{"gemm_fwd_l0", "gemm_fwd_l1", "gemm_fwd_l2", "gemm_fwd_l3+"},
-                                        {"gemm_dgrad_l0", "gemm_dgrad_l1", "gemm_dgrad_l2", "gemm_dgrad_l3+"},
-                                        {"gemm_wgrad_l0", "gemm_wgrad_l1", "gemm_wgrad_l2", "gemm_wgrad_l3+"}};
-    const char* kNames[3] = {kNamesL[0][m->cur_layer < 3 ? m->cur_layer : 3], kNamesL[1][m->cur_layer < 3 ? m->cur_layer : 3],
-                             kNamesL[2][m->cur_layer < 3 ? m->cur_layer : 3]};
+    const char* name = gemm_mark(mode, m->cur_layer);
     mark(m, "mlp_other");
     if (m->operands == kBf16Operands) {
-        int rc = tc_gemm_bf16(m, mode, A, B, M, N, ep, splits, ksplit_len);
-        mark(m, kNames[mode]);
+        if (mode != EPI_FWD) { set_error("bf16x3: gradient GEMMs run as groups"); return WD_EINVAL; }
+        int rc = tc_gemm_bf16(m, A, B, M, N, ep);
+        mark(m, name);
         return rc;
     }
     if (m->gemm_engine == WD_GEMM_TC3X || m->gemm_engine == WD_GEMM_TC1X) {
         int rc = tc_gemm(m, mode, A, B, M, N, ep, splits, ksplit_len);
-        if (rc != WD_EUNSUPPORTED) { mark(m, kNames[mode]); return rc; }
+        if (rc != WD_EUNSUPPORTED) { mark(m, name); return rc; }
         m->gemm_fallbacks++;
         static bool warned = false;
         if (!warned) { fprintf(stderr, "libwd_b200: wgmma engine does not cover a GEMM (M=%d N=%d segs=%d): running it on the FFMA kernel\n", M, N, A.n); warned = true; }
     }
     launch_gemm(m, mode, A, B, M, N, ep, splits, ksplit_len);
-    mark(m, kNames[mode]);
+    mark(m, name);
     return WD_OK;
 }
+
+struct GemmGroup {
+    WdModel* m;
+    int mode;
+    std::vector<GemmProblem> probs;
+    int add(const GemmProblem& p) {
+        if (m->operands != kBf16Operands) return run_gemm(m, mode, p.A, p.B, p.M, p.N, p.ep, p.splits, p.ksplit_len);
+        probs.push_back(p);
+        return WD_OK;
+    }
+    int flush(const char* name) {
+        if (probs.empty()) return WD_OK;
+        mark(m, "mlp_other");
+        const int rc = tc_gemm_bf16_group(m, mode, probs.data(), (int)probs.size());
+        mark(m, name);
+        probs.clear();
+        return rc;
+    }
+};
 
 __global__ void transpose_kernel(const float* __restrict__ in, int ld_in, int M, int Mpad, int N, float* __restrict__ out, int ld_out) {
     __shared__ float t[32][33];
@@ -597,9 +620,8 @@
 __global__ void __launch_bounds__(256) dense_vec_kernel(const DenseTensor* __restrict__ T, int nt, int64_t total4, const float* __restrict__ gpart,
                                                         float* __restrict__ G, float* __restrict__ P, float* __restrict__ S1, float* __restrict__ S2,
                                                         __nv_bfloat16* __restrict__ Wq_hi, __nv_bfloat16* __restrict__ Wq_lo, OptParamsD dnn, OptParamsD lin, int lin_tensor,
-                                                        int live_row_tiles, int64_t begin4, int64_t hole_lo4, int64_t hole_hi4) {
-    for (int64_t i4 = begin4 + (int64_t)blockIdx.x * blockDim.x + threadIdx.x; i4 < total4; i4 += (int64_t)gridDim.x * blockDim.x) {
-        if (i4 >= hole_lo4 && i4 < hole_hi4) continue;
+                                                        int live_row_tiles) {
+    for (int64_t i4 = (int64_t)blockIdx.x * blockDim.x + threadIdx.x; i4 < total4; i4 += (int64_t)gridDim.x * blockDim.x) {
         const int64_t i = i4 * 4;
         int lo = 0, hi = nt - 1;
         while (lo < hi) {
@@ -865,42 +887,42 @@
                                                        L.t_gamma >= 0 ? m->d_P + m->dense[L.t_gamma].off : nullptr, m->activation,
                                                        m->batch_norm, L.dZ, L.dZT, m->ldt, pb, pg, pbe, m->dense[L.t_bias].gstride, dr);
             if (!fused[l]) m->launches++;
+            GemmGroup dg{m, EPI_STORE, {}};
             for (int s = 0; s < L.n_in_segs; ++s) {
                 const Seg& sg = L.segs[s];
                 if (sg.src < 0 && !need_dx0) continue;
                 float* dst; int dld, acc;
                 grad_dst(sg.src, &dst, &dld, &acc);
-                GemmA A{}; GemmB W{};
-                dgrad_operands(m, L, sg, A, W);
-                Epi ep{};
-                ep.C = dst; ep.ldc = dld; ep.accumulate = acc;
-                int rc = run_gemm(m, EPI_STORE, A, W, B, sg.width_phys, ep);
+                GemmProblem g{};
+                dgrad_operands(m, L, sg, g.A, g.B);
+                g.M = B; g.N = sg.width_phys; g.splits = 1;
+                g.ep.C = dst; g.ep.ldc = dld; g.ep.accumulate = acc;
+                int rc = dg.add(g);
                 if (rc) return rc;
             }
+            if (int rc = dg.flush(gemm_mark(EPI_STORE, l))) return rc;
             if (l == 0 && &tw == &m->towers.back() && need_dx0 && m->ev_dx0 && m->record_dx0) {
                 WD_CUDA(cudaEventRecord(m->ev_dx0, m->stream));
                 m->dx0_recorded = true;
             }
         }
+        GemmGroup wg{m, EPI_WGRAD, {}};
         for (int l = tw.n_hidden - 1; l >= 0; --l) {
             Layer& L = tw.layers[l];
             m->cur_layer = l;
             const DenseTensor& tkn = m->dense[L.t_kernel];
-            if (l == 0 && m->record_wgrad_rest && m->towers.size() == 1 && L.n_in_segs == 1) {
-                WD_CUDA(cudaEventRecord(m->ev_wgrad_rest, m->stream));
-                m->dense_split_tensor = L.t_kernel;
-            }
             for (int s = 0; s < L.n_in_segs; ++s) {
                 const Seg& sg = L.segs[s];
-                GemmA A{}; GemmB W{};
-                wgrad_operands(m, tw, L, sg, A, W);
-                Epi ep{};
-                ep.C = m->d_gpart + tkn.gpart_off + (int64_t)sg.k_off * L.N_phys; ep.ldc = L.N_phys; ep.split_stride = tkn.gstride;
-                const int ks = ((Bk + L.wgrad_splits - 1) / L.wgrad_splits + 31) / 32 * 32;
-                int rc = run_gemm(m, EPI_WGRAD, A, W, sg.width_phys, L.N_phys, ep, L.wgrad_splits, ks);
+                GemmProblem g{};
+                wgrad_operands(m, tw, L, sg, g.A, g.B);
+                g.M = sg.width_phys; g.N = L.N_phys; g.splits = L.wgrad_splits;
+                g.ksplit_len = ((Bk + L.wgrad_splits - 1) / L.wgrad_splits + 31) / 32 * 32;
+                g.ep.C = m->d_gpart + tkn.gpart_off + (int64_t)sg.k_off * L.N_phys; g.ep.ldc = L.N_phys; g.ep.split_stride = tkn.gstride;
+                int rc = wg.add(g);
                 if (rc) return rc;
             }
         }
+        if (int rc = wg.flush("gemm_wgrad")) return rc;
     }
     WD_CUDA(cudaGetLastError());
     return WD_OK;
@@ -956,7 +978,7 @@
         if (m->fuse_dense) return WD_OK;
         OptParamsD z{};
         dense_vec_kernel<0><<<grid_for(m->dense_count / 4, 256), 256, 0, m->stream>>>(m->d_dense_desc, (int)m->dense.size(), m->dense_count / 4, m->d_gpart,
-            m->d_G, nullptr, nullptr, nullptr, nullptr, nullptr, z, z, -1, rts, 0, 0, 0);
+            m->d_G, nullptr, nullptr, nullptr, nullptr, nullptr, z, z, -1, rts);
         m->launches++;
         WD_CUDA(cudaGetLastError());
         return WD_OK;
@@ -976,18 +998,12 @@
     if (m->operands == kBf16Operands) {
         const int rts = (m->dbatch.B + 127) / 128;
         const int g = grid_for(m->dense_count / 4, 256);
-        if (m->fuse_dense) {
-            int64_t b4 = 0, e4 = m->dense_count / 4, hlo = 0, hhi = 0;
-            if (m->dense_part && m->dense_split_tensor >= 0) {
-                const DenseTensor& t = m->dense[m->dense_split_tensor];
-                const int64_t k0 = t.off / 4, k1 = (t.off + t.count + 3) / 4;
-                if (m->dense_part == 1) { b4 = k0; e4 = k1; } else { hlo = k0; hhi = k1; }
-            }
-            dense_vec_kernel<2><<<grid_for(e4 - b4, 256), 256, 0, m->stream>>>(m->d_dense_desc, (int)m->dense.size(), e4, m->d_gpart, m->d_G, m->d_P,
-                                                                                m->d_S1, m->d_S2, m->d_Wq_hi, m->d_Wq_lo, d, l, lin_tensor, rts, b4, hlo, hhi);
-        } else
+        if (m->fuse_dense)
+            dense_vec_kernel<2><<<g, 256, 0, m->stream>>>(m->d_dense_desc, (int)m->dense.size(), m->dense_count / 4, m->d_gpart, m->d_G, m->d_P,
+                                                          m->d_S1, m->d_S2, m->d_Wq_hi, m->d_Wq_lo, d, l, lin_tensor, rts);
+        else
             dense_vec_kernel<1><<<g, 256, 0, m->stream>>>(m->d_dense_desc, (int)m->dense.size(), m->dense_count / 4, m->d_gpart, m->d_G, m->d_P, m->d_S1,
-                                                          m->d_S2, m->d_Wq_hi, m->d_Wq_lo, d, l, lin_tensor, rts, 0, 0, 0);
+                                                          m->d_S2, m->d_Wq_hi, m->d_Wq_lo, d, l, lin_tensor, rts);
         m->launches++;
         WD_CUDA(cudaGetLastError());
         return WD_OK;
```

Result: no change. 10.54 million (median of 6 runs) (+0.5%).
